# OPTML-Group/Unlearn-Saliency

Measured on AMD Instinct MI355X. Metric: unlearn_steps_per_sec (ResNet-18/CIFAR-10 10%-forget, RL + SalUn mask, batch 256/GPU), higher is better.
Workload: dtype f32

## Files before the change

include/salun.h:

```cpp
#ifndef SALUN_H
#define SALUN_H

#include <stddef.h>
#include <stdint.h>

#ifdef __cplusplus
extern "C" {
#endif

#define SALUN_OK 0
#define SALUN_EINVAL (-22)
#define SALUN_ENOSPC (-28)
#define SALUN_EIO (-5)

#define SALUN_MAX_THRESHOLDS 16

typedef void *salun_stream_t;

int salun_version(void);
const char *salun_strerror(int code);
const char *salun_arch(void);
int salun_clock_probe(unsigned long long *out , int samples, int spins, salun_stream_t stream);

int salun_saliency_accumulate(float *acc , const float *g ,
                              double scale, const float *sqnorm ,
                              double max_norm, int64_t n, salun_stream_t stream);

#define SALUN_TOPK_FORCE_FULL_SCAN 1u
#define SALUN_TOPK_VALUES_ONLY 2u
size_t salun_mask_topk_workspace_bytes(int64_t n, int nk);
int salun_mask_topk(const float *acc , int64_t n, const int64_t *ks ,
                    int nk, uint8_t *const *masks_out ,
                    void *ws , size_t ws_bytes, salun_stream_t stream);
int salun_mask_topk_ex(const float *acc , int64_t n, const int64_t *ks ,
                       int nk, uint8_t *const *masks_out ,
                       void *ws , size_t ws_bytes, unsigned flags, salun_stream_t stream);
int salun_mask_topk_status(const void *ws , int *route_out , int *error_out ,
                           salun_stream_t stream);
int salun_mask_topk_thresholds(const void *ws , int nk, float *tau_out ,
                               salun_stream_t stream);

int salun_mask_u8_to_i64(const uint8_t *m , int64_t *out , int64_t n,
                         salun_stream_t stream);
int salun_mask_i64_to_u8(const int64_t *m , uint8_t *out , int64_t n,
                         salun_stream_t stream);
int salun_mask_popcount(const uint8_t *m , int64_t n, int64_t *count ,
                        void *ws , size_t ws_bytes, salun_stream_t stream);

int salun_masked_sgd_step(float *p , const float *g , float *buf ,
                          const uint8_t *m , double lr, double mu,
                          double wd, int first_step, int64_t n, salun_stream_t stream);

size_t salun_reduce_workspace_bytes(int64_t n);
int salun_grad_sqnorm(const float *g , int64_t n, float *out ,
                      void *ws , size_t ws_bytes, salun_stream_t stream);

int salun_masked_adam_step(float *p , const float *g , float *m1 ,
                           float *v , const uint8_t *mask ,
                           const float *sqnorm , double max_norm,
                           double gscale, double lr, double b1, double b2, double eps,
                           double wd, int step, int64_t n, salun_stream_t stream);

int salun_adam_coefficients(int64_t *step , double lr, double b1, double b2, float *coef ,
                            salun_stream_t stream);
int salun_masked_adam_step_coef(float *p , const float *g , float *m1 , float *v ,
                                const uint8_t *mask , const float *sqnorm ,
                                double max_norm, double gscale, const float *coef , double b1, double b2,
                                double eps, double wd, int64_t n, salun_stream_t stream);

int salun_adam_ema_step(float *p , const float *g , float *m1 , float *v ,
                        float *shadow , const uint8_t *mask ,
                        const float *sqnorm , double max_norm, double gscale, double lr, double b1,
                        double b2, double eps, double wd, double mu, int step, int64_t n, salun_stream_t stream);
int salun_adam_ema_step_coef(float *p , const float *g , float *m1 , float *v ,
                             float *shadow , const uint8_t *mask ,
                             const float *sqnorm , double max_norm, double gscale,
                             const float *coef , double b1, double b2, double eps, double wd, double mu,
                             int64_t n, salun_stream_t stream);

int salun_qsample(const float *x0 , const float *e ,
                  const float *sqrt_ab , const float *sqrt_1mab ,
                  const int64_t *t , int64_t T, float *xt , int64_t B,
                  int64_t chw, salun_stream_t stream);

size_t salun_sqerr_workspace_bytes(int64_t B, int64_t chw);
int salun_sqerr_loss(const float *a , const float *b , int64_t B,
                     int64_t chw, double coef, float *loss ,
                     float *per_sample , float *dloss_db ,
                     void *ws , size_t ws_bytes, salun_stream_t stream);

int salun_fim_square_accumulate(float *F , float *tmp , double n_data,
                                int64_t n, salun_stream_t stream);

int salun_conv2d_forward(const float *x , const float *w , const float *bias ,
                         float *y , int N, int C, int H, int W, int K, int R, int stride, int pad,
                         int P, int Q, salun_stream_t stream);
int salun_conv2d_forward_fused(const float *x , const float *w , const float *bias ,
                               const float *nbias , const float *addend ,
                               float *y , int N, int C, int H, int W, int K, int R, int stride, int pad,
                               int P, int Q, void *ws , size_t ws_bytes, salun_stream_t stream);
size_t salun_conv2d_data_workspace_bytes(int N, int outC, int outH, int outW, int R, int conv_stride);
int salun_conv2d_backward_data_ws(const float *dy , const float *w , const float *addend ,
                                  float *dx , int N, int C, int H, int W, int K, int R, int stride, int pad,
                                  int P, int Q, void *ws , size_t ws_bytes, salun_stream_t stream);
int salun_conv2d_backward_data(const float *dy , const float *w , float *dx , int N, int C,
                               int H, int W, int K, int R, int stride, int pad, int P, int Q,
                               salun_stream_t stream);
int salun_conv2d_backward_data_add(const float *dy , const float *w , const float *addend ,
                                   float *dx , int N, int C, int H, int W, int K, int R, int stride, int pad,
                                   int P, int Q, salun_stream_t stream);
size_t salun_channel_sum_workspace_bytes(int N, int K);
int salun_channel_sum(const float *dy , float *out , int N, int K, int HW, int accumulate,
                      void *ws , size_t ws_bytes, salun_stream_t stream);
size_t salun_conv2d_wgrad_workspace_bytes(int N, int C, int K, int R, int P, int Q);
int salun_conv2d_backward_weight(const float *x , const float *dy , float *dw , int N, int C,
                                 int H, int W, int K, int R, int stride, int pad, int P, int Q, int accumulate,
                                 void *ws , size_t ws_bytes, salun_stream_t stream);
#define SALUN_WGRAD_SHARED 1u
int salun_conv2d_backward_weight_ex(const float *x , const float *dy , float *dw , int N, int C,
                                    int H, int W, int K, int R, int stride, int pad, int P, int Q, int accumulate,
                                    unsigned flags, void *ws , size_t ws_bytes, salun_stream_t stream);

size_t salun_conv3x3_pack_bytes(int K, int C, int dgrad);
#define SALUN_PACK_MAX_JOBS 32
typedef struct {
  const float *w;
  float *img_fwd;
  float *img_dgrad;
  int32_t K, C;
} salun_pack_job_t;
int salun_conv3x3_pack_weights(const salun_pack_job_t *jobs , int njobs, salun_stream_t stream);
int salun_conv3x3_packed(const float *x , const float *img , const float *bias ,
                         const float *nbias , const float *addend , float *y ,
                         int N, int Cred, int H, int W, int Kout, int cfg, salun_stream_t stream);

int salun_conv2d_bf16_supported(int C, int K, int R, int stride, int pad);
int salun_conv2d_bf16_pack_weights(const float *w , uint16_t *wp , int K, int C, int R,
                                   salun_stream_t stream);
#define SALUN_BF16_PACK_MAX_JOBS 64
typedef struct {
  const float *w;
  uint16_t *wp;
  int32_t K, C, R, transposed;
} salun_bf16_pack_job_t;
int salun_bf16_pack_weights_batch(const salun_bf16_pack_job_t *jobs, int n, salun_stream_t stream);
size_t salun_conv2d_bf16_data_workspace_bytes(int N, int H, int W, int C, int K, int R, int stride, int pad);
int salun_conv2d_bf16_forward(const uint16_t *x , const uint16_t *wp , const float *bias ,
                              const float *nbias , const uint16_t *addend ,
                              uint16_t *y , int N, int H, int W, int C, int K, int R, int stride, int pad,
                              void *ws , size_t ws_bytes, salun_stream_t stream);
int salun_conv2d_bf16_backward_data(const uint16_t *dy , const uint16_t *wp ,
                                    const uint16_t *addend , uint16_t *dx , int N, int H, int W,
                                    int C, int K, int R, int stride, int pad, void *ws , size_t ws_bytes,
                                    salun_stream_t stream);
size_t salun_conv2d_bf16_wgrad_workspace_bytes(int N, int H, int W, int C, int K, int R, int stride, int pad);
int salun_conv2d_bf16_backward_weight(const uint16_t *x , const uint16_t *dy , float *dw ,
                                      float *db , int N, int H, int W, int C, int K, int R, int stride,
                                      int pad, int accumulate, void *ws , size_t ws_bytes,
                                      salun_stream_t stream);
size_t salun_colsum_bf16_workspace_bytes(int K);
int salun_colsum_bf16(const uint16_t *dy , float *db , float *dnb , int64_t M, int K,
                      int images, int accumulate, void *ws , size_t ws_bytes, salun_stream_t stream);
int salun_conv2d_bf16_backward_weight_ex(const uint16_t *x , const uint16_t *dy , float *dw ,
                                         float *db , float *dnb , int N, int H, int W, int C,
                                         int K, int R, int stride, int pad, int accumulate, void *ws ,
                                         size_t ws_bytes, salun_stream_t stream);

size_t salun_gn_bf16_workspace_bytes(int N, int C, int HW, int G);
int salun_gn_bf16_forward(const uint16_t *x , const float *gamma , const float *beta ,
                          uint16_t *y , float *mr , float *ab , int N, int C, int HW, int G,
                          double eps, int silu, void *ws , size_t ws_bytes, salun_stream_t stream);
int salun_gn_bf16_backward(const uint16_t *dy , const uint16_t *x , const float *gamma ,
                           const float *mr , const float *ab , uint16_t *dx , float *dgamma ,
                           float *dbeta , int N, int C, int HW, int G, int silu, int accumulate, void *ws ,
                           size_t ws_bytes, salun_stream_t stream);

int salun_attn_supported(int D);
int salun_attn_forward(const uint16_t *q , const uint16_t *k , const uint16_t *v , uint16_t *o ,
                       float *lse , int B, int H, int Nq, int Nk, int D, long long q_bs, int q_ld,
                       long long k_bs, int k_ld, long long v_bs, int v_ld, long long o_bs, int o_ld, double scale,
                       salun_stream_t stream);
int salun_attn_backward(const uint16_t *q , const uint16_t *k , const uint16_t *v ,
                        const uint16_t *o , const uint16_t *d_o , const float *lse ,
                        uint16_t *dq , uint16_t *dk , uint16_t *dv , float *dsum , int B, int H,
                        int Nq, int Nk, int D, long long q_bs, int q_ld, long long k_bs, int k_ld, long long v_bs, int v_ld,
                        long long o_bs, int o_ld, long long do_bs, int do_ld, double scale, salun_stream_t stream);

size_t salun_ln_bf16_workspace_bytes(int64_t rows, int C);
int salun_ln_bf16_forward(const uint16_t *x , const float *gamma , const float *beta ,
                          uint16_t *y , float *stats , int64_t rows, int C, double eps,
                          salun_stream_t stream);
int salun_ln_bf16_backward(const uint16_t *dy , const uint16_t *x , const float *gamma ,
                           const float *stats , uint16_t *dx , float *dgamma , float *dbeta ,
                           int64_t rows, int C, int accumulate, void *ws , size_t ws_bytes, salun_stream_t stream);
int salun_geglu_bf16_forward(const uint16_t *h , uint16_t *out , int64_t rows, int F, salun_stream_t stream);
int salun_geglu_bf16_backward(const uint16_t *h , const uint16_t *dy , uint16_t *dh , int64_t rows,
                              int F, salun_stream_t stream);

size_t salun_bn_workspace_bytes(int C);
int salun_bn_forward(const float *x , const float *res , float *y ,
                     const float *gamma , const float *beta , float *running_mean ,
                     float *running_var , long long *num_batches_tracked ,
                     float *save_mean , float *save_invstd ,
                     int N, int C, int HW, int training, double momentum, double eps, int relu, void *ws ,
                     size_t ws_bytes, salun_stream_t stream);
int salun_bn_backward(const float *dy , const float *y , const float *x ,
                      const float *gamma , const float *save_mean , const float *save_invstd ,
                      float *dx , float *dres , float *dgamma , float *dbeta ,
                      float *grad_gamma_acc , float *grad_beta_acc ,
                      int N, int C, int HW, int training, int relu, void *ws , size_t ws_bytes,
                      salun_stream_t stream);

size_t salun_gn_workspace_bytes(int N, int C);
int salun_gn_forward(const float *x , float *y , const float *gamma , const float *beta ,
                     float *save_mean , float *save_rstd , int N, int C, int HW, int G, double eps,
                     int silu, salun_stream_t stream);
int salun_gn_backward(const float *dz , const float *x , const float *gamma ,
                      const float *beta , const float *save_mean , const float *save_rstd ,
                      float *dx , float *dgamma , float *dbeta ,
                      float *grad_gamma_acc , float *grad_beta_acc ,
                      int N, int C, int HW, int G, int silu, void *ws , size_t ws_bytes,
                      salun_stream_t stream);

int salun_gn_backward_fused(const float *dz , const float *x , const float *gamma ,
                            const float *beta , const float *save_mean , const float *save_rstd ,
                            const float *addend , float *dx , float *dgamma ,
                            float *dbeta , float *grad_gamma_acc ,
                            float *grad_beta_acc , float *nk_sum ,
                            float *csum , float *csum_acc , int N, int C, int HW, int G,
                            int silu, void *ws , size_t ws_bytes, salun_stream_t stream);

int salun_param_diff(const float *p , const float *p0 , float *out , int64_t n,
                     salun_stream_t stream);
int salun_soft_threshold_step(float *p , const float *p0 , const float *tau ,
                              int64_t n, salun_stream_t stream);

size_t salun_ewc_workspace_bytes(int64_t n);
int salun_ewc_penalty_grad(const float *p , const float *p_star , const float *F ,
                           float *g , double lambda, float *loss_out , int64_t n,
                           void *ws , size_t ws_bytes, salun_stream_t stream);

int salun_image_batch(const uint8_t *data , const int64_t *idx ,
                      const int32_t *crop , const uint8_t *flip ,
                      float *out , int64_t B, int H, int W, int C, int pad,
                      salun_stream_t stream);

#define SALUN_GEMM_MAX_JOBS 32
#define SALUN_GEMM_MAX_SEGS 32
typedef struct {
  const float *A , *B ;
  int32_t K;
  int32_t a_i, a_k, b_j, b_k;
} salun_gemm_seg_t;
typedef struct {
  float *C ;
  const float *bias ;
  int32_t M, N, ldc;
  int32_t seg0, nseg;
  int32_t accumulate;
} salun_gemm_job_t;
size_t salun_gemm_f32_workspace_bytes(const salun_gemm_job_t *jobs , int njobs,
                                      const salun_gemm_seg_t *segs , int nsegs,
                                      int batch_outer, int batch_inner);
int salun_gemm_f32(const salun_gemm_job_t *jobs , int njobs, const salun_gemm_seg_t *segs , int nsegs,
                   int batch_outer, int batch_inner, const int64_t *batch_strides ,
                   double alpha, void *ws , size_t ws_bytes, salun_stream_t stream);
size_t salun_colsum_f32_workspace_bytes(int64_t M, int N);
int salun_colsum_f32(const float *x , float *out , int64_t M, int N, int64_t ld, int accumulate,
                     void *ws , size_t ws_bytes, salun_stream_t stream);
int salun_softmax_rows(float *s , int64_t rows, int n, int ld, salun_stream_t stream);
int salun_softmax_rows_backward(const float *p , float *dp , int64_t rows, int n, int ld,
                                double scale, salun_stream_t stream);

int salun_gemm_bf16_supported(int64_t M, int N, int K);
int salun_gemm_bf16_nt(const void *x , const void *w , const float *bias ,
                       const void *addend , void *y , int64_t M, int N, int K,
                       int variant, salun_stream_t stream);
int salun_gemm_bf16_tn_supported(int64_t M, int Na, int Nb);
size_t salun_gemm_bf16_tn_workspace_bytes(int64_t M, int Na, int Nb, int variant);
int salun_gemm_bf16_tn(const void *dy , const void *x , float *dw , int64_t M, int Na, int Nb,
                       int accumulate, int variant, void *ws , size_t ws_bytes, salun_stream_t stream);
int salun_pack_bf16(const float *w , void *wp , int N, int K, int transposed, salun_stream_t stream);

int salun_dropout(const float *x , float *y , int64_t n_samples, int64_t chw,
                  int64_t sample_offset, double p, uint64_t seed,
                  const uint64_t *seed_dev , salun_stream_t stream);
int salun_u64_add(uint64_t *value , uint64_t inc, salun_stream_t stream);

size_t salun_iu_dot_workspace_bytes(int B, int64_t n);
int salun_iu_conv_dot(const float *y2 , const float *dy , int B, int64_t n, double *out ,
                      void *ws , size_t ws_bytes, salun_stream_t stream);
int salun_iu_bn_dot(const float *x , const float *dy , const float *running_mean ,
                    const float *running_var , double eps, const float *u0_gamma ,
                    const float *u0_beta , const float *u1_gamma , const float *u1_beta ,
                    int B, int C, int HW, double *out , void *ws , size_t ws_bytes,
                    salun_stream_t stream);
int salun_iu_linear_dot(const float *x , const float *dy , const float *u0_w ,
                        const float *u0_b , const float *u1_w , const float *u1_b ,
                        int B, int M, int K, double *out , salun_stream_t stream);
int salun_iu_recurrence(const double *ab , int64_t n, double N, double *out ,
                        salun_stream_t stream);
int salun_iu_apply(float *p , const float *v , const float *g0 , const double *beta ,
                   const uint8_t *mask , double alpha, int64_t n, salun_stream_t stream);

size_t salun_ff_conv_sq_workspace_bytes(int G, int B, int C, int K, int R, int P, int Q);
int salun_ff_conv_sq(const float *x , const float *dy , const float *w , float *F ,
                     int G, int B, int C, int H, int W, int K, int R, int stride, int pad, int P, int Q,
                     void *ws , size_t ws_bytes, salun_stream_t stream);
int salun_ff_linear_sq(const float *x , const float *dy , const float *w , float *F ,
                       int G, int B, int M, int K, salun_stream_t stream);
size_t salun_ff_vec_sq_workspace_bytes(int G, int C);
int salun_ff_vec_sq(const float *x , const float *dy , const float *running_mean ,
                    const float *running_var , double eps, const float *w , int G, int B,
                    int C, int HW, float *F_gamma , float *F_beta , void *ws ,
                    size_t ws_bytes, salun_stream_t stream);
int salun_ff_apply(float *p , const float *F , const int64_t *table , int nparam, int64_t ntiles,
                   double nbatches, double alpha, uint64_t seed, salun_stream_t stream);

int salun_fill_uniform(float *out , int64_t n, uint64_t seed, double lo, double hi,
                       salun_stream_t stream);
int salun_fill_normal(float *out , int64_t n, uint64_t seed, double mean, double std,
                      salun_stream_t stream);
int salun_fill_u8(uint8_t *out , int64_t n, uint64_t seed, salun_stream_t stream);

#define SALUN_SAMPLER_ANCESTRAL 0
#define SALUN_SAMPLER_GENERALIZED 1
int salun_sampler_step(const float *x_t , const float *eps_cond , const float *eps_null ,
                       double cond_scale, const float *abar , int table_len, int idx_t, int idx_next, int variant,
                       double eta, const float *noise , uint64_t seed,
                       const int64_t *image_ids , int64_t step, float *x_next ,
                       float *x0 , int64_t B, int64_t chw, salun_stream_t stream);

int salun_sampler_noise(float *out , uint64_t seed, const int64_t *image_ids , int64_t step, int64_t B,
                        int64_t chw, salun_stream_t stream);

size_t salun_minmax_workspace_bytes(int64_t n);
int salun_minmax(const float *x , int64_t n, float *lohi , void *ws , size_t ws_bytes,
                 salun_stream_t stream);

int salun_images_to_u8(const float *x , uint8_t *out , int64_t B, int C, int HW, int rescaled,
                       const float *range , salun_stream_t stream);

#ifdef __cplusplus
}
#endif
#endif
```

unlearn_saliency_amd/_lib.py:

```python
from __future__ import annotations

import ctypes
import os
import subprocess

_HERE = os.path.dirname(os.path.abspath(__file__))
LIB_PATH = os.environ.get("SALUN_LIB") or os.path.join(_HERE, "libsalun.so")
CSRC_DIR = os.path.join(_HERE, "csrc")

SALUN_OK = 0
SALUN_EINVAL = -22
SALUN_ENOSPC = -28
SALUN_EIO = -5
SALUN_MAX_THRESHOLDS = 16
SALUN_TOPK_FORCE_FULL_SCAN = 1
SALUN_TOPK_VALUES_ONLY = 2
SALUN_WGRAD_SHARED = 1

c_void_p, c_int, c_int64, c_uint64 = ctypes.c_void_p, ctypes.c_int, ctypes.c_int64, ctypes.c_uint64
c_double, c_size_t = ctypes.c_double, ctypes.c_size_t

class GemmSeg(ctypes.Structure):
    _fields_ = [("A", c_void_p), ("B", c_void_p), ("K", ctypes.c_int32), ("a_i", ctypes.c_int32),
                ("a_k", ctypes.c_int32), ("b_j", ctypes.c_int32), ("b_k", ctypes.c_int32)]


class GemmJob(ctypes.Structure):
    _fields_ = [("C", c_void_p), ("bias", c_void_p), ("M", ctypes.c_int32), ("N", ctypes.c_int32),
                ("ldc", ctypes.c_int32), ("seg0", ctypes.c_int32), ("nseg", ctypes.c_int32),
                ("accumulate", ctypes.c_int32)]


class PackJob(ctypes.Structure):
    _fields_ = [("w", c_void_p), ("img_fwd", c_void_p), ("img_dgrad", c_void_p), ("K", ctypes.c_int32),
                ("C", ctypes.c_int32)]


class Bf16PackJob(ctypes.Structure):
    _fields_ = [("w", c_void_p), ("wp", c_void_p), ("K", ctypes.c_int32), ("C", ctypes.c_int32), ("R", ctypes.c_int32),
                ("transposed", ctypes.c_int32)]


SALUN_BF16_PACK_MAX_JOBS = 64
SALUN_GEMM_MAX_JOBS = 32
SALUN_GEMM_MAX_SEGS = 32

SIGNATURES = {
    "salun_version": (c_int, []),
    "salun_strerror": (ctypes.c_char_p, [c_int]),
    "salun_arch": (ctypes.c_char_p, []),
    "salun_clock_probe": (c_int, [c_void_p, c_int, c_int, c_void_p]),
    "salun_saliency_accumulate": (c_int, [c_void_p, c_void_p, c_double, c_void_p, c_double, c_int64, c_void_p]),
    "salun_mask_topk_workspace_bytes": (c_size_t, [c_int64, c_int]),
    "salun_mask_topk": (c_int, [c_void_p, c_int64, ctypes.POINTER(c_int64), c_int, ctypes.POINTER(c_void_p),
                                c_void_p, c_size_t, c_void_p]),
    "salun_mask_topk_ex": (c_int, [c_void_p, c_int64, ctypes.POINTER(c_int64), c_int, ctypes.POINTER(c_void_p),
                                   c_void_p, c_size_t, ctypes.c_uint, c_void_p]),
    "salun_mask_topk_status": (c_int, [c_void_p, ctypes.POINTER(c_int), ctypes.POINTER(c_int), c_void_p]),
    "salun_mask_topk_thresholds": (c_int, [c_void_p, c_int, c_void_p, c_void_p]),
    "salun_mask_u8_to_i64": (c_int, [c_void_p, c_void_p, c_int64, c_void_p]),
    "salun_mask_i64_to_u8": (c_int, [c_void_p, c_void_p, c_int64, c_void_p]),
    "salun_mask_popcount": (c_int, [c_void_p, c_int64, c_void_p, c_void_p, c_size_t, c_void_p]),
    "salun_masked_sgd_step": (c_int, [c_void_p, c_void_p, c_void_p, c_void_p, c_double, c_double, c_double, c_int,
                                      c_int64, c_void_p]),
    "salun_reduce_workspace_bytes": (c_size_t, [c_int64]),
    "salun_grad_sqnorm": (c_int, [c_void_p, c_int64, c_void_p, c_void_p, c_size_t, c_void_p]),
    "salun_masked_adam_step": (c_int, [c_void_p, c_void_p, c_void_p, c_void_p, c_void_p, c_void_p, c_double,
                                       c_double, c_double, c_double, c_double, c_double, c_double, c_int, c_int64,
                                       c_void_p]),
    "salun_adam_coefficients": (c_int, [c_void_p, c_double, c_double, c_double, c_void_p, c_void_p]),
    "salun_masked_adam_step_coef": (c_int, [c_void_p, c_void_p, c_void_p, c_void_p, c_void_p, c_void_p, c_double,
                                            c_double, c_void_p, c_double, c_double, c_double, c_double, c_int64,
                                            c_void_p]),
    "salun_adam_ema_step": (c_int, [c_void_p, c_void_p, c_void_p, c_void_p, c_void_p, c_void_p, c_void_p, c_double,
                                    c_double, c_double, c_double, c_double, c_double, c_double, c_double, c_int, c_int64,
                                    c_void_p]),
    "salun_adam_ema_step_coef": (c_int, [c_void_p, c_void_p, c_void_p, c_void_p, c_void_p, c_void_p, c_void_p, c_double,
                                         c_double, c_void_p, c_double, c_double, c_double, c_double, c_double, c_int64,
                                         c_void_p]),
    "salun_qsample": (c_int, [c_void_p, c_void_p, c_void_p, c_void_p, c_void_p, c_int64, c_void_p, c_int64, c_int64,
                              c_void_p]),
    "salun_sqerr_workspace_bytes": (c_size_t, [c_int64, c_int64]),
    "salun_sqerr_loss": (c_int, [c_void_p, c_void_p, c_int64, c_int64, c_double, c_void_p, c_void_p, c_void_p,
                                 c_void_p, c_size_t, c_void_p]),
    "salun_fim_square_accumulate": (c_int, [c_void_p, c_void_p, c_double, c_int64, c_void_p]),
    "salun_conv2d_forward": (c_int, [c_void_p, c_void_p, c_void_p, c_void_p] + [c_int] * 10 + [c_void_p]),
    "salun_conv2d_forward_fused": (c_int, [c_void_p] * 6 + [c_int] * 10 + [c_void_p, c_size_t, c_void_p]),
    "salun_conv2d_data_workspace_bytes": (c_size_t, [c_int] * 6),
    "salun_conv2d_backward_data_ws": (c_int, [c_void_p] * 4 + [c_int] * 10 + [c_void_p, c_size_t, c_void_p]),
    "salun_conv2d_backward_data": (c_int, [c_void_p, c_void_p, c_void_p] + [c_int] * 10 + [c_void_p]),
    "salun_channel_sum_workspace_bytes": (c_size_t, [c_int] * 2),
    "salun_channel_sum": (c_int, [c_void_p, c_void_p] + [c_int] * 4 + [c_void_p, c_size_t, c_void_p]),
    "salun_conv2d_wgrad_workspace_bytes": (c_size_t, [c_int] * 6),
    "salun_conv3x3_pack_bytes": (c_size_t, [c_int] * 3),
    "salun_conv3x3_pack_weights": (c_int, [c_void_p, c_int, c_void_p]),
    "salun_conv3x3_packed": (c_int, [c_void_p] * 6 + [c_int] * 6 + [c_void_p]),
    "salun_conv2d_backward_weight": (c_int, [c_void_p, c_void_p, c_void_p] + [c_int] * 11 + [c_void_p, c_size_t,
                                                                                          c_void_p]),
    "salun_conv2d_backward_weight_ex": (c_int, [c_void_p, c_void_p, c_void_p] + [c_int] * 11 + [ctypes.c_uint, c_void_p,
                                                                                                 c_size_t, c_void_p]),
    "salun_conv2d_bf16_supported": (c_int, [c_int] * 5),
    "salun_conv2d_bf16_pack_weights": (c_int, [c_void_p, c_void_p, c_int, c_int, c_int, c_void_p]),
    "salun_bf16_pack_weights_batch": (c_int, [c_void_p, c_int, c_void_p]),
    "salun_conv2d_bf16_data_workspace_bytes": (c_size_t, [c_int] * 8),
    "salun_conv2d_bf16_forward": (c_int, [c_void_p] * 6 + [c_int] * 8 + [c_void_p, c_size_t, c_void_p]),
    "salun_conv2d_bf16_backward_data": (c_int, [c_void_p] * 4 + [c_int] * 8 + [c_void_p, c_size_t, c_void_p]),
    "salun_conv2d_bf16_wgrad_workspace_bytes": (c_size_t, [c_int] * 8),
    "salun_conv2d_bf16_backward_weight": (c_int, [c_void_p] * 4 + [c_int] * 9 + [c_void_p, c_size_t, c_void_p]),
    "salun_colsum_bf16_workspace_bytes": (c_size_t, [c_int]),
    "salun_colsum_bf16": (c_int, [c_void_p, c_void_p, c_void_p, c_int64, c_int, c_int, c_int, c_void_p, c_size_t, c_void_p]),
    "salun_conv2d_bf16_backward_weight_ex": (c_int, [c_void_p] * 5 + [c_int] * 9 + [c_void_p, c_size_t, c_void_p]),
    "salun_gn_bf16_workspace_bytes": (c_size_t, [c_int] * 4),
    "salun_gn_bf16_forward": (c_int, [c_void_p] * 6 + [c_int] * 4 + [c_double, c_int, c_void_p, c_size_t, c_void_p]),
    "salun_gn_bf16_backward": (c_int, [c_void_p] * 8 + [c_int] * 6 + [c_void_p, c_size_t, c_void_p]),
    "salun_attn_supported": (c_int, [c_int]),
    "salun_attn_forward": (c_int, [c_void_p] * 5 + [c_int] * 5 + [ctypes.c_longlong, c_int] * 4 + [c_double, c_void_p]),
    "salun_attn_backward": (c_int, [c_void_p] * 10 + [c_int] * 5 + [ctypes.c_longlong, c_int] * 5 + [c_double, c_void_p]),
    "salun_ln_bf16_workspace_bytes": (c_size_t, [c_int64, c_int]),
    "salun_ln_bf16_forward": (c_int, [c_void_p] * 5 + [c_int64, c_int, c_double, c_void_p]),
    "salun_ln_bf16_backward": (c_int, [c_void_p] * 7 + [c_int64, c_int, c_int, c_void_p, c_size_t, c_void_p]),
    "salun_geglu_bf16_forward": (c_int, [c_void_p, c_void_p, c_int64, c_int, c_void_p]),
    "salun_geglu_bf16_backward": (c_int, [c_void_p, c_void_p, c_void_p, c_int64, c_int, c_void_p]),
    "salun_bn_workspace_bytes": (c_size_t, [c_int]),
    "salun_bn_forward": (c_int, [c_void_p] * 10 + [c_int] * 4 + [c_double, c_double, c_int, c_void_p, c_size_t, c_void_p]),
    "salun_bn_backward": (c_int, [c_void_p] * 12 + [c_int] * 5 + [c_void_p, c_size_t, c_void_p]),
    "salun_conv2d_backward_data_add": (c_int, [c_void_p] * 4 + [c_int] * 10 + [c_void_p]),
    "salun_gn_workspace_bytes": (c_size_t, [c_int, c_int]),
    "salun_gn_forward": (c_int, [c_void_p] * 6 + [c_int] * 4 + [c_double, c_int, c_void_p]),
    "salun_gn_backward": (c_int, [c_void_p] * 11 + [c_int] * 5 + [c_void_p, c_size_t, c_void_p]),
    "salun_gn_backward_fused": (c_int, [c_void_p] * 15 + [c_int] * 5 + [c_void_p, c_size_t, c_void_p]),
    "salun_param_diff": (c_int, [c_void_p, c_void_p, c_void_p, c_int64, c_void_p]),
    "salun_soft_threshold_step": (c_int, [c_void_p, c_void_p, c_void_p, c_int64, c_void_p]),
    "salun_ewc_workspace_bytes": (c_size_t, [c_int64]),
    "salun_ewc_penalty_grad": (c_int, [c_void_p] * 4 + [c_double, c_void_p, c_int64, c_void_p, c_size_t, c_void_p]),
    "salun_image_batch": (c_int, [c_void_p, c_void_p, c_void_p, c_void_p, c_void_p, c_int64, c_int, c_int, c_int,
                                  c_int, c_void_p]),
    "salun_gemm_f32_workspace_bytes": (c_size_t, [ctypes.POINTER(GemmJob), c_int, ctypes.POINTER(GemmSeg), c_int, c_int,
                                                  c_int]),
    "salun_gemm_f32": (c_int, [ctypes.POINTER(GemmJob), c_int, ctypes.POINTER(GemmSeg), c_int, c_int, c_int,
                               ctypes.POINTER(c_int64), c_double, c_void_p, c_size_t, c_void_p]),
    "salun_colsum_f32_workspace_bytes": (c_size_t, [c_int64, c_int]),
    "salun_colsum_f32": (c_int, [c_void_p, c_void_p, c_int64, c_int, c_int64, c_int, c_void_p, c_size_t, c_void_p]),
    "salun_softmax_rows": (c_int, [c_void_p, c_int64, c_int, c_int, c_void_p]),
    "salun_softmax_rows_backward": (c_int, [c_void_p, c_void_p, c_int64, c_int, c_int, c_double, c_void_p]),
    "salun_gemm_bf16_supported": (c_int, [c_int64, c_int, c_int]),
    "salun_gemm_bf16_nt": (c_int, [c_void_p, c_void_p, c_void_p, c_void_p, c_void_p, c_int64, c_int, c_int, c_int, c_void_p]),
    "salun_pack_bf16": (c_int, [c_void_p, c_void_p, c_int, c_int, c_int, c_void_p]),
    "salun_gemm_bf16_tn_supported": (c_int, [c_int64, c_int, c_int]),
    "salun_gemm_bf16_tn_workspace_bytes": (c_size_t, [c_int64, c_int, c_int, c_int]),
    "salun_gemm_bf16_tn": (c_int, [c_void_p, c_void_p, c_void_p, c_int64, c_int, c_int, c_int, c_int, c_void_p, c_size_t, c_void_p]),
    "salun_dropout": (c_int, [c_void_p, c_void_p, c_int64, c_int64, c_int64, c_double, c_uint64, c_void_p, c_void_p]),
    "salun_u64_add": (c_int, [c_void_p, c_uint64, c_void_p]),
    "salun_iu_dot_workspace_bytes": (c_size_t, [c_int, c_int64]),
    "salun_iu_conv_dot": (c_int, [c_void_p, c_void_p, c_int, c_int64, c_void_p, c_void_p, c_size_t, c_void_p]),
    "salun_iu_bn_dot": (c_int, [c_void_p] * 4 + [c_double] + [c_void_p] * 4 + [c_int] * 3 + [c_void_p, c_void_p,
                                                                                           c_size_t, c_void_p]),
    "salun_iu_linear_dot": (c_int, [c_void_p] * 6 + [c_int] * 3 + [c_void_p, c_void_p]),
    "salun_iu_recurrence": (c_int, [c_void_p, c_int64, c_double, c_void_p, c_void_p]),
    "salun_iu_apply": (c_int, [c_void_p] * 5 + [c_double, c_int64, c_void_p]),
    "salun_ff_conv_sq_workspace_bytes": (c_size_t, [c_int] * 7),
    "salun_ff_conv_sq": (c_int, [c_void_p] * 4 + [c_int] * 11 + [c_void_p, c_size_t, c_void_p]),
    "salun_ff_linear_sq": (c_int, [c_void_p] * 4 + [c_int] * 4 + [c_void_p]),
    "salun_ff_vec_sq_workspace_bytes": (c_size_t, [c_int, c_int]),
    "salun_ff_vec_sq": (c_int, [c_void_p] * 4 + [c_double, c_void_p] + [c_int] * 4 + [c_void_p] * 3
                        + [c_size_t, c_void_p]),
    "salun_ff_apply": (c_int, [c_void_p] * 3 + [c_int, c_int64, c_double, c_double, c_uint64, c_void_p]),
    "salun_fill_uniform": (c_int, [c_void_p, c_int64, c_uint64, c_double, c_double, c_void_p]),
    "salun_fill_normal": (c_int, [c_void_p, c_int64, c_uint64, c_double, c_double, c_void_p]),
    "salun_fill_u8": (c_int, [c_void_p, c_int64, c_uint64, c_void_p]),
    "salun_sampler_step": (c_int, [c_void_p, c_void_p, c_void_p, c_double, c_void_p, c_int, c_int, c_int, c_int,
                                   c_double, c_void_p, c_uint64, c_void_p, c_int64, c_void_p, c_void_p, c_int64,
                                   c_int64, c_void_p]),
    "salun_sampler_noise": (c_int, [c_void_p, c_uint64, c_void_p, c_int64, c_int64, c_int64, c_void_p]),
    "salun_minmax_workspace_bytes": (c_size_t, [c_int64]),
    "salun_minmax": (c_int, [c_void_p, c_int64, c_void_p, c_void_p, c_size_t, c_void_p]),
    "salun_images_to_u8": (c_int, [c_void_p, c_void_p, c_int64, c_int, c_int, c_int, c_void_p, c_void_p]),
}

_lib = None


def build(verbose: bool = False) -> str:
    cmd = ["make", "-C", CSRC_DIR, "-j4"] + ([] if verbose else ["-s"])
    subprocess.check_call(cmd)
    if not os.path.exists(LIB_PATH):
        raise RuntimeError(f"build did not produce {LIB_PATH}")
    return LIB_PATH


def lib() -> ctypes.CDLL:
    global _lib
    if _lib is None:
        if not os.path.exists(LIB_PATH):
            raise ImportError(
                f"{LIB_PATH} is missing: the SalUn HIP extension has not been built "
                f"(run `make -C {CSRC_DIR}` or `python -c 'import __graft_entry__ as g; g.build()'`). "
                "There is no CPU fallback.")
        L = ctypes.CDLL(LIB_PATH)
        for name, (res, args) in SIGNATURES.items():
            try:
                fn = getattr(L, name)
            except AttributeError as e:
                raise ImportError(f"{LIB_PATH} does not export {name}; rebuild it") from e
            fn.restype = res
            fn.argtypes = args
        _lib = L
    return _lib


class SalunError(RuntimeError):
    pass


def check(code: int, what: str) -> None:
    if code != SALUN_OK:
        msg = lib().salun_strerror(code).decode()
        raise SalunError(f"{what} failed: {msg} ({code})")
```

unlearn_saliency_amd/csrc/salun_norm.hip:

```cpp
#include "salun_common.h"

namespace {

constexpr int BN_MAX_SPLIT = 64;


struct BnWalk {
  int n, i, dn, di, hw4;
  __device__ __forceinline__ BnWalk(int n_lo, int hw4_) : hw4(hw4_) {
    const int t = threadIdx.x;
    n = n_lo + t / hw4_;
    i = t - (t / hw4_) * hw4_;
    dn = 256 / hw4_;
    di = 256 - dn * hw4_;
  }
  __device__ __forceinline__ void next() {
    n += dn;
    i += di;
    if (i >= hw4) { i -= hw4; ++n; }
  }
};

__global__ __launch_bounds__(256) void k_bn_stats_partial(const float *__restrict__ x, int N, int C, int HW, int nsplit,
                                                          double *__restrict__ partial) {
  __shared__ double lds[4];
  const int c = blockIdx.x, s = blockIdx.y;
  const int n_lo = (int)((int64_t)N * s / nsplit), n_hi = (int)((int64_t)N * (s + 1) / nsplit);
  float s1 = 0.f, s2 = 0.f;
  double d1 = 0.0, d2 = 0.0;
  const int hw4 = HW >> 2;
  const int work = (n_hi - n_lo) * hw4;
  int it = 0;
  BnWalk wk(n_lo, hw4);
#pragma unroll 2
  for (int e = threadIdx.x; e < work; e += 256, ++it, wk.next()) {
    const int n = wk.n, i = wk.i;
    const float4 v = reinterpret_cast<const float4 *>(x + ((size_t)n * C + c) * HW)[i];
    s1 += (v.x + v.y) + (v.z + v.w);
    s2 += (v.x * v.x + v.y * v.y) + (v.z * v.z + v.w * v.w);
    if ((it & 7) == 7) { d1 += s1; d2 += s2; s1 = 0.f; s2 = 0.f; }
  }
  d1 += s1; d2 += s2;
  const double t1 = salun_block_sum(d1, lds);
  const double t2 = salun_block_sum(d2, lds);
  if (threadIdx.x == 0) {
    partial[((size_t)c * nsplit + s) * 2 + 0] = t1;
    partial[((size_t)c * nsplit + s) * 2 + 1] = t2;
  }
}

__device__ __forceinline__ void bn_channel_stats(const double *__restrict__ partial, int c, int nsplit, double M,
                                                 float eps, float *s_out , bool publish,
                                                 float momentum, float *__restrict__ mean, float *__restrict__ invstd,
                                                 float *__restrict__ running_mean, float *__restrict__ running_var) {
  if (threadIdx.x < 64) {
    double s1 = 0.0, s2 = 0.0;
    if ((int)threadIdx.x < nsplit) {
      s1 = partial[((size_t)c * nsplit + threadIdx.x) * 2 + 0];
      s2 = partial[((size_t)c * nsplit + threadIdx.x) * 2 + 1];
    }
    s1 = salun_wave_sum(s1);
    s2 = salun_wave_sum(s2);
    if (threadIdx.x == 0) {
      const double mu = s1 / M;
      double var = s2 / M - mu * mu;
      if (var < 0.0) var = 0.0;
      const float is = (float)(1.0 / sqrt(var + (double)eps));
      s_out[0] = (float)mu;
      s_out[1] = is;
      if (publish) {
        mean[c] = (float)mu;
        invstd[c] = is;
        if (running_mean) {
          running_mean[c] = (1.f - momentum) * running_mean[c] + momentum * (float)mu;
          const double unbiased = (M > 1.0) ? var * M / (M - 1.0) : var;
          running_var[c] = (1.f - momentum) * running_var[c] + momentum * (float)unbiased;
        }
      }
    }
  }
  __syncthreads();
}

template <bool RELU, bool RES, bool TRAIN>
__global__ __launch_bounds__(256) void k_bn_apply(const float *__restrict__ x, const float *__restrict__ res,
                                                  float *__restrict__ y, const double *__restrict__ partial,
                                                  float *__restrict__ mean, float *__restrict__ invstd,
                                                  const float *__restrict__ gamma, const float *__restrict__ beta,
                                                  float *__restrict__ running_mean, float *__restrict__ running_var,
                                                  long long *__restrict__ num_batches_tracked, int N, int C, int HW,
                                                  int nsplit, float eps, float momentum) {
  __shared__ float st[2];
  const int c = blockIdx.x, s = blockIdx.y;
  if (TRAIN) {
    if (num_batches_tracked && c == 0 && s == 0 && threadIdx.x == 0) *num_batches_tracked += 1;
    bn_channel_stats(partial, c, nsplit, (double)N * HW, eps, st, s == 0, momentum, mean, invstd, running_mean,
                     running_var);
  } else {
    if (threadIdx.x == 0) {
      st[0] = running_mean[c];
      st[1] = 1.0f / sqrtf(running_var[c] + eps);
      if (s == 0) { mean[c] = st[0]; invstd[c] = st[1]; }
    }
    __syncthreads();
  }
  const float a = st[1] * gamma[c];
  const float b = beta[c] - st[0] * a;
  const int n_lo = (int)((int64_t)N * s / nsplit), n_hi = (int)((int64_t)N * (s + 1) / nsplit);
  const int hw4 = HW >> 2;
  const int work = (n_hi - n_lo) * hw4;
  BnWalk wk(n_lo, hw4);
#pragma unroll 2
  for (int e = threadIdx.x; e < work; e += 256, wk.next()) {
    const int n = wk.n, i = wk.i;
    const size_t off = ((size_t)n * C + c) * HW;
    const float4 v = reinterpret_cast<const float4 *>(x + off)[i];
    float4 o;
    o.x = v.x * a + b; o.y = v.y * a + b; o.z = v.z * a + b; o.w = v.w * a + b;
    if (RES) {
      const float4 r = reinterpret_cast<const float4 *>(res + off)[i];
      o.x += r.x; o.y += r.y; o.z += r.z; o.w += r.w;
    }
    if (RELU) {
      o.x = o.x > 0.f ? o.x : 0.f; o.y = o.y > 0.f ? o.y : 0.f;
      o.z = o.z > 0.f ? o.z : 0.f; o.w = o.w > 0.f ? o.w : 0.f;
    }
    reinterpret_cast<float4 *>(y + off)[i] = o;
  }
}

template <bool RELU>
__global__ __launch_bounds__(256) void k_bn_bwd_partial(const float *__restrict__ dy, const float *__restrict__ y,
                                                        const float *__restrict__ x, const float *__restrict__ mean,
                                                        const float *__restrict__ invstd, int N, int C, int HW,
                                                        int nsplit, double *__restrict__ partial) {
  __shared__ double lds[4];
  const int c = blockIdx.x, s = blockIdx.y;
  const int n_lo = (int)((int64_t)N * s / nsplit), n_hi = (int)((int64_t)N * (s + 1) / nsplit);
  const float mu = mean[c], is = invstd[c];
  float s1 = 0.f, s2 = 0.f;
  double d1 = 0.0, d2 = 0.0;
  const int hw4 = HW >> 2;
  const int work = (n_hi - n_lo) * hw4;
  int it = 0;
  BnWalk wk(n_lo, hw4);
#pragma unroll 2
  for (int e = threadIdx.x; e < work; e += 256, ++it, wk.next()) {
    const int n = wk.n, i = wk.i;
    const size_t off = ((size_t)n * C + c) * HW;
    float4 g = reinterpret_cast<const float4 *>(dy + off)[i];
    const float4 xv = reinterpret_cast<const float4 *>(x + off)[i];
    if (RELU) {
      const float4 yv = reinterpret_cast<const float4 *>(y + off)[i];
      g.x = yv.x > 0.f ? g.x : 0.f; g.y = yv.y > 0.f ? g.y : 0.f;
      g.z = yv.z > 0.f ? g.z : 0.f; g.w = yv.w > 0.f ? g.w : 0.f;
    }
    s1 += (g.x + g.y) + (g.z + g.w);
    s2 += (g.x * ((xv.x - mu) * is) + g.y * ((xv.y - mu) * is)) + (g.z * ((xv.z - mu) * is) + g.w * ((xv.w - mu) * is));
    if ((it & 7) == 7) { d1 += s1; d2 += s2; s1 = 0.f; s2 = 0.f; }
  }
  d1 += s1; d2 += s2;
  const double t1 = salun_block_sum(d1, lds);
  const double t2 = salun_block_sum(d2, lds);
  if (threadIdx.x == 0) {
    partial[((size_t)c * nsplit + s) * 2 + 0] = t1;
    partial[((size_t)c * nsplit + s) * 2 + 1] = t2;
  }
}

template <bool RELU, bool TRAIN, bool DRES>
__global__ __launch_bounds__(256) void k_bn_bwd_apply(const float *__restrict__ dy, const float *__restrict__ y,
                                                      const float *__restrict__ x, const float *__restrict__ mean,
                                                      const float *__restrict__ invstd,
                                                      const float *__restrict__ gamma,
                                                      const double *__restrict__ partial, float *__restrict__ dgamma,
                                                      float *__restrict__ dbeta, float *__restrict__ gacc,
                                                      float *__restrict__ bacc, float *__restrict__ dx,
                                                      float *__restrict__ dres, int N, int C, int HW, int nsplit,
                                                      float inv_m) {
  __shared__ float sg[2];
  const int c = blockIdx.x, s = blockIdx.y;
  if (threadIdx.x < 64) {
    double s1 = 0.0, s2 = 0.0;
    if ((int)threadIdx.x < nsplit) {
      s1 = partial[((size_t)c * nsplit + threadIdx.x) * 2 + 0];
      s2 = partial[((size_t)c * nsplit + threadIdx.x) * 2 + 1];
    }
    s1 = salun_wave_sum(s1);
    s2 = salun_wave_sum(s2);
    if (threadIdx.x == 0) {
      sg[0] = (float)s1;
      sg[1] = (float)s2;
      if (s == 0) {
        dbeta[c] = (float)s1;
        dgamma[c] = (float)s2;
        if (gacc) gacc[c] += (float)s2;
        if (bacc) bacc[c] += (float)s1;
      }
    }
  }
  __syncthreads();
  const float mu = mean[c], is = invstd[c];
  const float gi = gamma[c] * is;
  const float kb = sg[0] * inv_m, kg = sg[1] * inv_m;
  const int n_lo = (int)((int64_t)N * s / nsplit), n_hi = (int)((int64_t)N * (s + 1) / nsplit);
  const int hw4 = HW >> 2;
  const int work = (n_hi - n_lo) * hw4;
  BnWalk wk(n_lo, hw4);
#pragma unroll 2
  for (int e = threadIdx.x; e < work; e += 256, wk.next()) {
    const int n = wk.n, i = wk.i;
    const size_t off = ((size_t)n * C + c) * HW;
    float4 g = reinterpret_cast<const float4 *>(dy + off)[i];
    if (RELU) {
      const float4 yv = reinterpret_cast<const float4 *>(y + off)[i];
      g.x = yv.x > 0.f ? g.x : 0.f; g.y = yv.y > 0.f ? g.y : 0.f;
      g.z = yv.z > 0.f ? g.z : 0.f; g.w = yv.w > 0.f ? g.w : 0.f;
    }
    if (DRES) reinterpret_cast<float4 *>(dres + off)[i] = g;
    float4 o;
    if (TRAIN) {
      const float4 xv = reinterpret_cast<const float4 *>(x + off)[i];
      o.x = gi * (g.x - (kb + ((xv.x - mu) * is) * kg));
      o.y = gi * (g.y - (kb + ((xv.y - mu) * is) * kg));
      o.z = gi * (g.z - (kb + ((xv.z - mu) * is) * kg));
      o.w = gi * (g.w - (kb + ((xv.w - mu) * is) * kg));
    } else {
      o.x = gi * g.x; o.y = gi * g.y; o.z = gi * g.z; o.w = gi * g.w;
    }
    reinterpret_cast<float4 *>(dx + off)[i] = o;
  }
}

inline int bn_nsplit(int N, int C) {
  int ns = (1024 + C - 1) / C;
  if (ns > N) ns = N;
  if (ns > BN_MAX_SPLIT) ns = BN_MAX_SPLIT;
  if (ns < 1) ns = 1;
  return ns;
}

}

SALUN_EXPORT size_t salun_bn_workspace_bytes(int C) {
  return sizeof(double) * 2 * (size_t)(C > 0 ? C : 0) * BN_MAX_SPLIT;
}

SALUN_EXPORT int salun_bn_forward(const float *x, const float *res, float *y, const float *gamma, const float *beta,
                                  float *running_mean, float *running_var, long long *num_batches_tracked,
                                  float *save_mean, float *save_invstd, int N, int C, int HW, int training,
                                  double momentum, double eps, int relu, void *ws, size_t ws_bytes,
                                  salun_stream_t stream) {
  if (!x || !y || !gamma || !beta || !save_mean || !save_invstd || N < 1 || C < 1 || HW < 4 || (HW & 3))
    return SALUN_EINVAL;
  if (!training && (!running_mean || !running_var)) return SALUN_EINVAL;
  if (!salun_aligned16(x) || !salun_aligned16(y) || (res && !salun_aligned16(res))) return SALUN_EINVAL;
  hipStream_t st = salun_hip_stream(stream);
  const int ns = bn_nsplit(N, C);
  double *partial = static_cast<double *>(ws);
  if (training) {
    if (!ws || ws_bytes < salun_bn_workspace_bytes(C)) return SALUN_ENOSPC;
    hipLaunchKernelGGL(k_bn_stats_partial, dim3(C, ns), dim3(256), 0, st, x, N, C, HW, ns, partial);
    SALUN_LAUNCH_CHECK();
  }
#define SALUN_BN_APPLY(RELU_, RES_, TRAIN_)                                                                       \
  hipLaunchKernelGGL((k_bn_apply<RELU_, RES_, TRAIN_>), dim3(C, ns), dim3(256), 0, st, x, res, y, partial,         \
                     save_mean, save_invstd, gamma, beta, running_mean, running_var, num_batches_tracked, N, C,  \
                     HW, ns, (float)eps, (float)momentum)
  const bool r = relu != 0, a = res != nullptr, t = training != 0;
  if (r && a && t) SALUN_BN_APPLY(true, true, true);
  else if (r && a) SALUN_BN_APPLY(true, true, false);
  else if (r && t) SALUN_BN_APPLY(true, false, true);
  else if (r) SALUN_BN_APPLY(true, false, false);
  else if (a && t) SALUN_BN_APPLY(false, true, true);
  else if (a) SALUN_BN_APPLY(false, true, false);
  else if (t) SALUN_BN_APPLY(false, false, true);
  else SALUN_BN_APPLY(false, false, false);
#undef SALUN_BN_APPLY
  SALUN_LAUNCH_CHECK();
  return SALUN_OK;
}

SALUN_EXPORT int salun_bn_backward(const float *dy, const float *y, const float *x, const float *gamma,
                                   const float *save_mean, const float *save_invstd, float *dx, float *dres,
                                   float *dgamma, float *dbeta, float *grad_gamma_acc, float *grad_beta_acc, int N,
                                   int C, int HW, int training, int relu, void *ws, size_t ws_bytes,
                                   salun_stream_t stream) {
  if (!dy || !x || !gamma || !save_mean || !save_invstd || !dx || !dgamma || !dbeta || N < 1 || C < 1 || HW < 4 ||
      (HW & 3) || (relu && !y))
    return SALUN_EINVAL;
  if (!ws || ws_bytes < salun_bn_workspace_bytes(C)) return SALUN_ENOSPC;
  if (!salun_aligned16(dy) || !salun_aligned16(x) || !salun_aligned16(dx) || (y && !salun_aligned16(y)) ||
      (dres && !salun_aligned16(dres)))
    return SALUN_EINVAL;
  hipStream_t st = salun_hip_stream(stream);
  const int ns = bn_nsplit(N, C);
  double *partial = static_cast<double *>(ws);
  if (relu) hipLaunchKernelGGL(k_bn_bwd_partial<true>, dim3(C, ns), dim3(256), 0, st, dy, y, x, save_mean, save_invstd, N, C, HW, ns, partial);
  else hipLaunchKernelGGL(k_bn_bwd_partial<false>, dim3(C, ns), dim3(256), 0, st, dy, y, x, save_mean, save_invstd, N, C, HW, ns, partial);
  SALUN_LAUNCH_CHECK();
  const float inv_m = (float)(1.0 / ((double)N * HW));
#define SALUN_BN_BWD(RELU_, TRAIN_, DRES_)                                                                          \
  hipLaunchKernelGGL((k_bn_bwd_apply<RELU_, TRAIN_, DRES_>), dim3(C, ns), dim3(256), 0, st, dy, y, x, save_mean,   \
                     save_invstd, gamma, partial, dgamma, dbeta, grad_gamma_acc, grad_beta_acc, dx, dres, N, C, HW, \
                     ns, inv_m)
  const bool r = relu != 0, t = training != 0, d = dres != nullptr;
  if (r && t && d) SALUN_BN_BWD(true, true, true);
  else if (r && t) SALUN_BN_BWD(true, true, false);
  else if (r && d) SALUN_BN_BWD(true, false, true);
  else if (r) SALUN_BN_BWD(true, false, false);
  else if (t && d) SALUN_BN_BWD(false, true, true);
  else if (t) SALUN_BN_BWD(false, true, false);
  else if (d) SALUN_BN_BWD(false, false, true);
  else SALUN_BN_BWD(false, false, false);
#undef SALUN_BN_BWD
  SALUN_LAUNCH_CHECK();
  return SALUN_OK;
}

namespace {

constexpr int GN_ITEMS = 16;
constexpr int GN_MAX_SEG = 1024;

__device__ __forceinline__ float gn_sigmoid(float y) { return 1.0f / (1.0f + expf(-y)); }

__device__ __forceinline__ float seg_sum(float v, int r) {
  for (int off = 1; off < r; off <<= 1) v += __shfl_xor(v, off, 64);
  return v;
}

template <bool SILU, int ITEMS>
__global__ __launch_bounds__(256) void k_gn_fwd(const float *__restrict__ x, float *__restrict__ y,
                                                const float *__restrict__ gamma, const float *__restrict__ beta,
                                                float *__restrict__ mean, float *__restrict__ rstd, int C, int HW,
                                                int G, float eps) {
  constexpr bool CACHED = ITEMS > 0;
  __shared__ double lds[4];
  __shared__ float st[2];
  const int ng = blockIdx.x, n = ng / G, g = ng - n * G;
  const int cpg = C / G;
  const int L = cpg * HW, nvec = L >> 2;
  const size_t base = ((size_t)n * C + (size_t)g * cpg) * HW;
  const float4 *xv = reinterpret_cast<const float4 *>(x + base);
  float4 v[CACHED ? ITEMS : 1];
  float s1 = 0.f, s2 = 0.f;
  double d1 = 0.0, d2 = 0.0;
  if (CACHED) {
#pragma unroll
    for (int i = 0; i < (CACHED ? ITEMS : 1); ++i) {
      const int e = threadIdx.x + i * 256;
      if (e < nvec) v[i] = xv[e];
    }
#pragma unroll
    for (int i = 0; i < (CACHED ? ITEMS : 1); ++i) {
      const int e = threadIdx.x + i * 256;
      if (e < nvec) {
        s1 += (v[i].x + v[i].y) + (v[i].z + v[i].w);
        s2 += (v[i].x * v[i].x + v[i].y * v[i].y) + (v[i].z * v[i].z + v[i].w * v[i].w);
      }
    }
    d1 = s1; d2 = s2;
  } else {
    int it = 0;
    for (int e = threadIdx.x; e < nvec; e += 256, ++it) {
      const float4 t = xv[e];
      s1 += (t.x + t.y) + (t.z + t.w);
      s2 += (t.x * t.x + t.y * t.y) + (t.z * t.z + t.w * t.w);
      if ((it & 15) == 15) { d1 += s1; d2 += s2; s1 = 0.f; s2 = 0.f; }
    }
    d1 += s1; d2 += s2;
  }
  const double t1 = salun_block_sum(d1, lds);
  const double t2 = salun_block_sum(d2, lds);
  if (threadIdx.x == 0) {
    const double mu = t1 / L;
    double var = t2 / L - mu * mu;
    if (var < 0.0) var = 0.0;
    st[0] = (float)mu;
    st[1] = (float)(1.0 / sqrt(var + (double)eps));
    mean[ng] = st[0];
    rstd[ng] = st[1];
  }
  __syncthreads();
  const float mu = st[0], rs = st[1];
  const int hw4 = HW >> 2;
  float4 *yv = reinterpret_cast<float4 *>(y + base);
  auto apply = [&](int e, float4 t) {
    const int c = g * cpg + e / hw4;
    const float a = rs * gamma[c];
    const float b = beta[c] - mu * a;
    float4 o;
    o.x = t.x * a + b; o.y = t.y * a + b; o.z = t.z * a + b; o.w = t.w * a + b;
    if (SILU) {
      o.x = o.x * gn_sigmoid(o.x); o.y = o.y * gn_sigmoid(o.y);
      o.z = o.z * gn_sigmoid(o.z); o.w = o.w * gn_sigmoid(o.w);
    }
    yv[e] = o;
  };
  if (CACHED) {
#pragma unroll
    for (int i = 0; i < (CACHED ? ITEMS : 1); ++i) {
      const int e = threadIdx.x + i * 256;
      if (e < nvec) apply(e, v[i]);
    }
  } else {
    for (int e = threadIdx.x; e < nvec; e += 256) apply(e, xv[e]);
  }
}

template <bool SILU, int ITEMS, bool EXTRA>
__global__ __launch_bounds__(256) void k_gn_bwd(const float *__restrict__ dz, const float *__restrict__ x,
                                                const float *__restrict__ gamma, const float *__restrict__ beta,
                                                const float *__restrict__ mean, const float *__restrict__ rstd,
                                                float *__restrict__ dx, float *__restrict__ part_dgamma,
                                                float *__restrict__ part_dbeta, int C, int HW, int G,
                                                const float *__restrict__ addend, float *__restrict__ nk_sum) {
  constexpr bool CACHED = ITEMS > 0;
  __shared__ float seg_g[GN_MAX_SEG], seg_b[GN_MAX_SEG];
  __shared__ float grp[2];
  const int ng = blockIdx.x, n = ng / G, g = ng - n * G;
  const int cpg = C / G;
  const int L = cpg * HW, nvec = L >> 2, hw4 = HW >> 2;
  const size_t base = ((size_t)n * C + (size_t)g * cpg) * HW;
  const float4 *xv = reinterpret_cast<const float4 *>(x + base);
  const float4 *gv = reinterpret_cast<const float4 *>(dz + base);
  const float mu = mean[ng], rs = rstd[ng];
  const int r = hw4 < 64 ? hw4 : 64;
  const int segs_per_ch = hw4 / r;
  float4 xc[CACHED ? ITEMS : 1], dc[CACHED ? ITEMS : 1];
  float gac[CACHED ? ITEMS : 1], bec[CACHED ? ITEMS : 1];

  auto dy_of = [&](float ga, float be, float4 xt, float4 gt, float4 &xh) {
    xh.x = (xt.x - mu) * rs; xh.y = (xt.y - mu) * rs; xh.z = (xt.z - mu) * rs; xh.w = (xt.w - mu) * rs;
    if (SILU) {
      const float y0 = xh.x * ga + be, y1 = xh.y * ga + be, y2 = xh.z * ga + be, y3 = xh.w * ga + be;
      const float s0 = gn_sigmoid(y0), s1 = gn_sigmoid(y1), s2 = gn_sigmoid(y2), s3 = gn_sigmoid(y3);
      gt.x = gt.x * (s0 * (1.0f + y0 * (1.0f - s0)));
      gt.y = gt.y * (s1 * (1.0f + y1 * (1.0f - s1)));
      gt.z = gt.z * (s2 * (1.0f + y2 * (1.0f - s2)));
      gt.w = gt.w * (s3 * (1.0f + y3 * (1.0f - s3)));
    }
    return gt;
  };
  auto seg_accumulate = [&](int e, float4 dyv, float4 xh, bool valid) {
    float sg = valid ? (dyv.x * xh.x + dyv.y * xh.y) + (dyv.z * xh.z + dyv.w * xh.w) : 0.f;
    float sb = valid ? (dyv.x + dyv.y) + (dyv.z + dyv.w) : 0.f;
    sg = seg_sum(sg, r);
    sb = seg_sum(sb, r);
    if (valid && (threadIdx.x & (r - 1)) == 0) {
      seg_g[e / r] = sg;
      seg_b[e / r] = sb;
    }
  };
  const int nround = (nvec + 255) / 256;
  if (CACHED) {
#pragma unroll
    for (int i = 0; i < (CACHED ? ITEMS : 1); ++i) {
      const int e = threadIdx.x + i * 256;
      if (e < nvec) {
        xc[i] = xv[e];
        dc[i] = gv[e];
        const int c = g * cpg + e / hw4;
        gac[i] = gamma[c];
        bec[i] = beta[c];
      }
    }
#pragma unroll
    for (int i = 0; i < (CACHED ? ITEMS : 1); ++i) {
      if (i < nround) {
        const int e = threadIdx.x + i * 256;
        const bool valid = e < nvec;
        float4 xh = make_float4(0.f, 0.f, 0.f, 0.f);
        if (valid) dc[i] = dy_of(gac[i], bec[i], xc[i], dc[i], xh);
        seg_accumulate(valid ? e : 0, valid ? dc[i] : xh, xh, valid);
      }
    }
  } else {
    for (int i = 0; i < nround; ++i) {
      const int e = threadIdx.x + i * 256;
      const bool valid = e < nvec;
      float4 xh = make_float4(0.f, 0.f, 0.f, 0.f), d = xh;
      if (valid) {
        const int c = g * cpg + e / hw4;
        d = dy_of(gamma[c], beta[c], xv[e], gv[e], xh);
      }
      seg_accumulate(valid ? e : 0, d, xh, valid);
    }
  }
  __syncthreads();
  float my_g = 0.f, my_b = 0.f;
  if ((int)threadIdx.x < cpg) {
    for (int s = 0; s < segs_per_ch; ++s) {
      my_g += seg_g[threadIdx.x * segs_per_ch + s];
      my_b += seg_b[threadIdx.x * segs_per_ch + s];
    }
    const int c = g * cpg + threadIdx.x;
    part_dgamma[(size_t)n * C + c] = my_g;
    part_dbeta[(size_t)n * C + c] = my_b;
  }
  __syncthreads();
  if ((int)threadIdx.x < cpg) {
    const float ga = gamma[g * cpg + threadIdx.x];
    seg_g[threadIdx.x] = my_g * ga;
    seg_b[threadIdx.x] = my_b * ga;
  }
  __syncthreads();
  if (threadIdx.x == 0) {
    float a = 0.f, b = 0.f;
    for (int c = 0; c < cpg; ++c) { b += seg_g[c]; a += seg_b[c]; }
    grp[0] = a / (float)L;
    grp[1] = b / (float)L;
  }
  __syncthreads();
  const float ma = grp[0], mb = grp[1];
  float4 *ov = reinterpret_cast<float4 *>(dx + base);
  const float4 *av = reinterpret_cast<const float4 *>(EXTRA && addend ? addend + base : nullptr);
  auto emit = [&](int e, float ga, float4 xt, float4 dyv) {
    float4 o;
    o.x = rs * (dyv.x * ga - ma - ((xt.x - mu) * rs) * mb);
    o.y = rs * (dyv.y * ga - ma - ((xt.y - mu) * rs) * mb);
    o.z = rs * (dyv.z * ga - ma - ((xt.z - mu) * rs) * mb);
    o.w = rs * (dyv.w * ga - ma - ((xt.w - mu) * rs) * mb);
    if (EXTRA && av) {
      const float4 ad = av[e];
      o.x += ad.x; o.y += ad.y; o.z += ad.z; o.w += ad.w;
    }
    ov[e] = o;
    return o;
  };
  const bool want_nk = EXTRA && nk_sum != nullptr;
  auto nk_accumulate = [&](int e, float4 o, bool valid) {
    float sv = valid ? (o.x + o.y) + (o.z + o.w) : 0.f;
    sv = seg_sum(sv, r);
    if (valid && (threadIdx.x & (r - 1)) == 0) seg_g[e / r] = sv;
  };
  if (CACHED) {
#pragma unroll
    for (int i = 0; i < (CACHED ? ITEMS : 1); ++i) {
      const int e = threadIdx.x + i * 256;
      const bool valid = e < nvec;
      float4 o = make_float4(0.f, 0.f, 0.f, 0.f);
      if (valid) o = emit(e, gac[i], xc[i], dc[i]);
      if (EXTRA) {
        if (want_nk && i < nround) nk_accumulate(valid ? e : 0, o, valid);
      }
    }
  } else {
    for (int i = 0; i < nround; ++i) {
      const int e = threadIdx.x + i * 256;
      const bool valid = e < nvec;
      float4 o = make_float4(0.f, 0.f, 0.f, 0.f);
      if (valid) {
        float4 xh;
        const float4 xt = xv[e];
        const int c = g * cpg + e / hw4;
        const float ga = gamma[c];
        o = emit(e, ga, xt, dy_of(ga, beta[c], xt, gv[e], xh));
      }
      if (EXTRA) {
        if (want_nk) nk_accumulate(valid ? e : 0, o, valid);
      }
    }
  }
  if (EXTRA) {
    if (want_nk) {
      __syncthreads();
      if ((int)threadIdx.x < cpg) {
        float t = 0.f;
        for (int sgi = 0; sgi < segs_per_ch; ++sgi) t += seg_g[threadIdx.x * segs_per_ch + sgi];
        nk_sum[(size_t)n * C + g * cpg + threadIdx.x] = t;
      }
    }
  }
}

__global__ __launch_bounds__(256) void k_gn_bwd_final(const float *__restrict__ part_dgamma,
                                                      const float *__restrict__ part_dbeta, int N, int C,
                                                      float *__restrict__ dgamma, float *__restrict__ dbeta,
                                                      float *__restrict__ gacc, float *__restrict__ bacc,
                                                      const float *__restrict__ part_nk ,
                                                      float *__restrict__ csum ,
                                                      float *__restrict__ csum_acc ) {
  __shared__ double s_g[8][33], s_b[8][33], s_k[8][33];
  const int cx = threadIdx.x & 31, ry = threadIdx.x >> 5;
  const int c = blockIdx.x * 32 + cx;
  double sg = 0.0, sb = 0.0, sk = 0.0;
  if (c < C)
    for (int n = ry; n < N; n += 8) {
      sg += (double)part_dgamma[(size_t)n * C + c];
      sb += (double)part_dbeta[(size_t)n * C + c];
      if (part_nk) sk += (double)part_nk[(size_t)n * C + c];
    }
  s_g[ry][cx] = sg; s_b[ry][cx] = sb; s_k[ry][cx] = sk;
  __syncthreads();
  if (ry != 0 || c >= C) return;
  for (int q = 1; q < 8; ++q) { sg += s_g[q][cx]; sb += s_b[q][cx]; sk += s_k[q][cx]; }
  dgamma[c] = (float)sg;
  dbeta[c] = (float)sb;
  if (gacc) gacc[c] += (float)sg;
  if (bacc) bacc[c] += (float)sb;
  if (part_nk && csum) csum[c] = (float)sk;
  if (part_nk && csum_acc) csum_acc[c] += (float)sk;
}

inline int gn_items(int C, int HW, int G) {
  const int64_t nvec = (int64_t)(C / G) * HW / 4;
  for (int it = 1; it <= GN_ITEMS; it <<= 1)
    if (nvec <= (int64_t)it * 256) return it;
  return 0;
}

inline bool gn_shape_ok(int N, int C, int HW, int G) {
  if (N < 1 || C < 1 || G < 1 || C % G != 0 || HW < 4 || (HW & (HW - 1)) != 0) return false;
  const int cpg = C / G;
  if (cpg > 256) return false;
  const int hw4 = HW >> 2, r = hw4 < 64 ? hw4 : 64;
  return (int64_t)cpg * hw4 / r <= GN_MAX_SEG && (int64_t)cpg * HW < (1 << 30);
}

}

SALUN_EXPORT size_t salun_gn_workspace_bytes(int N, int C) {
  return sizeof(float) * 2 * (size_t)(N > 0 ? N : 0) * (size_t)(C > 0 ? C : 0);
}

SALUN_EXPORT int salun_gn_forward(const float *x, float *y, const float *gamma, const float *beta, float *save_mean,
                                  float *save_rstd, int N, int C, int HW, int G, double eps, int silu,
                                  salun_stream_t stream) {
  if (!x || !y || !gamma || !beta || !save_mean || !save_rstd || !gn_shape_ok(N, C, HW, G)) return SALUN_EINVAL;
  if (!salun_aligned16(x) || !salun_aligned16(y)) return SALUN_EINVAL;
  hipStream_t st = salun_hip_stream(stream);
  const int items = gn_items(C, HW, G);
#define SALUN_GN_FWD(S_, I_) \
  hipLaunchKernelGGL((k_gn_fwd<S_, I_>), dim3(N * G), dim3(256), 0, st, x, y, gamma, beta, save_mean, save_rstd, C, HW, G, (float)eps)
#define SALUN_GN_FWD_I(S_)                    \
  switch (items) {                            \
    case 1: SALUN_GN_FWD(S_, 1); break;       \
    case 2: SALUN_GN_FWD(S_, 2); break;       \
    case 4: SALUN_GN_FWD(S_, 4); break;       \
    case 8: SALUN_GN_FWD(S_, 8); break;       \
    case 16: SALUN_GN_FWD(S_, 16); break;     \
    default: SALUN_GN_FWD(S_, 0); break;      \
  }
  if (silu) { SALUN_GN_FWD_I(true) } else { SALUN_GN_FWD_I(false) }
#undef SALUN_GN_FWD_I
#undef SALUN_GN_FWD
  SALUN_LAUNCH_CHECK();
  return SALUN_OK;
}

SALUN_EXPORT int salun_gn_backward_fused(const float *dz, const float *x, const float *gamma, const float *beta,
                                         const float *save_mean, const float *save_rstd, const float *addend,
                                         float *dx, float *dgamma, float *dbeta, float *grad_gamma_acc,
                                         float *grad_beta_acc, float *nk_sum, float *csum, float *csum_acc, int N,
                                         int C, int HW, int G, int silu, void *ws, size_t ws_bytes,
                                         salun_stream_t stream) {
  if (!dz || !x || !gamma || !beta || !save_mean || !save_rstd || !dx || !dgamma || !dbeta || !gn_shape_ok(N, C, HW, G))
    return SALUN_EINVAL;
  if ((csum || csum_acc) && !nk_sum) return SALUN_EINVAL;
  if (addend == dx) return SALUN_EINVAL;
  if (!ws || ws_bytes < salun_gn_workspace_bytes(N, C)) return SALUN_ENOSPC;
  if (!salun_aligned16(dz) || !salun_aligned16(x) || !salun_aligned16(dx) || (addend && !salun_aligned16(addend)))
    return SALUN_EINVAL;
  hipStream_t st = salun_hip_stream(stream);
  float *pg = static_cast<float *>(ws), *pb = pg + (size_t)N * C;
  const int items = gn_items(C, HW, G);
  const bool extra = addend != nullptr || nk_sum != nullptr;
#define SALUN_GN_BWD(S_, I_, E_) \
  hipLaunchKernelGGL((k_gn_bwd<S_, I_, E_>), dim3(N * G), dim3(256), 0, st, dz, x, gamma, beta, save_mean, save_rstd, dx, pg, pb, C, HW, G, addend, nk_sum)
#define SALUN_GN_BWD_I(S_, E_)                    \
  switch (items) {                                \
    case 1: SALUN_GN_BWD(S_, 1, E_); break;       \
    case 2: SALUN_GN_BWD(S_, 2, E_); break;       \
    case 4: SALUN_GN_BWD(S_, 4, E_); break;       \
    case 8: SALUN_GN_BWD(S_, 8, E_); break;       \
    case 16: SALUN_GN_BWD(S_, 16, E_); break;     \
    default: SALUN_GN_BWD(S_, 0, E_); break;      \
  }
  if (silu) {
    if (extra) { SALUN_GN_BWD_I(true, true) } else { SALUN_GN_BWD_I(true, false) }
  } else {
    if (extra) { SALUN_GN_BWD_I(false, true) } else { SALUN_GN_BWD_I(false, false) }
  }
#undef SALUN_GN_BWD_I
#undef SALUN_GN_BWD
  SALUN_LAUNCH_CHECK();
  hipLaunchKernelGGL(k_gn_bwd_final, dim3((C + 31) / 32), dim3(256), 0, st, pg, pb, N, C, dgamma, dbeta,
                     grad_gamma_acc, grad_beta_acc, nk_sum, csum, csum_acc);
  SALUN_LAUNCH_CHECK();
  return SALUN_OK;
}

SALUN_EXPORT int salun_gn_backward(const float *dz, const float *x, const float *gamma, const float *beta,
                                   const float *save_mean, const float *save_rstd, float *dx, float *dgamma,
                                   float *dbeta, float *grad_gamma_acc, float *grad_beta_acc, int N, int C, int HW,
                                   int G, int silu, void *ws, size_t ws_bytes, salun_stream_t stream) {
  return salun_gn_backward_fused(dz, x, gamma, beta, save_mean, save_rstd, nullptr, dx, dgamma, dbeta, grad_gamma_acc,
                                 grad_beta_acc, nullptr, nullptr, nullptr, N, C, HW, G, silu, ws, ws_bytes, stream);
}
```

unlearn_saliency_amd/norm.py:

```python
from __future__ import annotations

import torch

from .fastfn import FastFunction
import torch.nn as nn
import torch.nn.functional as F

from . import gradsink, ops


class _FusedBN(FastFunction):
    @staticmethod
    def forward(ctx, x, weight, bias, residual, running_mean, running_var, training, momentum, eps, relu, nbt=None):
        out = ops.bn_forward(x, residual, weight, bias, running_mean, running_var, training, momentum, eps, relu, nbt)
        if out is None:
            raise RuntimeError("fused BN: unsupported shape (H*W must be a multiple of 4)")
        y, mean, invstd = out
        ctx.save_for_backward(x, y if relu else None, weight, bias, mean, invstd)
        ctx.params = (weight, bias)
        ctx.cfg = (bool(training), bool(relu), residual is not None)
        ctx.mark_non_differentiable(mean, invstd)
        return y

    @staticmethod
    def backward(ctx, dy):
        x, y, weight, bias, mean, invstd = ctx.saved_tensors
        training, relu, has_res = ctx.cfg
        gw, gb = gradsink.sink(ctx.params[0]), gradsink.sink(ctx.params[1])
        if gw is None or gb is None:
            gw = gb = None
        dx, dres, dgamma, dbeta = ops.bn_backward(dy.contiguous(), y, x, weight, mean, invstd, training, relu,
                                                  has_res and ctx.needs_input_grad[3], gw, gb)
        if gw is not None:
            gradsink.arrived(weight)
            gradsink.arrived(bias)
            dgamma = dbeta = None
        return dx, dgamma, dbeta, dres, None, None, None, None, None, None, None


def _eligible(x: torch.Tensor, bn: nn.BatchNorm2d) -> bool:
    return (type(bn) is nn.BatchNorm2d and x.is_cuda and x.dtype == torch.float32 and x.dim() == 4 and (x.shape[2] * x.shape[3]) % 4 == 0
            and bn.affine and bn.track_running_stats and bn.momentum is not None and not torch.is_autocast_enabled())


def fused_bn_act(x: torch.Tensor, bn: nn.BatchNorm2d, residual: torch.Tensor = None, relu: bool = True):
    if not _eligible(x, bn):
        y = bn(x)
        if residual is not None:
            y = y + residual
        return F.relu(y) if relu else y
    x = x.contiguous()
    if residual is not None:
        residual = residual.contiguous()
    return _FusedBN.apply(x, bn.weight, bn.bias, residual, bn.running_mean, bn.running_var, bn.training,
                          bn.momentum, bn.eps, relu, bn.num_batches_tracked)


class _FusedGN(FastFunction):
    @staticmethod
    def forward(ctx, x, weight, bias, groups, eps, silu):
        out = ops.gn_forward(x, weight, bias, groups, eps, silu)
        if out is None:
            raise RuntimeError("fused GroupNorm: unsupported shape")
        z, mean, rstd = out
        ctx.save_for_backward(x, weight, bias, mean, rstd)
        ctx.params = (weight, bias)
        ctx.cfg = (int(groups), bool(silu))
        return z

    @staticmethod
    def backward(ctx, dz):
        x, weight, bias, mean, rstd = ctx.saved_tensors
        groups, silu = ctx.cfg
        gw, gb = gradsink.sink(ctx.params[0]), gradsink.sink(ctx.params[1])
        if gw is None or gb is None:
            gw = gb = None
        dx, dgamma, dbeta = ops.gn_backward(dz.contiguous(), x, weight, bias, mean, rstd, groups, silu, gw, gb)
        if gw is not None:
            dgamma = dbeta = None
        return dx, dgamma, dbeta, None, None, None


class _FusedGN16(FastFunction):

    @staticmethod
    def forward(ctx, x, weight, bias, groups, eps, silu):
        xn = x.contiguous(memory_format=torch.channels_last).permute(0, 2, 3, 1)
        y, mr, ab = ops.gn_bf16_forward(xn, weight, bias, groups, eps, silu)
        ctx.save_for_backward(xn, mr, ab)
        ctx.params = (weight, bias)
        ctx.cfg = (int(groups), bool(silu))
        return y.permute(0, 3, 1, 2)

    @staticmethod
    def backward(ctx, dy):
        xn, mr, ab = ctx.saved_tensors
        weight, bias = ctx.params
        groups, silu = ctx.cfg
        dyn = dy.to(torch.bfloat16).contiguous(memory_format=torch.channels_last).permute(0, 2, 3, 1)
        gw, gb = gradsink.sink(ctx.params[0]), gradsink.sink(ctx.params[1])
        sunk = gw is not None and gb is not None
        if not sunk:
            gw, gb = torch.empty_like(weight), torch.empty_like(bias)
        dx = ops.gn_bf16_backward(dyn, xn, weight, mr, ab, groups, silu, gw, gb, accumulate=sunk)
        return dx.permute(0, 3, 1, 2), (None if sunk else gw), (None if sunk else gb), None, None, None


_FUSED_GN = True


def enable_fused_gn(flag: bool) -> None:
    global _FUSED_GN
    _FUSED_GN = bool(flag)


def fused_gn_act(x: torch.Tensor, gn: nn.GroupNorm, silu: bool = True) -> torch.Tensor:
    hw = x.shape[2] * x.shape[3] if x.dim() == 4 else 0
    if (_FUSED_GN and type(gn) in _GN_TYPES and x.is_cuda and x.dtype == torch.bfloat16 and x.dim() == 4 and gn.affine
            and x.shape[1] % 8 == 0 and gn.weight.dtype == torch.float32):
        return _FusedGN16.apply(x, gn.weight, gn.bias, gn.num_groups, gn.eps, silu)
    if (_FUSED_GN and type(gn) in _GN_TYPES and x.is_cuda and x.dtype == torch.float32 and x.dim() == 4
            and gn.affine and hw >= 4 and (hw & (hw - 1)) == 0 and x.shape[1] // gn.num_groups <= 256
            and not torch.is_autocast_enabled()):
        return _FusedGN.apply(x.contiguous(), gn.weight, gn.bias, gn.num_groups, gn.eps, silu)
    y = gn(x)
    return y * torch.sigmoid(y) if silu else y


_GN_TYPES = {nn.GroupNorm}


def use_fused_bn(model: nn.Module, blocks: bool = True) -> int:
    from .Classification.models import resnet_cifar as R
    n = 0
    for mod in model.modules():
        if isinstance(mod, R.BasicBlock):
            mod.fused_bn = True
            mod.fused_block = bool(blocks)
            n += 2 + (1 if mod.downsample is not None else 0)
        elif isinstance(mod, R.ResNetCifar):
            mod.fused_bn = True
            n += 1
    return n
```

unlearn_saliency_amd/ops.py:

```python
from __future__ import annotations

import ctypes
from typing import Optional, Sequence

import torch

from .fastfn import FastFunction

from . import _lib, ringpack, weightimg
from ._lib import c_double, c_int, c_int64, c_size_t, c_uint64, c_void_p, check
from .streams import _stream, _stream_handle


def _dev(t: Optional[torch.Tensor], dtype: torch.dtype, name: str, allow_none: bool = False) -> c_void_p:
    if t is None:
        if allow_none:
            return c_void_p(None)
        raise ValueError(f"{name} must not be None")
    if not t.is_cuda:
        raise RuntimeError(f"{name}: the SalUn HIP kernels need a device tensor (got {t.device}); no CPU fallback")
    if t.dtype != dtype:
        raise TypeError(f"{name}: expected {dtype}, got {t.dtype}")
    if not t.is_contiguous():
        raise ValueError(f"{name} must be contiguous")
    return c_void_p(t.data_ptr())


_shape_memo: dict = {}


def _q(name: str, *args):
    key = (name,) + args
    v = _shape_memo.get(key)
    if v is None:
        fn = getattr(_lib.lib(), name)
        v = _shape_memo[key] = fn(*[c_int64(a) if t is c_int64 else a for a, t in zip(args, fn.argtypes)])
    return v


_ws: dict[tuple, torch.Tensor] = {}


def workspace(nbytes: int, device: torch.device, tag: str = "",
              stream: Optional[torch.cuda.Stream] = None) -> torch.Tensor:
    idx = device.index if device.index is not None else torch.cuda.current_device()
    key = (idx, None if tag == "topk" else _stream_handle(idx) if stream is None else stream.cuda_stream, tag)
    w = _ws.get(key)
    if w is None or w.numel() < nbytes:
        with torch.cuda.stream(stream):
            w = torch.empty(max(int(nbytes), 1 << 20), dtype=torch.uint8, device=device)
        _ws[key] = w
    return w


PARAM_EPOCH = weightimg.PARAM_EPOCH
PACK_CALLS = weightimg.BF16_LAUNCHES


def saliency_accumulate(acc: torch.Tensor, g: torch.Tensor, scale: float = 1.0,
                        sqnorm: Optional[torch.Tensor] = None, max_norm: float = 1.0) -> None:
    assert acc.numel() == g.numel()
    check(_lib.lib().salun_saliency_accumulate(_dev(acc, torch.float32, "acc"), _dev(g, torch.float32, "g"),
                                               c_double(scale), _dev(sqnorm, torch.float32, "sqnorm", True),
                                               c_double(max_norm), c_int64(acc.numel()), _stream()),
          "salun_saliency_accumulate")


class TopkFailed(RuntimeError):
    """The full-scan route's grid barrier timed out (its workgroups were not co-resident): the masks are garbage."""


def mask_topk(acc: torch.Tensor, ks: Sequence[int], out: Optional[Sequence[torch.Tensor]] = None,
              flags: int = 0, check: bool = False) -> list[torch.Tensor]:
    L = _lib.lib()
    n, nk = acc.numel(), len(ks)
    if not 1 <= nk <= _lib.SALUN_MAX_THRESHOLDS:
        raise ValueError(f"1 <= len(ks) <= {_lib.SALUN_MAX_THRESHOLDS}")
    values_only = bool(flags & _lib.SALUN_TOPK_VALUES_ONLY)
    if values_only:
        out, marr = [], None
    else:
        if out is None:
            n_pad = (n + 255) & ~255
            out = [r[:n] for r in torch.empty((nk, n_pad), dtype=torch.uint8, device=acc.device).unbind(0)]
        assert len(out) == nk and all(o.numel() == n for o in out)
        marr = (c_void_p * nk)(*[_dev(o, torch.uint8, "mask").value for o in out])
    nbytes = L.salun_mask_topk_workspace_bytes(c_int64(n), c_int(nk))
    ws = workspace(nbytes, acc.device, "topk")
    karr = (c_int64 * nk)(*[int(k) for k in ks])
    _lib.check(L.salun_mask_topk_ex(_dev(acc, torch.float32, "acc"), c_int64(n), karr, c_int(nk), marr,
                                    c_void_p(ws.data_ptr()), c_size_t(ws.numel()), ctypes.c_uint(flags), _stream()),
               "salun_mask_topk")
    if check:
        route, err = mask_topk_status(acc.device)
        from . import dist as sdist
        if sdist.collectives_on():
            flag = torch.tensor([int(err)], dtype=torch.int32, device=acc.device)
            torch.distributed.all_reduce(flag, op=torch.distributed.ReduceOp.MAX)
            err = int(flag.item())
        if err:
            raise TopkFailed(f"salun_mask_topk: the full scan's grid barrier timed out (route {route}, n = {n}): "
                             "its workgroups were not co-resident; no mask was produced")
    return list(out)


def mask_topk_status(device: torch.device) -> tuple[int, int]:
    ws = workspace(0, device, "topk")
    route, err = c_int(0), c_int(0)
    check(_lib.lib().salun_mask_topk_status(c_void_p(ws.data_ptr()), ctypes.byref(route), ctypes.byref(err), _stream()),
          "salun_mask_topk_status")
    return route.value, err.value


def mask_topk_thresholds(device: torch.device, nk: int) -> torch.Tensor:
    ws = workspace(0, device, "topk")
    out = torch.empty(nk, dtype=torch.float32, device=device)
    check(_lib.lib().salun_mask_topk_thresholds(c_void_p(ws.data_ptr()), c_int(nk), c_void_p(out.data_ptr()),
                                                _stream()), "salun_mask_topk_thresholds")
    return out


def mask_u8_to_i64(m: torch.Tensor) -> torch.Tensor:
    out = torch.empty(m.shape, dtype=torch.int64, device=m.device)
    check(_lib.lib().salun_mask_u8_to_i64(_dev(m, torch.uint8, "mask"), c_void_p(out.data_ptr()),
                                          c_int64(m.numel()), _stream()), "salun_mask_u8_to_i64")
    return out


def mask_i64_to_u8(m: torch.Tensor, out: Optional[torch.Tensor] = None) -> torch.Tensor:
    if out is None:
        out = torch.empty(m.shape, dtype=torch.uint8, device=m.device)
    check(_lib.lib().salun_mask_i64_to_u8(_dev(m, torch.int64, "mask"), _dev(out, torch.uint8, "out"),
                                          c_int64(m.numel()), _stream()), "salun_mask_i64_to_u8")
    return out


def mask_popcount(m: torch.Tensor) -> int:
    L = _lib.lib()
    ws = workspace(L.salun_reduce_workspace_bytes(c_int64(m.numel())), m.device)
    out = torch.empty(1, dtype=torch.int64, device=m.device)
    check(L.salun_mask_popcount(_dev(m, torch.uint8, "mask"), c_int64(m.numel()), c_void_p(out.data_ptr()),
                                c_void_p(ws.data_ptr()), c_size_t(ws.numel()), _stream()), "salun_mask_popcount")
    return int(out.item())


def masked_sgd_step(p: torch.Tensor, g: torch.Tensor, buf: Optional[torch.Tensor], m: Optional[torch.Tensor],
                    lr: float, momentum: float, weight_decay: float, first_step: bool) -> None:
    n = p.numel()
    assert g.numel() == n and (buf is None or buf.numel() == n) and (m is None or m.numel() == n)
    weightimg.params_written()
    check(_lib.lib().salun_masked_sgd_step(_dev(p, torch.float32, "p"), _dev(g, torch.float32, "g"),
                                           _dev(buf, torch.float32, "buf", True), _dev(m, torch.uint8, "mask", True),
                                           c_double(lr), c_double(momentum), c_double(weight_decay),
                                           c_int(int(first_step)), c_int64(n), _stream()), "salun_masked_sgd_step")


def grad_sqnorm(g: torch.Tensor, out: Optional[torch.Tensor] = None) -> torch.Tensor:
    L = _lib.lib()
    if out is None:
        out = torch.empty(1, dtype=torch.float32, device=g.device)
    ws = workspace(L.salun_reduce_workspace_bytes(c_int64(g.numel())), g.device)
    check(L.salun_grad_sqnorm(_dev(g, torch.float32, "g"), c_int64(g.numel()), _dev(out, torch.float32, "out"),
                              c_void_p(ws.data_ptr()), c_size_t(ws.numel()), _stream()), "salun_grad_sqnorm")
    return out


def masked_adam_step(p: torch.Tensor, g: torch.Tensor, m1: torch.Tensor, v: torch.Tensor,
                     mask: Optional[torch.Tensor], lr: float, beta1: float, beta2: float, eps: float,
                     weight_decay: float, step: int, sqnorm: Optional[torch.Tensor] = None,
                     max_norm: float = 1.0, gscale: float = 1.0) -> None:
    n = p.numel()
    assert g.numel() == n and m1.numel() == n and v.numel() == n and (mask is None or mask.numel() == n)
    weightimg.params_written()
    check(_lib.lib().salun_masked_adam_step(_dev(p, torch.float32, "p"), _dev(g, torch.float32, "g"),
                                            _dev(m1, torch.float32, "exp_avg"), _dev(v, torch.float32, "exp_avg_sq"),
                                            _dev(mask, torch.uint8, "mask", True),
                                            _dev(sqnorm, torch.float32, "sqnorm", True), c_double(max_norm),
                                            c_double(gscale), c_double(lr), c_double(beta1), c_double(beta2),
                                            c_double(eps), c_double(weight_decay), c_int(int(step)), c_int64(n),
                                            _stream()), "salun_masked_adam_step")


def adam_coefficients(step_dev: torch.Tensor, lr: float, beta1: float, beta2: float, coef: torch.Tensor) -> None:
    check(_lib.lib().salun_adam_coefficients(_dev(step_dev, torch.int64, "step"), c_double(lr), c_double(beta1),
                                             c_double(beta2), _dev(coef, torch.float32, "coef"), _stream()),
          "salun_adam_coefficients")


def masked_adam_step_coef(p, g, m1, v, mask, coef, beta1, beta2, eps, weight_decay, sqnorm=None, max_norm=1.0,
                          gscale=1.0) -> None:
    n = p.numel()
    weightimg.params_written()
    check(_lib.lib().salun_masked_adam_step_coef(_dev(p, torch.float32, "p"), _dev(g, torch.float32, "g"),
                                                 _dev(m1, torch.float32, "exp_avg"), _dev(v, torch.float32, "exp_avg_sq"),
                                                 _dev(mask, torch.uint8, "mask", True),
                                                 _dev(sqnorm, torch.float32, "sqnorm", True), c_double(max_norm),
                                                 c_double(gscale), _dev(coef, torch.float32, "coef"), c_double(beta1),
                                                 c_double(beta2), c_double(eps), c_double(weight_decay), c_int64(n),
                                                 _stream()), "salun_masked_adam_step_coef")


def adam_ema_step(p: torch.Tensor, g: torch.Tensor, m1: torch.Tensor, v: torch.Tensor, shadow: torch.Tensor,
                  mask: Optional[torch.Tensor], lr: float, beta1: float, beta2: float, eps: float, weight_decay: float,
                  mu: float, step: int, sqnorm: Optional[torch.Tensor] = None, max_norm: float = 1.0,
                  gscale: float = 1.0) -> None:
    n = p.numel()
    assert g.numel() == n and m1.numel() == n and v.numel() == n and shadow.numel() == n
    assert mask is None or mask.numel() == n
    weightimg.params_written()
    check(_lib.lib().salun_adam_ema_step(_dev(p, torch.float32, "p"), _dev(g, torch.float32, "g"),
                                         _dev(m1, torch.float32, "exp_avg"), _dev(v, torch.float32, "exp_avg_sq"),
                                         _dev(shadow, torch.float32, "shadow"), _dev(mask, torch.uint8, "mask", True),
                                         _dev(sqnorm, torch.float32, "sqnorm", True), c_double(max_norm),
                                         c_double(gscale), c_double(lr), c_double(beta1), c_double(beta2),
                                         c_double(eps), c_double(weight_decay), c_double(mu), c_int(int(step)),
                                         c_int64(n), _stream()), "salun_adam_ema_step")


def adam_ema_step_coef(p, g, m1, v, shadow, mask, coef, beta1, beta2, eps, weight_decay, mu, sqnorm=None, max_norm=1.0,
                       gscale=1.0) -> None:
    n = p.numel()
    assert g.numel() == n and m1.numel() == n and v.numel() == n and shadow.numel() == n
    assert mask is None or mask.numel() == n
    weightimg.params_written()
    check(_lib.lib().salun_adam_ema_step_coef(_dev(p, torch.float32, "p"), _dev(g, torch.float32, "g"),
                                              _dev(m1, torch.float32, "exp_avg"), _dev(v, torch.float32, "exp_avg_sq"),
                                              _dev(shadow, torch.float32, "shadow"),
                                              _dev(mask, torch.uint8, "mask", True),
                                              _dev(sqnorm, torch.float32, "sqnorm", True), c_double(max_norm),
                                              c_double(gscale), _dev(coef, torch.float32, "coef"), c_double(beta1),
                                              c_double(beta2), c_double(eps), c_double(weight_decay), c_double(mu),
                                              c_int64(n), _stream()), "salun_adam_ema_step_coef")


def qsample(x0: torch.Tensor, e: torch.Tensor, sqrt_ab: torch.Tensor, sqrt_1mab: torch.Tensor,
            t: torch.Tensor) -> torch.Tensor:
    B = x0.shape[0]
    chw = x0.numel() // max(B, 1)
    xt = torch.empty_like(x0)
    check(_lib.lib().salun_qsample(_dev(x0, torch.float32, "x0"), _dev(e, torch.float32, "e"),
                                   _dev(sqrt_ab, torch.float32, "sqrt_ab"), _dev(sqrt_1mab, torch.float32, "sqrt_1mab"),
                                   _dev(t, torch.int64, "t"), c_int64(sqrt_ab.numel()), c_void_p(xt.data_ptr()),
                                   c_int64(B), c_int64(chw), _stream()), "salun_qsample")
    return xt


def sqerr_loss(a: torch.Tensor, b: torch.Tensor, coef: float, want_per_sample: bool = False,
               want_grad: bool = True):
    L = _lib.lib()
    B = a.shape[0]
    chw = a.numel() // B
    loss = torch.empty(1, dtype=torch.float32, device=a.device)
    per = torch.empty(B, dtype=torch.float32, device=a.device) if want_per_sample else None
    d = torch.empty_like(b) if want_grad else None
    ws = workspace(L.salun_sqerr_workspace_bytes(c_int64(B), c_int64(chw)), a.device)
    check(L.salun_sqerr_loss(_dev(a, torch.float32, "a"), _dev(b, torch.float32, "b"), c_int64(B), c_int64(chw),
                             c_double(coef), c_void_p(loss.data_ptr()), _dev(per, torch.float32, "per_sample", True),
                             _dev(d, torch.float32, "dloss", True), c_void_p(ws.data_ptr()), c_size_t(ws.numel()),
                             _stream()), "salun_sqerr_loss")
    return loss, per, d


class _SqErr(FastFunction):

    @staticmethod
    def forward(ctx, target, pred, coef):
        loss, _, d = sqerr_loss(target.contiguous(), pred.contiguous(), coef, want_grad=True)
        ctx.save_for_backward(d)
        return loss.reshape(())

    @staticmethod
    def backward(ctx, grad_out):
        (d,) = ctx.saved_tensors
        return None, d * grad_out, None


def eps_mse(e: torch.Tensor, out: torch.Tensor) -> torch.Tensor:
    return _SqErr.apply(e, out, 1.0 / e.shape[0])


def mse_loss(target: torch.Tensor, pred: torch.Tensor) -> torch.Tensor:
    return _SqErr.apply(target, pred, 1.0 / target.numel())


def dropout(x: torch.Tensor, p: float, key: int, sample_offset: int = 0, out: Optional[torch.Tensor] = None,
            seed_dev: Optional[torch.Tensor] = None) -> torch.Tensor:
    n = x.shape[0]
    chw = x.numel() // max(n, 1)
    y = out if out is not None else torch.empty_like(x)
    check(_lib.lib().salun_dropout(_dev(x, torch.float32, "x"), _dev(y, torch.float32, "y"), c_int64(n), c_int64(chw),
                                   c_int64(sample_offset), c_double(p), c_uint64(key & 0xFFFFFFFFFFFFFFFF),
                                   _dev(seed_dev, torch.int64, "seed_dev", True), _stream()), "salun_dropout")
    return y


class _Dropout(FastFunction):
    @staticmethod
    def forward(ctx, x, p, key, offset):
        ctx.cfg = (float(p), int(key), int(offset))
        return dropout(x.contiguous(), p, key, offset)

    @staticmethod
    def backward(ctx, dy):
        p, key, offset = ctx.cfg
        return dropout(dy.contiguous(), p, key, offset), None, None, None


def dropout_fn(x: torch.Tensor, p: float, key: int, sample_offset: int = 0) -> torch.Tensor:
    return _Dropout.apply(x, float(p), int(key), int(sample_offset))


def fim_square_accumulate(F: torch.Tensor, tmp: torch.Tensor, n_data: float) -> None:
    check(_lib.lib().salun_fim_square_accumulate(_dev(F, torch.float32, "F"), _dev(tmp, torch.float32, "tmp"),
                                                 c_double(n_data), c_int64(F.numel()), _stream()),
          "salun_fim_square_accumulate")


def _data_ws_bytes(N: int, outC: int, outH: int, outW: int, R: int, conv_stride: int) -> int:
    return _q("salun_conv2d_data_workspace_bytes", N, outC, outH, outW, R, conv_stride)


def conv2d_forward(x: torch.Tensor, w: torch.Tensor, bias: Optional[torch.Tensor], stride: int, pad: int,
                   P: int, Q: int, nbias: Optional[torch.Tensor] = None,
                   addend: Optional[torch.Tensor] = None) -> Optional[torch.Tensor]:
    N, C, H, W = x.shape
    K, _, R, _ = w.shape
    if nbias is not None and tuple(nbias.shape) != (N, K):
        raise ValueError(f"nbias must be [{N}, {K}], got {tuple(nbias.shape)}")
    if addend is not None and tuple(addend.shape) != (N, K, P, Q):
        raise ValueError(f"addend must be {(N, K, P, Q)}, got {tuple(addend.shape)}")
    if R == 3 and stride == 1 and pad == 1 and P == H and Q == W:
        imgs = ringpack.images(w)
        if imgs is not None:
            y = conv3x3_packed(x, imgs[0], K, bias=bias, nbias=nbias, addend=addend)
            if y is not None:
                return y
    y = torch.empty((N, K, P, Q), dtype=torch.float32, device=x.device)
    L = _lib.lib()
    wsb = _data_ws_bytes(N, K, P, Q, R, stride)
    ws = workspace(wsb, x.device) if wsb else None
    rc = L.salun_conv2d_forward_fused(_dev(x, torch.float32, "x"), _dev(w, torch.float32, "w"),
                                      _dev(bias, torch.float32, "bias", True),
                                      _dev(nbias, torch.float32, "nbias", True),
                                      _dev(addend, torch.float32, "addend", True), c_void_p(y.data_ptr()),
                                      N, C, H, W, K, R, stride, pad, P, Q,
                                      c_void_p(ws.data_ptr() if ws is not None else None), c_size_t(wsb), _stream())
    if rc == _lib.SALUN_EINVAL:
        return None
    check(rc, "salun_conv2d_forward_fused")
    return y


def conv2d_backward_data(dy: torch.Tensor, w: torch.Tensor, x_shape, stride: int, pad: int,
                         addend: Optional[torch.Tensor] = None) -> Optional[torch.Tensor]:
    N, C, H, W = x_shape
    K, _, R, _ = w.shape
    P, Q = dy.shape[2], dy.shape[3]
    if R == 3 and stride == 1 and pad == 1 and P == H and Q == W:
        imgs = ringpack.images(w)
        if imgs is not None:
            dx = conv3x3_packed(dy, imgs[1], C, addend=addend)
            if dx is not None:
                return dx
    dx = torch.empty((N, C, H, W), dtype=torch.float32, device=dy.device)
    L = _lib.lib()
    wsb = _data_ws_bytes(N, C, H, W, R, 1) if stride == 1 else 0
    ws = workspace(wsb, dy.device) if wsb else None
    rc = L.salun_conv2d_backward_data_ws(_dev(dy, torch.float32, "dy"), _dev(w, torch.float32, "w"),
                                         _dev(addend, torch.float32, "addend", True),
                                         c_void_p(dx.data_ptr()), N, C, H, W, K, R, stride, pad, P, Q,
                                         c_void_p(ws.data_ptr() if ws is not None else None), c_size_t(wsb), _stream())
    if rc == _lib.SALUN_EINVAL:
        return None
    check(rc, "salun_conv2d_backward_data")
    return dx


WGRAD_KERNEL = [None]


def conv2d_backward_weight(x: torch.Tensor, dy: torch.Tensor, w_shape, stride: int, pad: int,
                           out: Optional[torch.Tensor] = None, accumulate: bool = False,
                           shared: bool = False, stream: Optional[torch.cuda.Stream] = None) -> Optional[torch.Tensor]:
    N, C, H, W = x.shape
    K, _, R, _ = w_shape
    P, Q = dy.shape[2], dy.shape[3]
    L = _lib.lib()
    nbytes = L.salun_conv2d_wgrad_workspace_bytes(N, C, K, R, P, Q)
    if nbytes == 0:
        return None
    ws = workspace(nbytes, x.device, stream=stream)
    dw = out if out is not None else torch.empty(tuple(w_shape), dtype=torch.float32, device=x.device)
    rc = L.salun_conv2d_backward_weight_ex(_dev(x, torch.float32, "x"), _dev(dy, torch.float32, "dy"),
                                           _dev(dw, torch.float32, "dw"), N, C, H, W, K, R, stride, pad, P, Q,
                                           int(bool(accumulate and out is not None)),
                                           _lib.SALUN_WGRAD_SHARED if (shared if WGRAD_KERNEL[0] is None
                                                                       else WGRAD_KERNEL[0] == "shared") else 0,
                                           c_void_p(ws.data_ptr()), c_size_t(ws.numel()),
                                           c_void_p(_stream_handle() if stream is None else stream.cuda_stream))
    if rc == _lib.SALUN_EINVAL:
        return None
    check(rc, "salun_conv2d_backward_weight")
    return dw


def conv3x3_pack(w: torch.Tensor, dgrad: bool, out: Optional[torch.Tensor] = None) -> Optional[torch.Tensor]:
    K, C = w.shape[0], w.shape[1]
    L = _lib.lib()
    nbytes = int(L.salun_conv3x3_pack_bytes(K, C, int(dgrad)))
    if nbytes == 0 or tuple(w.shape[2:]) != (3, 3):
        return None
    img = out if out is not None and out.numel() * 4 == nbytes else torch.empty(nbytes // 4, dtype=torch.float32,
                                                                                device=w.device)
    _dev(w, torch.float32, "w")
    job = _lib.PackJob(w.data_ptr(), None if dgrad else img.data_ptr(), img.data_ptr() if dgrad else None, K, C)
    check(L.salun_conv3x3_pack_weights(ctypes.cast(ctypes.pointer(job), c_void_p), 1, _stream()),
          "salun_conv3x3_pack_weights")
    return img


def conv3x3_packed(x: torch.Tensor, img: torch.Tensor, Kout: int, bias: Optional[torch.Tensor] = None,
                   nbias: Optional[torch.Tensor] = None, addend: Optional[torch.Tensor] = None,
                   out: Optional[torch.Tensor] = None, cfg: int = 0) -> Optional[torch.Tensor]:
    N, Cred, H, W = x.shape
    y = out if out is not None else torch.empty((N, Kout, H, W), dtype=torch.float32, device=x.device)
    rc = _lib.lib().salun_conv3x3_packed(_dev(x, torch.float32, "x"), c_void_p(img.data_ptr()),
                                         _dev(bias, torch.float32, "bias", True),
                                         _dev(nbias, torch.float32, "nbias", True),
                                         _dev(addend, torch.float32, "addend", True), c_void_p(y.data_ptr()),
                                         N, Cred, H, W, Kout, int(cfg), _stream())
    if rc == _lib.SALUN_EINVAL:
        return None
    check(rc, "salun_conv3x3_packed")
    return y


def channel_sum(dy: torch.Tensor, out: Optional[torch.Tensor] = None, accumulate: bool = False) -> torch.Tensor:
    N, K = dy.shape[0], dy.shape[1]
    HW = dy.shape[2] * dy.shape[3]
    L = _lib.lib()
    ws = workspace(L.salun_channel_sum_workspace_bytes(N, K), dy.device)
    res = out if out is not None else torch.empty(K, dtype=torch.float32, device=dy.device)
    check(L.salun_channel_sum(_dev(dy, torch.float32, "dy"), _dev(res, torch.float32, "out"), N, K, HW,
                              int(bool(accumulate and out is not None)), c_void_p(ws.data_ptr()), c_size_t(ws.numel()),
                              _stream()), "salun_channel_sum")
    return res


def conv2d_bf16_supported(C: int, K: int, R: int, stride: int, pad: int) -> bool:
    return bool(_q("salun_conv2d_bf16_supported", C, K, R, stride, pad))


def conv2d_bf16_pack(w: torch.Tensor, out: Optional[torch.Tensor] = None) -> torch.Tensor:
    K, C, R, _ = w.shape
    if out is None:
        out = torch.empty((K, R * R, C), dtype=torch.bfloat16, device=w.device)
    check(_lib.lib().salun_conv2d_bf16_pack_weights(_dev(w, torch.float32, "w"), _dev(out, torch.bfloat16, "wp"), K, C, R,
                                                    _stream()), "salun_conv2d_bf16_pack_weights")
    return out


def bf16_pack_batch(jobs) -> int:
    jobs = list(jobs)
    if not jobs:
        return 0
    L, st, cap = _lib.lib(), _stream(), _lib.SALUN_BF16_PACK_MAX_JOBS
    launches = 0
    for i in range(0, len(jobs), cap):
        part = jobs[i:i + cap]
        arr = (_lib.Bf16PackJob * len(part))()
        for a, (w, wp, K, C, R, tr) in zip(arr, part):
            _dev(w, torch.float32, "w")
            _dev(wp, torch.bfloat16, "wp")
            a.w, a.wp, a.K, a.C, a.R, a.transposed = w.data_ptr(), wp.data_ptr(), K, C, R, int(bool(tr))
        check(L.salun_bf16_pack_weights_batch(ctypes.cast(arr, c_void_p), len(part), st), "salun_bf16_pack_weights_batch")
        launches += 1
    return launches


def conv2d_bf16_forward(x: torch.Tensor, wp: torch.Tensor, R: int, stride: int, pad: int,
                        bias: Optional[torch.Tensor] = None, nbias: Optional[torch.Tensor] = None,
                        addend: Optional[torch.Tensor] = None) -> torch.Tensor:
    N, H, W, C = x.shape
    K = wp.shape[0]
    OH, OW = (H + 2 * pad - R) // stride + 1, (W + 2 * pad - R) // stride + 1
    _dev(x, torch.bfloat16, "x")
    y = torch.empty((N, OH, OW, K), dtype=torch.bfloat16, device=x.device)
    ws = workspace(_q("salun_conv2d_bf16_data_workspace_bytes", N, H, W, C, K, R, stride, pad), x.device)
    check(_lib.lib().salun_conv2d_bf16_forward(_dev(x, torch.bfloat16, "x"), _dev(wp, torch.bfloat16, "wp"),
                                               _dev(bias, torch.float32, "bias", True),
                                               _dev(nbias, torch.float32, "nbias", True),
                                               _dev(addend, torch.bfloat16, "addend", True), c_void_p(y.data_ptr()),
                                               N, H, W, C, K, R, stride, pad, c_void_p(ws.data_ptr()),
                                               c_size_t(ws.numel()), _stream()), "salun_conv2d_bf16_forward")
    return y


def conv2d_bf16_backward_data(dy: torch.Tensor, wp: torch.Tensor, x_shape, R: int, stride: int, pad: int,
                              addend: Optional[torch.Tensor] = None) -> torch.Tensor:
    N, H, W, C = x_shape
    K = wp.shape[0]
    _dev(dy, torch.bfloat16, "dy")
    dx = torch.empty((N, H, W, C), dtype=torch.bfloat16, device=dy.device)
    ws = workspace(_q("salun_conv2d_bf16_data_workspace_bytes", N, H, W, C, K, R, stride, pad), dy.device)
    check(_lib.lib().salun_conv2d_bf16_backward_data(_dev(dy, torch.bfloat16, "dy"), _dev(wp, torch.bfloat16, "wp"),
                                                     _dev(addend, torch.bfloat16, "addend", True),
                                                     c_void_p(dx.data_ptr()), N, H, W, C, K, R, stride, pad,
                                                     c_void_p(ws.data_ptr()), c_size_t(ws.numel()), _stream()),
          "salun_conv2d_bf16_backward_data")
    return dx


def conv2d_bf16_backward_weight(x: torch.Tensor, dy: torch.Tensor, w_shape, stride: int, pad: int,
                                out: Optional[torch.Tensor] = None, accumulate: bool = False,
                                bias_out: Optional[torch.Tensor] = None,
                                nbias_out: Optional[torch.Tensor] = None,
                                stream: Optional[torch.cuda.Stream] = None) -> torch.Tensor:
    N, H, W, C = x.shape
    K, _, R, _ = w_shape
    L = _lib.lib()
    nbytes = _q("salun_conv2d_bf16_wgrad_workspace_bytes", N, H, W, C, K, R, stride, pad)
    if nbytes == 0:
        raise ValueError(f"bf16 backward-weight: unsupported shape C={C} K={K} R={R} stride={stride} pad={pad}")
    ws = workspace(nbytes, x.device, stream=stream)
    dw = out if out is not None else torch.empty(tuple(w_shape), dtype=torch.float32, device=x.device)
    if nbias_out is not None and tuple(nbias_out.shape) != (N, K):
        raise ValueError(f"nbias_out must be [{N}, {K}]")
    check(L.salun_conv2d_bf16_backward_weight_ex(_dev(x, torch.bfloat16, "x"), _dev(dy, torch.bfloat16, "dy"),
                                                 _dev(dw, torch.float32, "dw"), _dev(bias_out, torch.float32, "db", True),
                                                 _dev(nbias_out, torch.float32, "dnb", True),
                                                 N, H, W, C, K, R, stride, pad, int(bool(accumulate and out is not None)),
                                                 c_void_p(ws.data_ptr()), c_size_t(ws.numel()),
                                                 c_void_p(_stream_handle() if stream is None else stream.cuda_stream)),
          "salun_conv2d_bf16_backward_weight_ex")
    return dw


def colsum_bf16(dy: torch.Tensor, images: int, bias_out: Optional[torch.Tensor] = None,
                nbias_out: Optional[torch.Tensor] = None, accumulate: bool = False) -> None:
    K = dy.shape[-1]
    M = dy.numel() // K
    ws = workspace(_q("salun_colsum_bf16_workspace_bytes", K), dy.device)
    check(_lib.lib().salun_colsum_bf16(_dev(dy, torch.bfloat16, "dy"), _dev(bias_out, torch.float32, "db", True),
                                       _dev(nbias_out, torch.float32, "dnb", True), c_int64(M), K, int(images),
                                       int(bool(accumulate)), c_void_p(ws.data_ptr()), c_size_t(ws.numel()), _stream()),
          "salun_colsum_bf16")


def gemm_bf16_supported(M: int, N: int, K: int) -> bool:
    return bool(_q("salun_gemm_bf16_supported", int(M), int(N), int(K)))


def gemm_bf16_nt(x: torch.Tensor, w: torch.Tensor, bias: Optional[torch.Tensor] = None,
                 addend: Optional[torch.Tensor] = None, variant: int = 0) -> torch.Tensor:
    M, K = x.shape
    N = w.shape[0]
    assert w.shape[1] == K
    y = torch.empty((M, N), dtype=torch.bfloat16, device=x.device)
    check(_lib.lib().salun_gemm_bf16_nt(_dev(x, torch.bfloat16, "x"), _dev(w, torch.bfloat16, "w"),
                                        _dev(bias, torch.float32, "bias", True), _dev(addend, torch.bfloat16, "addend", True),
                                        c_void_p(y.data_ptr()), c_int64(M), N, K, int(variant), _stream()),
          "salun_gemm_bf16_nt")
    return y


def gemm_bf16_tn_supported(M: int, Na: int, Nb: int) -> bool:
    return bool(_lib.lib().salun_gemm_bf16_tn_supported(c_int64(M), int(Na), int(Nb)))


def gemm_bf16_tn(dy: torch.Tensor, x: torch.Tensor, out: Optional[torch.Tensor] = None, accumulate: bool = False,
                 variant: int = 0) -> torch.Tensor:
    M, Na = dy.shape
    Nb = x.shape[1]
    assert x.shape[0] == M
    L = _lib.lib()
    if not L.salun_gemm_bf16_tn_supported(c_int64(M), Na, Nb):
        raise ValueError(f"gemm_bf16_tn: unsupported shape M={M} Na={Na} Nb={Nb}")
    nbytes = L.salun_gemm_bf16_tn_workspace_bytes(c_int64(M), Na, Nb, int(variant))
    ws = workspace(nbytes, x.device) if nbytes else None
    dw = out if out is not None else torch.empty((Na, Nb), dtype=torch.float32, device=x.device)
    check(L.salun_gemm_bf16_tn(_dev(dy, torch.bfloat16, "dy"), _dev(x, torch.bfloat16, "x"), _dev(dw, torch.float32, "dw"),
                               c_int64(M), Na, Nb, int(bool(accumulate and out is not None)), int(variant),
                               c_void_p(ws.data_ptr() if ws is not None else None), c_size_t(nbytes), _stream()),
          "salun_gemm_bf16_tn")
    return dw


def pack_bf16(w: torch.Tensor, transposed: bool = False, out: Optional[torch.Tensor] = None) -> torch.Tensor:
    N, K = w.shape
    if out is None:
        out = torch.empty((K, N) if transposed else (N, K), dtype=torch.bfloat16, device=w.device)
    check(_lib.lib().salun_pack_bf16(_dev(w, torch.float32, "w"), _dev(out, torch.bfloat16, "wp"), N, K, int(bool(transposed)),
                                     _stream()), "salun_pack_bf16")
    return out


def gn_bf16_forward(x: torch.Tensor, gamma: torch.Tensor, beta: torch.Tensor, groups: int, eps: float, silu: bool):
    N, H, W, C = x.shape
    L = _lib.lib()
    ws = workspace(_q("salun_gn_bf16_workspace_bytes", N, C, H * W, groups), x.device)
    y = torch.empty_like(x)
    mr = torch.empty((N, groups, 2), dtype=torch.float32, device=x.device)
    ab = torch.empty((N, C, 2), dtype=torch.float32, device=x.device)
    check(L.salun_gn_bf16_forward(_dev(x, torch.bfloat16, "x"), _dev(gamma, torch.float32, "gamma"),
                                  _dev(beta, torch.float32, "beta"), c_void_p(y.data_ptr()), c_void_p(mr.data_ptr()),
                                  c_void_p(ab.data_ptr()), N, C, H * W, groups, c_double(eps), int(bool(silu)),
                                  c_void_p(ws.data_ptr()), c_size_t(ws.numel()), _stream()), "salun_gn_bf16_forward")
    return y, mr, ab


def gn_bf16_backward(dy: torch.Tensor, x: torch.Tensor, gamma: torch.Tensor, mr: torch.Tensor, ab: torch.Tensor,
                     groups: int, silu: bool, dgamma: torch.Tensor, dbeta: torch.Tensor, accumulate: bool) -> torch.Tensor:
    N, H, W, C = x.shape
    L = _lib.lib()
    ws = workspace(_q("salun_gn_bf16_workspace_bytes", N, C, H * W, groups), x.device)
    dx = torch.empty_like(x)
    check(L.salun_gn_bf16_backward(_dev(dy, torch.bfloat16, "dy"), _dev(x, torch.bfloat16, "x"),
                                   _dev(gamma, torch.float32, "gamma"), _dev(mr, torch.float32, "mr"),
                                   _dev(ab, torch.float32, "ab"), c_void_p(dx.data_ptr()),
                                   _dev(dgamma, torch.float32, "dgamma"), _dev(dbeta, torch.float32, "dbeta"), N, C, H * W,
                                   groups, int(bool(silu)), int(bool(accumulate)), c_void_p(ws.data_ptr()),
                                   c_size_t(ws.numel()), _stream()), "salun_gn_bf16_backward")
    return dx


def attn_supported(D: int) -> bool:
    return bool(_q("salun_attn_supported", int(D)))


def _tok_view(t: torch.Tensor, name: str):
    if not t.is_cuda or t.dtype != torch.bfloat16 or t.dim() != 4:
        raise TypeError(f"{name}: expected a 4-D bfloat16 device tensor [B, tokens, H, D]")
    B, N, H, D = t.shape
    if t.stride(3) != 1 or (H > 1 and t.stride(2) != D):
        raise ValueError(f"{name}: heads must be adjacent runs of D contiguous channels")
    return c_void_p(t.data_ptr()), ctypes.c_longlong(t.stride(0) if B > 1 else N * t.stride(1)), c_int(t.stride(1))


def attn_forward(q: torch.Tensor, k: torch.Tensor, v: torch.Tensor, scale: float, need_lse: bool = True):
    B, Nq, H, D = q.shape
    Nk = k.shape[1]
    o = torch.empty((B, Nq, H, D), dtype=torch.bfloat16, device=q.device)
    lse = torch.empty((B * H, Nq), dtype=torch.float32, device=q.device) if need_lse else None
    qp, qb, ql = _tok_view(q, "q")
    kp, kb, kl = _tok_view(k, "k")
    vp, vb, vl = _tok_view(v, "v")
    op, ob, ol = _tok_view(o, "o")
    check(_lib.lib().salun_attn_forward(qp, kp, vp, op, c_void_p(lse.data_ptr() if need_lse else None), B, H, Nq, Nk, D,
                                        qb, ql, kb, kl, vb, vl, ob, ol, c_double(scale), _stream()), "salun_attn_forward")
    return o, lse


def attn_backward(q, k, v, o, d_o, lse, scale: float):
    B, Nq, H, D = q.shape
    Nk = k.shape[1]
    dq = torch.empty((B, Nq, H, D), dtype=torch.bfloat16, device=q.device)
    dk = torch.empty((B, Nk, H, D), dtype=torch.bfloat16, device=q.device)
    dv = torch.empty((B, Nk, H, D), dtype=torch.bfloat16, device=q.device)
    dsum = torch.empty((B * H, Nq), dtype=torch.float32, device=q.device)
    qp, qb, ql = _tok_view(q, "q")
    kp, kb, kl = _tok_view(k, "k")
    vp, vb, vl = _tok_view(v, "v")
    op, ob, ol = _tok_view(o, "o")
    dp, db, dl = _tok_view(d_o, "d_o")
    check(_lib.lib().salun_attn_backward(qp, kp, vp, op, dp, _dev(lse, torch.float32, "lse"), c_void_p(dq.data_ptr()),
                                         c_void_p(dk.data_ptr()), c_void_p(dv.data_ptr()), c_void_p(dsum.data_ptr()),
                                         B, H, Nq, Nk, D, qb, ql, kb, kl, vb, vl, ob, ol, db, dl, c_double(scale), _stream()),
          "salun_attn_backward")
    return dq, dk, dv


class _Attn(FastFunction):
    @staticmethod
    def forward(ctx, q, k, v, scale):
        o, lse = attn_forward(q, k, v, scale, need_lse=True)
        ctx.save_for_backward(q, k, v, o, lse)
        ctx.scale = float(scale)
        return o

    @staticmethod
    def backward(ctx, d_o):
        q, k, v, o, lse = ctx.saved_tensors
        if d_o.stride(3) != 1 or d_o.stride(2) != d_o.shape[3]:
            d_o = d_o.contiguous()
        dq, dk, dv = attn_backward(q, k, v, o, d_o.to(torch.bfloat16), lse, ctx.scale)
        return dq, dk, dv, None


def attention(q: torch.Tensor, k: torch.Tensor, v: torch.Tensor, scale: float) -> torch.Tensor:
    return _Attn.apply(q, k, v, float(scale))


class _LayerNorm16(FastFunction):

    @staticmethod
    def forward(ctx, x, weight, bias, eps):
        C = x.shape[-1]
        xc = x.contiguous()
        rows = xc.numel() // C
        y = torch.empty_like(xc)
        stats = torch.empty((rows, 2), dtype=torch.float32, device=x.device)
        check(_lib.lib().salun_ln_bf16_forward(_dev(xc, torch.bfloat16, "x"), _dev(weight, torch.float32, "gamma"),
                                               _dev(bias, torch.float32, "beta"), c_void_p(y.data_ptr()),
                                               c_void_p(stats.data_ptr()), c_int64(rows), C, c_double(eps), _stream()),
              "salun_ln_bf16_forward")
        ctx.save_for_backward(xc, stats)
        ctx.params = (weight, bias)
        return y

    @staticmethod
    def backward(ctx, dy):
        from . import gradsink
        xc, stats = ctx.saved_tensors
        weight, bias = ctx.params
        C = xc.shape[-1]
        rows = xc.numel() // C
        dyc = dy.to(torch.bfloat16).contiguous()
        L = _lib.lib()
        ws = workspace(_q("salun_ln_bf16_workspace_bytes", rows, C), xc.device)
        gw, gb = gradsink.sink(ctx.params[0]), gradsink.sink(ctx.params[1])
        sunk = gw is not None and gb is not None
        if not sunk:
            gw, gb = torch.empty_like(weight), torch.empty_like(bias)
        dx = torch.empty_like(xc)
        check(L.salun_ln_bf16_backward(_dev(dyc, torch.bfloat16, "dy"), _dev(xc, torch.bfloat16, "x"),
                                       _dev(weight, torch.float32, "gamma"), _dev(stats, torch.float32, "stats"),
                                       c_void_p(dx.data_ptr()), _dev(gw, torch.float32, "dgamma"),
                                       _dev(gb, torch.float32, "dbeta"), c_int64(rows), C, int(sunk),
                                       c_void_p(ws.data_ptr()), c_size_t(ws.numel()), _stream()), "salun_ln_bf16_backward")
        return dx, (None if sunk else gw), (None if sunk else gb), None


def layer_norm_bf16(x: torch.Tensor, ln: "torch.nn.LayerNorm") -> torch.Tensor:
    return _LayerNorm16.apply(x, ln.weight, ln.bias, float(ln.eps))


class _Geglu16(FastFunction):

    @staticmethod
    def forward(ctx, h):
        hc = h.contiguous()
        F2 = hc.shape[-1]
        rows = hc.numel() // F2
        out = torch.empty(hc.shape[:-1] + (F2 // 2,), dtype=torch.bfloat16, device=h.device)
        check(_lib.lib().salun_geglu_bf16_forward(_dev(hc, torch.bfloat16, "h"), c_void_p(out.data_ptr()), c_int64(rows),
                                                  F2 // 2, _stream()), "salun_geglu_bf16_forward")
        ctx.save_for_backward(hc)
        return out

    @staticmethod
    def backward(ctx, dy):
        (hc,) = ctx.saved_tensors
        F2 = hc.shape[-1]
        rows = hc.numel() // F2
        dyc = dy.to(torch.bfloat16).contiguous()
        dh = torch.empty_like(hc)
        check(_lib.lib().salun_geglu_bf16_backward(_dev(hc, torch.bfloat16, "h"), _dev(dyc, torch.bfloat16, "dy"),
                                                   c_void_p(dh.data_ptr()), c_int64(rows), F2 // 2, _stream()),
              "salun_geglu_bf16_backward")
        return dh


def geglu_bf16(h: torch.Tensor) -> torch.Tensor:
    return _Geglu16.apply(h)


def bn_forward(x, res, gamma, beta, running_mean, running_var, training, momentum, eps, relu,
               num_batches_tracked=None):
    N, C, H, W = x.shape
    L = _lib.lib()
    y = torch.empty_like(x)
    mean = torch.empty(C, dtype=torch.float32, device=x.device)
    invstd = torch.empty(C, dtype=torch.float32, device=x.device)
    ws = workspace(L.salun_bn_workspace_bytes(C), x.device)
    rc = L.salun_bn_forward(_dev(x, torch.float32, "x"), _dev(res, torch.float32, "res", True), c_void_p(y.data_ptr()),
                            _dev(gamma, torch.float32, "weight"), _dev(beta, torch.float32, "bias"),
                            _dev(running_mean, torch.float32, "running_mean", True),
                            _dev(running_var, torch.float32, "running_var", True),
                            _dev(num_batches_tracked, torch.int64, "num_batches_tracked", True),
                            c_void_p(mean.data_ptr()),
                            c_void_p(invstd.data_ptr()), N, C, H * W, int(bool(training)), c_double(momentum),
                            c_double(eps), int(bool(relu)), c_void_p(ws.data_ptr()), c_size_t(ws.numel()), _stream())
    if rc == _lib.SALUN_EINVAL:
        return None
    check(rc, "salun_bn_forward")
    return y, mean, invstd


def bn_backward(dy, y, x, gamma, mean, invstd, training, relu, want_dres, gamma_grad_acc=None, beta_grad_acc=None):
    N, C, H, W = x.shape
    L = _lib.lib()
    dx = torch.empty_like(x)
    dres = torch.empty_like(x) if want_dres else None
    dgamma = torch.empty(C, dtype=torch.float32, device=x.device)
    dbeta = torch.empty(C, dtype=torch.float32, device=x.device)
    ws = workspace(L.salun_bn_workspace_bytes(C), x.device)
    check(L.salun_bn_backward(_dev(dy, torch.float32, "dy"), _dev(y, torch.float32, "y", True),
                              _dev(x, torch.float32, "x"), _dev(gamma, torch.float32, "weight"),
                              _dev(mean, torch.float32, "mean"), _dev(invstd, torch.float32, "invstd"),
                              c_void_p(dx.data_ptr()), _dev(dres, torch.float32, "dres", True),
                              c_void_p(dgamma.data_ptr()), c_void_p(dbeta.data_ptr()),
                              _dev(gamma_grad_acc, torch.float32, "gamma.grad", True),
                              _dev(beta_grad_acc, torch.float32, "beta.grad", True), N, C, H * W,
                              int(bool(training)), int(bool(relu)), c_void_p(ws.data_ptr()), c_size_t(ws.numel()),
                              _stream()), "salun_bn_backward")
    return dx, dres, dgamma, dbeta


def gn_forward(x, gamma, beta, groups, eps, silu):
    N, C, H, W = x.shape
    z = torch.empty_like(x)
    mean = torch.empty(N * groups, dtype=torch.float32, device=x.device)
    rstd = torch.empty(N * groups, dtype=torch.float32, device=x.device)
    rc = _lib.lib().salun_gn_forward(_dev(x, torch.float32, "x"), c_void_p(z.data_ptr()),
                                     _dev(gamma, torch.float32, "weight"), _dev(beta, torch.float32, "bias"),
                                     c_void_p(mean.data_ptr()), c_void_p(rstd.data_ptr()), N, C, H * W, int(groups),
                                     c_double(eps), int(bool(silu)), _stream())
    if rc == _lib.SALUN_EINVAL:
        return None
    check(rc, "salun_gn_forward")
    return z, mean, rstd


def gn_backward(dz, x, gamma, beta, mean, rstd, groups, silu, gamma_grad_acc=None, beta_grad_acc=None, addend=None,
                nk_sum: bool = False, csum: bool = False, csum_acc=None):
    N, C, H, W = x.shape
    L = _lib.lib()
    dx = torch.empty_like(x)
    dgamma = torch.empty(C, dtype=torch.float32, device=x.device)
    dbeta = torch.empty(C, dtype=torch.float32, device=x.device)
    ws = workspace(L.salun_gn_workspace_bytes(N, C), x.device)
    if addend is not None and addend.shape != x.shape:
        raise ValueError("gn_backward: addend must have the shape of x")
    want_nk = bool(nk_sum or csum or csum_acc is not None)
    nk = torch.empty((N, C), dtype=torch.float32, device=x.device) if want_nk else None
    cs = torch.empty(C, dtype=torch.float32, device=x.device) if csum else None
    check(L.salun_gn_backward_fused(_dev(dz, torch.float32, "dz"), _dev(x, torch.float32, "x"),
                                    _dev(gamma, torch.float32, "weight"), _dev(beta, torch.float32, "bias"),
                                    _dev(mean, torch.float32, "mean"), _dev(rstd, torch.float32, "rstd"),
                                    _dev(addend, torch.float32, "addend", True),
                                    c_void_p(dx.data_ptr()), c_void_p(dgamma.data_ptr()), c_void_p(dbeta.data_ptr()),
                                    _dev(gamma_grad_acc, torch.float32, "weight.grad", True),
                                    _dev(beta_grad_acc, torch.float32, "bias.grad", True),
                                    _dev(nk, torch.float32, "nk_sum", True), _dev(cs, torch.float32, "csum", True),
                                    _dev(csum_acc, torch.float32, "csum_acc", True), N, C, H * W, int(groups),
                                    int(bool(silu)), c_void_p(ws.data_ptr()), c_size_t(ws.numel()), _stream()),
          "salun_gn_backward_fused")
    if want_nk:
        return dx, dgamma, dbeta, nk, cs
    return dx, dgamma, dbeta


def proximal_step(p: torch.Tensor, p0: torch.Tensor, ratio: int, scratch: Optional[torch.Tensor] = None,
                  scratch_mask: Optional[torch.Tensor] = None) -> torch.Tensor:
    weightimg.params_written()
    n = p.numel()
    if ratio < 1:
        raise IndexError("index -1 is out of bounds for dimension 0 with size 0")
    if ratio > n:
        raise RuntimeError("selected index k out of range")
    L = _lib.lib()
    d = scratch if scratch is not None else torch.empty(n, dtype=torch.float32, device=p.device)
    check(L.salun_param_diff(_dev(p, torch.float32, "p"), _dev(p0, torch.float32, "p0"), _dev(d, torch.float32, "d"),
                             c_int64(n), _stream()), "salun_param_diff")
    mask_topk(d, [n - ratio + 1], flags=_lib.SALUN_TOPK_VALUES_ONLY)
    tau = mask_topk_thresholds(p.device, 1)
    check(L.salun_soft_threshold_step(_dev(p, torch.float32, "p"), _dev(p0, torch.float32, "p0"),
                                      c_void_p(tau.data_ptr()), c_int64(n), _stream()), "salun_soft_threshold_step")
    return tau


def ewc_penalty_grad(p: torch.Tensor, p_star: torch.Tensor, F: torch.Tensor, g: torch.Tensor, lam: float
                     ) -> torch.Tensor:
    n = p.numel()
    L = _lib.lib()
    out = torch.empty(2, dtype=torch.float32, device=p.device)
    ws = workspace(L.salun_ewc_workspace_bytes(c_int64(n)), p.device)
    check(L.salun_ewc_penalty_grad(_dev(p, torch.float32, "p"), _dev(p_star, torch.float32, "p_star"),
                                   _dev(F, torch.float32, "F"), _dev(g, torch.float32, "g"), c_double(lam),
                                   c_void_p(out.data_ptr()), c_int64(n), c_void_p(ws.data_ptr()),
                                   c_size_t(ws.numel()), _stream()), "salun_ewc_penalty_grad")
    return out


def image_batch(data: torch.Tensor, idx: torch.Tensor, crop: Optional[torch.Tensor] = None,
                flip: Optional[torch.Tensor] = None, pad: int = 4, out: Optional[torch.Tensor] = None) -> torch.Tensor:
    num, H, W, C = data.shape
    B = idx.numel()
    if out is None:
        out = torch.empty((B, C, H, W), dtype=torch.float32, device=data.device)
    check(_lib.lib().salun_image_batch(_dev(data, torch.uint8, "data"), _dev(idx, torch.int64, "idx"),
                                       _dev(crop, torch.int32, "crop", True), _dev(flip, torch.uint8, "flip", True),
                                       c_void_p(out.data_ptr()), c_int64(B), c_int(H), c_int(W), c_int(C), c_int(pad),
                                       _stream()), "salun_image_batch")
    return out


def fill_uniform(n: int, seed: int, lo: float = 0.0, hi: float = 1.0, device="cuda") -> torch.Tensor:
    out = torch.empty(n, dtype=torch.float32, device=device)
    check(_lib.lib().salun_fill_uniform(c_void_p(out.data_ptr()), c_int64(n), c_uint64(seed), c_double(lo),
                                        c_double(hi), _stream()), "salun_fill_uniform")
    return out


def fill_normal(n: int, seed: int, mean: float = 0.0, std: float = 1.0, device="cuda") -> torch.Tensor:
    out = torch.empty(n, dtype=torch.float32, device=device)
    check(_lib.lib().salun_fill_normal(c_void_p(out.data_ptr()), c_int64(n), c_uint64(seed), c_double(mean),
                                       c_double(std), _stream()), "salun_fill_normal")
    return out


def fill_u8(n: int, seed: int, device="cuda") -> torch.Tensor:
    out = torch.empty(n, dtype=torch.uint8, device=device)
    check(_lib.lib().salun_fill_u8(c_void_p(out.data_ptr()), c_int64(n), c_uint64(seed), _stream()), "salun_fill_u8")
    return out
```

unlearn_saliency_amd/resblock.py:

```python
from __future__ import annotations

import torch

from .fastfn import FastFunction
import torch.nn as nn

import os

from . import dist as sdist
from . import draws, gradsink, ops, wgrad_side

FWD_SHORTCUT_BESIDE = os.environ.get("SALUN_FWD_SHORTCUT_BESIDE", "1") != "0"


def _bn_args(bn: nn.BatchNorm2d):
    return bn.running_mean, bn.running_var, bn.training, bn.momentum, bn.eps


class _BasicBlockFn(FastFunction):
    @staticmethod
    def forward(ctx, x, blk, w1, g1, b1, w2, g2, b2, wd, gd, bd):
        s = blk.conv1.stride[0]
        N, C, H, W = x.shape
        P, Q = (H + 2 - 3) // s + 1, (W + 2 - 3) // s + 1
        training = blk.bn1.training
        cd = md = idd = None
        fork = None
        if wd is not None:
            def shortcut():
                cd_ = ops.conv2d_forward(x, wd, None, s, 0, P, Q)
                return (cd_,) + tuple(ops.bn_forward(cd_, None, gd, bd, *_bn_args(blk.downsample[1]), False,
                                                     blk.downsample[1].num_batches_tracked))
            if (FWD_SHORTCUT_BESIDE and wgrad_side.OVERLAP and x.is_cuda
                    and not torch.cuda.is_current_stream_capturing()):
                main, fork = torch.cuda.current_stream(x.device), wgrad_side.stream(x.device)
                fork.wait_stream(main)
                with torch.cuda.stream(fork):
                    cd, skip, md, idd = shortcut()
                x.record_stream(fork)
        c1 = ops.conv2d_forward(x, w1, None, s, 1, P, Q)
        y1, m1, i1 = ops.bn_forward(c1, None, g1, b1, *_bn_args(blk.bn1), True, blk.bn1.num_batches_tracked)
        c2 = ops.conv2d_forward(y1, w2, None, 1, 1, P, Q)
        if wd is None:
            skip = x
        elif fork is None:
            cd, skip, md, idd = shortcut()
        else:
            main.wait_stream(fork)
            for t in (cd, skip, md, idd):
                if t is not None:
                    t.record_stream(main)
        out, m2, i2 = ops.bn_forward(c2, skip, g2, b2, *_bn_args(blk.bn2), True, blk.bn2.num_batches_tracked)
        ctx.save_for_backward(x, c1, y1, c2, out, cd, w1, g1, b1, w2, g2, b2, wd, gd, bd, m1, i1, m2, i2, md, idd)
        ctx.cfg = (s, training)
        return out

    @staticmethod
    def backward(ctx, dout):
        x, c1, y1, c2, out, cd, w1, g1, b1, w2, g2, b2, wd, gd, bd, m1, i1, m2, i2, md, idd = ctx.saved_tensors
        s, training = ctx.cfg
        dout = dout.contiguous()
        grads = {}

        def bn_bwd(dy, y, xin, g, b, m, i, relu, want_dres):
            gw, gb = gradsink.sink(g), gradsink.sink(b)
            if gw is None or gb is None:
                gw = gb = None
            dx, dres, dg, db = ops.bn_backward(dy, y, xin, g, m, i, training, relu, want_dres, gw, gb)
            if gw is not None:
                gradsink.arrived(g)
                gradsink.arrived(b)
                dg = db = None
            return dx, dres, dg, db

        dev = dout.device
        overlap = wgrad_side.OVERLAP

        def wgrad(xin, dy, w, stride, pad):
            dst = gradsink.sink(w)
            if overlap:
                dw = wgrad_side.beside(dev, (xin, dy), lambda side: ops.conv2d_backward_weight(
                    xin, dy, w.shape, stride, pad, out=dst, accumulate=True, shared=True, stream=side), alloc=dst is None)
            else:
                dw = ops.conv2d_backward_weight(xin, dy, w.shape, stride, pad, out=dst, accumulate=True)
            if dst is not None:
                gradsink.arrived(w)
                return None
            return dw

        dc2, dskip, dg2, db2 = bn_bwd(dout, out, c2, g2, b2, m2, i2, True, True)
        dwd = dgd = dbd = None
        dxd = dskip
        if wd is not None:
            dcd, _, dgd, dbd = bn_bwd(dskip, None, cd, gd, bd, md, idd, False, False)
            dwd = wgrad(x, dcd, wd, s, 0)
            dxd = ops.conv2d_backward_data(dcd, wd, x.shape, s, 0) if ctx.needs_input_grad[0] else None
        dw2 = wgrad(y1, dc2, w2, 1, 1)
        dy1 = ops.conv2d_backward_data(dc2, w2, y1.shape, 1, 1)
        dc1, _, dg1, db1 = bn_bwd(dy1, y1, c1, g1, b1, m1, i1, True, False)
        dw1 = wgrad(x, dc1, w1, s, 1)
        dx = ops.conv2d_backward_data(dc1, w1, x.shape, s, 1, addend=dxd) if ctx.needs_input_grad[0] else None
        if overlap and not all(g is None for g in (dw1, dw2, dwd)):
            torch.cuda.current_stream(dev).wait_stream(wgrad_side.stream(dev))
            wgrad_side.release_held(dev)
        return dx, None, dw1, dg1, db1, dw2, dg2, db2, dwd, dgd, dbd


def _probe(blk, shape, device) -> bool:
    N, C, H, W = shape
    s = blk.conv1.stride[0]
    P, Q = (H + 2 - 3) // s + 1, (W + 2 - 3) // s + 1
    K = blk.conv1.out_channels
    if (P * Q) % 4 or (H * W) % 4:
        return False
    e = lambda *sh: torch.empty(sh, dtype=torch.float32, device=device)
    x, y1, dy = e(N, C, H, W), e(N, K, P, Q), e(N, K, P, Q)
    convs = [(x, blk.conv1.weight, s, 1), (y1, blk.conv2.weight, 1, 1)]
    if blk.downsample is not None:
        convs.append((x, blk.downsample[0].weight, s, 0))
    for xin, w, st, pad in convs:
        if ops.conv2d_forward(xin, w, None, st, pad, P, Q) is None:
            return False
        if ops.conv2d_backward_data(dy, w, xin.shape, st, pad, addend=xin) is None:
            return False
        if ops.conv2d_backward_weight(xin, dy, w.shape, st, pad) is None:
            return False
    return True


def _structure_ok(blk) -> bool:
    convs = [blk.conv1, blk.conv2] + ([blk.downsample[0]] if blk.downsample is not None else [])
    bns = [blk.bn1, blk.bn2] + ([blk.downsample[1]] if blk.downsample is not None else [])
    if any(type(b) is not nn.BatchNorm2d or not b.affine or not b.track_running_stats or b.momentum is None
           for b in bns):
        return False
    if any(c.bias is not None or c.groups != 1 or c.dilation != (1, 1) or c.weight.dtype != torch.float32
           for c in convs):
        return False
    if len({b.training for b in bns}) != 1:
        return False
    c1, c2 = blk.conv1, blk.conv2
    ok = (c1.kernel_size == (3, 3) and c1.padding == (1, 1) and c1.stride[0] == c1.stride[1] and c1.stride[0] in (1, 2)
          and c2.kernel_size == (3, 3) and c2.padding == (1, 1) and c2.stride == (1, 1))
    if blk.downsample is not None:
        d = blk.downsample[0]
        ok = ok and d.kernel_size == (1, 1) and d.padding == (0, 0) and d.stride == c1.stride
    else:
        ok = ok and c1.stride == (1, 1) and c1.in_channels == c1.out_channels
    return ok


def fused_basic_block(blk, x: torch.Tensor):
    if not (x.is_cuda and x.dtype == torch.float32 and x.dim() == 4) or torch.is_autocast_enabled():
        return None
    cache = blk.__dict__.setdefault("_fused_shapes", {})
    key = (tuple(x.shape), x.device)
    ok = cache.get(key)
    if ok is None:
        with torch.no_grad():
            ok = cache[key] = _structure_ok(blk) and _probe(blk, tuple(x.shape), x.device)
    if not ok or not _structure_ok(blk):
        return None
    x = x.contiguous()
    d = blk.downsample
    return _BasicBlockFn.apply(x, blk, blk.conv1.weight, blk.bn1.weight, blk.bn1.bias, blk.conv2.weight,
                               blk.bn2.weight, blk.bn2.bias, d[0].weight if d is not None else None,
                               d[1].weight if d is not None else None, d[1].bias if d is not None else None)


class _DiffusionResnetBlockFn(FastFunction):
    @staticmethod
    def forward(ctx, x, proj, blk, n1w, n1b, w1, b1, n2w, n2b, w2, b2, ws, bs):
        N, C, H, W = x.shape
        G1, G2 = blk.norm1.num_groups, blk.norm2.num_groups
        a1, m1, r1 = ops.gn_forward(x, n1w, n1b, G1, blk.norm1.eps, True)
        c1 = ops.conv2d_forward(a1, w1, b1, 1, 1, H, W, nbias=proj)
        a2, m2, r2 = ops.gn_forward(c1, n2w, n2b, G2, blk.norm2.eps, True)
        p = float(blk.dropout.p) if blk.dropout.training else 0.0
        dkey = None
        if p > 0.0:
            dkey = draws.dropout_key()
            a2 = ops.dropout(a2, p, dkey[0], dkey[1], out=a2)
        if ws is not None:
            sc = ops.conv2d_forward(x, ws, bs, 1, (ws.shape[2] - 1) // 2, H, W)
        else:
            sc = x
        out = ops.conv2d_forward(a2, w2, b2, 1, 1, H, W, addend=sc)
        ctx.save_for_backward(x, a1, c1, a2, n1w, n1b, w1, b1, n2w, n2b, w2, b2, ws, bs, m1, r1, m2, r2)
        ctx.cfg = (G1, G2, p, dkey)
        return out

    @staticmethod
    def backward(ctx, dout):
        x, a1, c1, a2, n1w, n1b, w1, b1, n2w, n2b, w2, b2, ws, bs, m1, r1, m2, r2 = ctx.saved_tensors
        G1, G2, p, dkey = ctx.cfg
        dout = dout.contiguous()
        dev = dout.device
        overlap = wgrad_side.OVERLAP
        returned = []

        def wgrad(xin, dy, w, pad):
            dst = gradsink.sink(w)
            if overlap:
                dw = wgrad_side.beside(dev, (xin, dy), lambda side: ops.conv2d_backward_weight(
                    xin, dy, w.shape, 1, pad, out=dst, accumulate=True, shared=True, stream=side), alloc=dst is None)
            else:
                dw = ops.conv2d_backward_weight(xin, dy, w.shape, 1, pad, out=dst, accumulate=True)
            if dst is not None:
                gradsink.arrived(w)
                return None
            returned.append(dw)
            return dw

        def gn_sinks(g, b):
            gw, gb = gradsink.sink(g), gradsink.sink(b)
            return (gw, gb) if gw is not None and gb is not None else (None, None)

        db2 = dbs = None
        s2, ss = gradsink.sink(b2), (gradsink.sink(bs) if bs is not None else None)
        if bs is None and s2 is not None:
            ops.channel_sum(dout, out=s2, accumulate=True)
        else:
            csum = ops.channel_sum(dout)
            if s2 is not None:
                s2.add_(csum)
            else:
                db2 = csum
            if bs is not None:
                if ss is not None:
                    ss.add_(csum)
                else:
                    dbs = csum.clone() if db2 is csum else csum
        dw2 = wgrad(a2, dout, w2, 1)
        da2 = ops.conv2d_backward_data(dout, w2, a2.shape, 1, 1)
        if dkey is not None:
            da2 = ops.dropout(da2, p, dkey[0], dkey[1], out=da2)
        gw, gb = gn_sinks(n2w, n2b)
        s1 = gradsink.sink(b1)
        dc1, dg2, dbt2, nk, cs = ops.gn_backward(da2, c1, n2w, n2b, m2, r2, G2, True, gw, gb, nk_sum=True,
                                                 csum=s1 is None, csum_acc=s1)
        if gw is not None:
            dg2 = dbt2 = None
        db1 = cs
        dproj = nk if ctx.needs_input_grad[1] else None
        dw1 = wgrad(a1, dc1, w1, 1)
        da1 = ops.conv2d_backward_data(dc1, w1, a1.shape, 1, 1)
        gw, gb = gn_sinks(n1w, n1b)
        dws = None
        if ws is None:
            dx, dg1, dbt1 = ops.gn_backward(da1, x, n1w, n1b, m1, r1, G1, True, gw, gb, addend=dout)
        else:
            pad = (ws.shape[2] - 1) // 2
            dws = wgrad(x, dout, ws, pad)
            dxg, dg1, dbt1 = ops.gn_backward(da1, x, n1w, n1b, m1, r1, G1, True, gw, gb)
            dx = ops.conv2d_backward_data(dout, ws, x.shape, 1, pad, addend=dxg)
        if gw is not None:
            dg1 = dbt1 = None
        if overlap and returned:
            torch.cuda.current_stream(dev).wait_stream(wgrad_side.stream(dev))
            wgrad_side.release_held(dev)
        if not ctx.needs_input_grad[0]:
            dx = None
        return dx, dproj, None, dg1, dbt1, dw1, db1, dg2, dbt2, dw2, db2, dws, dbs


def _diffusion_block_structure_ok(blk) -> bool:
    convs = [blk.conv1, blk.conv2]
    skip = getattr(blk, "conv_shortcut", None) if blk.use_conv_shortcut else getattr(blk, "nin_shortcut", None)
    if blk.in_channels != blk.out_channels:
        if skip is None:
            return False
        convs.append(skip)
    if any(type(n) is not nn.GroupNorm or not n.affine or n.weight.dtype != torch.float32
           for n in (blk.norm1, blk.norm2)):
        return False
    for c in convs:
        if (c.bias is None or c.groups != 1 or c.dilation != (1, 1) or c.stride != (1, 1)
                or c.padding_mode != "zeros" or c.weight.dtype != torch.float32):
            return False
    ok = all(c.kernel_size == (3, 3) and c.padding == (1, 1) for c in (blk.conv1, blk.conv2))
    if len(convs) == 3:
        k = convs[2].kernel_size
        ok = ok and k in ((1, 1), (3, 3)) and convs[2].padding == ((k[0] - 1) // 2,) * 2
    return ok and type(blk.dropout) is draws.CounterDropout and 0.0 <= blk.dropout.p < 1.0 and not blk.dropout.inplace


def _diffusion_block_probe(blk, shape, device) -> bool:
    N, C, H, W = shape
    K = blk.out_channels
    hw = H * W
    if hw < 4 or hw & (hw - 1) or C // blk.norm1.num_groups > 256 or K // blk.norm2.num_groups > 256:
        return False
    e = lambda *sh: torch.empty(sh, dtype=torch.float32, device=device)
    x, h, proj = e(N, C, H, W), e(N, K, H, W), e(N, K)
    try:
        for t, n in ((x, blk.norm1), (h, blk.norm2)):
            z, m, r = ops.gn_forward(t, n.weight, n.bias, n.num_groups, n.eps, True)
            ops.gn_backward(z, t, n.weight, n.bias, m, r, n.num_groups, True, addend=t, nk_sum=True)
    except Exception:
        return False
    convs = [(x, blk.conv1), (h, blk.conv2)]
    if C != K:
        convs.append((x, blk.conv_shortcut if blk.use_conv_shortcut else blk.nin_shortcut))
    for xin, c in convs:
        pad = c.padding[0]
        if ops.conv2d_forward(xin, c.weight, c.bias, 1, pad, H, W, nbias=proj, addend=h) is None:
            return False
        if ops.conv2d_backward_data(h, c.weight, xin.shape, 1, pad, addend=xin) is None:
            return False
        if ops.conv2d_backward_weight(xin, h, c.weight.shape, 1, pad) is None:
            return False
    return True


def fused_diffusion_resnet_block(blk, x: torch.Tensor, emb_act: torch.Tensor, proj: torch.Tensor = None):
    from . import norm
    if not (x.is_cuda and x.dtype == torch.float32 and x.dim() == 4) or torch.is_autocast_enabled() or not norm._FUSED_GN:
        return None
    cache = blk.__dict__.setdefault("_fused_shapes", {})
    key = (tuple(x.shape), x.device)
    ok = cache.get(key)
    if ok is None:
        with torch.no_grad():
            ok = cache[key] = _diffusion_block_structure_ok(blk) and _diffusion_block_probe(blk, tuple(x.shape), x.device)
    if not ok or not _diffusion_block_structure_ok(blk):
        return None
    if proj is None:
        proj = blk.temb_cemb_proj(emb_act)
    if proj.dtype != torch.float32 or tuple(proj.shape) != (x.shape[0], blk.out_channels):
        return None
    skip = None
    if blk.in_channels != blk.out_channels:
        skip = blk.conv_shortcut if blk.use_conv_shortcut else blk.nin_shortcut
    return _DiffusionResnetBlockFn.apply(x.contiguous(), proj.contiguous(), blk, blk.norm1.weight, blk.norm1.bias,
                                         blk.conv1.weight, blk.conv1.bias, blk.norm2.weight, blk.norm2.bias,
                                         blk.conv2.weight, blk.conv2.bias,
                                         skip.weight if skip is not None else None,
                                         skip.bias if skip is not None else None)
```

Baseline: 117.9.

## Recompute BN ReLU mask from x in backward instead of reading saved y

For BN+ReLU layers without a residual, the backward now rebuilds the ReLU mask by re-evaluating the affine transform on x with gamma and beta, so it no longer has to read the saved output y. This removes one full activation read per element in the backward partial and apply kernels. The standalone BN autograd path also stops saving y in that case, which lowers activation memory. It also adds a register-resident BN route, but that route is disabled by default (BN_RR_AUTO=false). The risk is mask mismatches where the recomputed pre-activation rounds differently near zero, so the code uses explicit _rn intrinsics to keep forward and backward arithmetic consistent.

After: 118.9 (median of 6 runs). No clear change (+0.8%).

```diff
diff --git a/include/salun.h b/include/salun.h
--- a/include/salun.h
+++ b/include/salun.h
@@ -197,6 +197,9 @@
 int salun_geglu_bf16_backward(const uint16_t *h , const uint16_t *dy , uint16_t *dh , int64_t rows,
                               int F, salun_stream_t stream);
 
+#define SALUN_BN_ROUTE_AUTO 0
+#define SALUN_BN_ROUTE_TWO_PASS 1
+#define SALUN_BN_ROUTE_REGISTER 2
 size_t salun_bn_workspace_bytes(int C);
 int salun_bn_forward(const float *x , const float *res , float *y ,
                      const float *gamma , const float *beta , float *running_mean ,
@@ -210,6 +213,19 @@
                       float *grad_gamma_acc , float *grad_beta_acc ,
                       int N, int C, int HW, int training, int relu, void *ws , size_t ws_bytes,
                       salun_stream_t stream);
+int salun_bn_forward_ex(const float *x , const float *res , float *y ,
+                        const float *gamma , const float *beta , float *running_mean ,
+                        float *running_var , long long *num_batches_tracked ,
+                        float *save_mean , float *save_invstd ,
+                        int N, int C, int HW, int training, double momentum, double eps, int relu, int route,
+                        void *ws , size_t ws_bytes, salun_stream_t stream);
+int salun_bn_backward_ex(const float *dy , const float *y ,
+                         const float *x , const float *gamma , const float *save_mean ,
+                         const float *save_invstd , float *dx , float *dres ,
+                         float *dgamma , float *dbeta , float *grad_gamma_acc ,
+                         float *grad_beta_acc , int N, int C, int HW, int training, int relu,
+                         const float *beta , int route, void *ws , size_t ws_bytes,
+                         salun_stream_t stream);
 
 size_t salun_gn_workspace_bytes(int N, int C);
 int salun_gn_forward(const float *x , float *y , const float *gamma , const float *beta ,
diff --git a/unlearn_saliency_amd/_lib.py b/unlearn_saliency_amd/_lib.py
--- a/unlearn_saliency_amd/_lib.py
+++ b/unlearn_saliency_amd/_lib.py
@@ -16,6 +16,7 @@
 SALUN_TOPK_FORCE_FULL_SCAN = 1
 SALUN_TOPK_VALUES_ONLY = 2
 SALUN_WGRAD_SHARED = 1
+SALUN_BN_ROUTE_AUTO, SALUN_BN_ROUTE_TWO_PASS, SALUN_BN_ROUTE_REGISTER = 0, 1, 2
 
 c_void_p, c_int, c_int64, c_uint64 = ctypes.c_void_p, ctypes.c_int, ctypes.c_int64, ctypes.c_uint64
 c_double, c_size_t = ctypes.c_double, ctypes.c_size_t
@@ -124,6 +125,9 @@
     "salun_bn_workspace_bytes": (c_size_t, [c_int]),
     "salun_bn_forward": (c_int, [c_void_p] * 10 + [c_int] * 4 + [c_double, c_double, c_int, c_void_p, c_size_t, c_void_p]),
     "salun_bn_backward": (c_int, [c_void_p] * 12 + [c_int] * 5 + [c_void_p, c_size_t, c_void_p]),
+    "salun_bn_forward_ex": (c_int, [c_void_p] * 10 + [c_int] * 4 + [c_double, c_double, c_int, c_int, c_void_p, c_size_t,
+                                                                   c_void_p]),
+    "salun_bn_backward_ex": (c_int, [c_void_p] * 12 + [c_int] * 5 + [c_void_p, c_int, c_void_p, c_size_t, c_void_p]),
     "salun_conv2d_backward_data_add": (c_int, [c_void_p] * 4 + [c_int] * 10 + [c_void_p]),
     "salun_gn_workspace_bytes": (c_size_t, [c_int, c_int]),
     "salun_gn_forward": (c_int, [c_void_p] * 6 + [c_int] * 4 + [c_double, c_int, c_void_p]),
diff --git a/unlearn_saliency_amd/csrc/salun_norm.hip b/unlearn_saliency_amd/csrc/salun_norm.hip
--- a/unlearn_saliency_amd/csrc/salun_norm.hip
+++ b/unlearn_saliency_amd/csrc/salun_norm.hip
@@ -3,6 +3,11 @@
 namespace {
 
 constexpr int BN_MAX_SPLIT = 64;
+constexpr int BN_RR_MAX_ITEMS = 16;
+constexpr int BN_RR_MIN_C = 128;
+constexpr bool BN_RR_AUTO = false;
+
+enum { BN_MASK_NONE = 0, BN_MASK_Y = 1, BN_MASK_X = 2 };
 
 
 struct BnWalk {
@@ -20,6 +25,62 @@
     if (i >= hw4) { i -= hw4; ++n; }
   }
 };
+
+__device__ __forceinline__ void bn_affine(float mean, float invstd, float gamma, float beta, float &a, float &b) {
+  a = __fmul_rn(invstd, gamma);
+  b = __fsub_rn(beta, __fmul_rn(mean, a));
+}
+__device__ __forceinline__ float bn_eval(float x, float a, float b) { return __fadd_rn(__fmul_rn(x, a), b); }
+
+__device__ __forceinline__ void bn_stats_item(const float4 &v, float &s1, float &s2) {
+  s1 += (v.x + v.y) + (v.z + v.w);
+  s2 += (v.x * v.x + v.y * v.y) + (v.z * v.z + v.w * v.w);
+}
+
+template <bool RELU, bool RES>
+__device__ __forceinline__ float4 bn_apply_item(const float4 &v, const float4 &r, float a, float b) {
+  float4 o;
+  o.x = bn_eval(v.x, a, b); o.y = bn_eval(v.y, a, b); o.z = bn_eval(v.z, a, b); o.w = bn_eval(v.w, a, b);
+  if (RES) { o.x += r.x; o.y += r.y; o.z += r.z; o.w += r.w; }
+  if (RELU) {
+    o.x = o.x > 0.f ? o.x : 0.f; o.y = o.y > 0.f ? o.y : 0.f;
+    o.z = o.z > 0.f ? o.z : 0.f; o.w = o.w > 0.f ? o.w : 0.f;
+  }
+  return o;
+}
+
+template <int MASK>
+__device__ __forceinline__ float4 bn_masked(float4 g, const float4 &xv, const float4 &yv, float a, float b) {
+  if (MASK == BN_MASK_Y) {
+    g.x = yv.x > 0.f ? g.x : 0.f; g.y = yv.y > 0.f ? g.y : 0.f;
+    g.z = yv.z > 0.f ? g.z : 0.f; g.w = yv.w > 0.f ? g.w : 0.f;
+  } else if (MASK == BN_MASK_X) {
+    g.x = bn_eval(xv.x, a, b) > 0.f ? g.x : 0.f; g.y = bn_eval(xv.y, a, b) > 0.f ? g.y : 0.f;
+    g.z = bn_eval(xv.z, a, b) > 0.f ? g.z : 0.f; g.w = bn_eval(xv.w, a, b) > 0.f ? g.w : 0.f;
+  }
+  return g;
+}
+
+__device__ __forceinline__ void bn_bwd_item(const float4 &g, const float4 &xv, float mu, float is, float &s1,
+                                            float &s2) {
+  s1 += (g.x + g.y) + (g.z + g.w);
+  s2 += (g.x * ((xv.x - mu) * is) + g.y * ((xv.y - mu) * is)) + (g.z * ((xv.z - mu) * is) + g.w * ((xv.w - mu) * is));
+}
+
+template <bool TRAIN>
+__device__ __forceinline__ float4 bn_dx_item(const float4 &g, const float4 &xv, float gi, float kb, float kg, float mu,
+                                             float is) {
+  float4 o;
+  if (TRAIN) {
+    o.x = gi * (g.x - (kb + ((xv.x - mu) * is) * kg));
+    o.y = gi * (g.y - (kb + ((xv.y - mu) * is) * kg));
+    o.z = gi * (g.z - (kb + ((xv.z - mu) * is) * kg));
+    o.w = gi * (g.w - (kb + ((xv.w - mu) * is) * kg));
+  } else {
+    o.x = gi * g.x; o.y = gi * g.y; o.z = gi * g.z; o.w = gi * g.w;
+  }
+  return o;
+}
 
 __global__ __launch_bounds__(256) void k_bn_stats_partial(const float *__restrict__ x, int N, int C, int HW, int nsplit,
                                                           double *__restrict__ partial) {
@@ -36,8 +97,7 @@
   for (int e = threadIdx.x; e < work; e += 256, ++it, wk.next()) {
     const int n = wk.n, i = wk.i;
     const float4 v = reinterpret_cast<const float4 *>(x + ((size_t)n * C + c) * HW)[i];
-    s1 += (v.x + v.y) + (v.z + v.w);
-    s2 += (v.x * v.x + v.y * v.y) + (v.z * v.z + v.w * v.w);
+    bn_stats_item(v, s1, s2);
     if ((it & 7) == 7) { d1 += s1; d2 += s2; s1 = 0.f; s2 = 0.f; }
   }
   d1 += s1; d2 += s2;
@@ -49,15 +109,15 @@
   }
 }
 
-__device__ __forceinline__ void bn_channel_stats(const double *__restrict__ partial, int c, int nsplit, double M,
+__device__ __forceinline__ void bn_channel_stats(const double *__restrict__ part, int c, int nsplit, double M,
                                                  float eps, float *s_out , bool publish,
                                                  float momentum, float *__restrict__ mean, float *__restrict__ invstd,
                                                  float *__restrict__ running_mean, float *__restrict__ running_var) {
   if (threadIdx.x < 64) {
     double s1 = 0.0, s2 = 0.0;
     if ((int)threadIdx.x < nsplit) {
-      s1 = partial[((size_t)c * nsplit + threadIdx.x) * 2 + 0];
-      s2 = partial[((size_t)c * nsplit + threadIdx.x) * 2 + 1];
+      s1 = part[threadIdx.x * 2 + 0];
+      s2 = part[threadIdx.x * 2 + 1];
     }
     s1 = salun_wave_sum(s1);
     s2 = salun_wave_sum(s2);
@@ -82,6 +142,25 @@
   __syncthreads();
 }
 
+template <bool TRAIN>
+__device__ __forceinline__ void bn_fwd_stats(const double *__restrict__ part, int c, int nsplit, double M, float eps,
+                                             float *st, bool publish, float momentum, float *__restrict__ mean,
+                                             float *__restrict__ invstd, float *__restrict__ running_mean,
+                                             float *__restrict__ running_var,
+                                             long long *__restrict__ num_batches_tracked) {
+  if (TRAIN) {
+    if (num_batches_tracked && c == 0 && publish && threadIdx.x == 0) *num_batches_tracked += 1;
+    bn_channel_stats(part, c, nsplit, M, eps, st, publish, momentum, mean, invstd, running_mean, running_var);
+  } else {
+    if (threadIdx.x == 0) {
+      st[0] = running_mean[c];
+      st[1] = 1.0f / sqrtf(running_var[c] + eps);
+      if (publish) { mean[c] = st[0]; invstd[c] = st[1]; }
+    }
+    __syncthreads();
+  }
+}
+
 template <bool RELU, bool RES, bool TRAIN>
 __global__ __launch_bounds__(256) void k_bn_apply(const float *__restrict__ x, const float *__restrict__ res,
                                                   float *__restrict__ y, const double *__restrict__ partial,
@@ -92,20 +171,10 @@
                                                   int nsplit, float eps, float momentum) {
   __shared__ float st[2];
   const int c = blockIdx.x, s = blockIdx.y;
-  if (TRAIN) {
-    if (num_batches_tracked && c == 0 && s == 0 && threadIdx.x == 0) *num_batches_tracked += 1;
-    bn_channel_stats(partial, c, nsplit, (double)N * HW, eps, st, s == 0, momentum, mean, invstd, running_mean,
-                     running_var);
-  } else {
-    if (threadIdx.x == 0) {
-      st[0] = running_mean[c];
-      st[1] = 1.0f / sqrtf(running_var[c] + eps);
-      if (s == 0) { mean[c] = st[0]; invstd[c] = st[1]; }
-    }
-    __syncthreads();
-  }
-  const float a = st[1] * gamma[c];
-  const float b = beta[c] - st[0] * a;
+  bn_fwd_stats<TRAIN>(partial + (size_t)c * nsplit * 2, c, nsplit, (double)N * HW, eps, st, s == 0, momentum, mean,
+                      invstd, running_mean, running_var, num_batches_tracked);
+  float a, b;
+  bn_affine(st[0], st[1], gamma[c], beta[c], a, b);
   const int n_lo = (int)((int64_t)N * s / nsplit), n_hi = (int)((int64_t)N * (s + 1) / nsplit);
   const int hw4 = HW >> 2;
   const int work = (n_hi - n_lo) * hw4;
@@ -115,29 +184,25 @@
     const int n = wk.n, i = wk.i;
     const size_t off = ((size_t)n * C + c) * HW;
     const float4 v = reinterpret_cast<const float4 *>(x + off)[i];
-    float4 o;
-    o.x = v.x * a + b; o.y = v.y * a + b; o.z = v.z * a + b; o.w = v.w * a + b;
-    if (RES) {
-      const float4 r = reinterpret_cast<const float4 *>(res + off)[i];
-      o.x += r.x; o.y += r.y; o.z += r.z; o.w += r.w;
-    }
-    if (RELU) {
-      o.x = o.x > 0.f ? o.x : 0.f; o.y = o.y > 0.f ? o.y : 0.f;
-      o.z = o.z > 0.f ? o.z : 0.f; o.w = o.w > 0.f ? o.w : 0.f;
-    }
-    reinterpret_cast<float4 *>(y + off)[i] = o;
-  }
-}
-
-template <bool RELU>
+    float4 r = v;
+    if (RES) r = reinterpret_cast<const float4 *>(res + off)[i];
+    reinterpret_cast<float4 *>(y + off)[i] = bn_apply_item<RELU, RES>(v, r, a, b);
+  }
+}
+
+template <int MASK>
 __global__ __launch_bounds__(256) void k_bn_bwd_partial(const float *__restrict__ dy, const float *__restrict__ y,
                                                         const float *__restrict__ x, const float *__restrict__ mean,
-                                                        const float *__restrict__ invstd, int N, int C, int HW,
+                                                        const float *__restrict__ invstd,
+                                                        const float *__restrict__ gamma,
+                                                        const float *__restrict__ beta, int N, int C, int HW,
                                                         int nsplit, double *__restrict__ partial) {
   __shared__ double lds[4];
   const int c = blockIdx.x, s = blockIdx.y;
   const int n_lo = (int)((int64_t)N * s / nsplit), n_hi = (int)((int64_t)N * (s + 1) / nsplit);
   const float mu = mean[c], is = invstd[c];
+  float a = 0.f, b = 0.f;
+  if (MASK == BN_MASK_X) bn_affine(mu, is, gamma[c], beta[c], a, b);
   float s1 = 0.f, s2 = 0.f;
   double d1 = 0.0, d2 = 0.0;
   const int hw4 = HW >> 2;
@@ -150,13 +215,10 @@
     const size_t off = ((size_t)n * C + c) * HW;
     float4 g = reinterpret_cast<const float4 *>(dy + off)[i];
     const float4 xv = reinterpret_cast<const float4 *>(x + off)[i];
-    if (RELU) {
-      const float4 yv = reinterpret_cast<const float4 *>(y + off)[i];
-      g.x = yv.x > 0.f ? g.x : 0.f; g.y = yv.y > 0.f ? g.y : 0.f;
-      g.z = yv.z > 0.f ? g.z : 0.f; g.w = yv.w > 0.f ? g.w : 0.f;
-    }
-    s1 += (g.x + g.y) + (g.z + g.w);
-    s2 += (g.x * ((xv.x - mu) * is) + g.y * ((xv.y - mu) * is)) + (g.z * ((xv.z - mu) * is) + g.w * ((xv.w - mu) * is));
+    float4 yv = xv;
+    if (MASK == BN_MASK_Y) yv = reinterpret_cast<const float4 *>(y + off)[i];
+    g = bn_masked<MASK>(g, xv, yv, a, b);
+    bn_bwd_item(g, xv, mu, is, s1, s2);
     if ((it & 7) == 7) { d1 += s1; d2 += s2; s1 = 0.f; s2 = 0.f; }
   }
   d1 += s1; d2 += s2;
@@ -168,11 +230,37 @@
   }
 }
 
-template <bool RELU, bool TRAIN, bool DRES>
+__device__ __forceinline__ void bn_bwd_channel_sums(const double *__restrict__ part, int c, int nsplit, bool publish,
+                                                    float *sg , float *__restrict__ dgamma,
+                                                    float *__restrict__ dbeta, float *__restrict__ gacc,
+                                                    float *__restrict__ bacc) {
+  if (threadIdx.x < 64) {
+    double s1 = 0.0, s2 = 0.0;
+    if ((int)threadIdx.x < nsplit) {
+      s1 = part[threadIdx.x * 2 + 0];
+      s2 = part[threadIdx.x * 2 + 1];
+    }
+    s1 = salun_wave_sum(s1);
+    s2 = salun_wave_sum(s2);
+    if (threadIdx.x == 0) {
+      sg[0] = (float)s1;
+      sg[1] = (float)s2;
+      if (publish) {
+        dbeta[c] = (float)s1;
+        dgamma[c] = (float)s2;
+        if (gacc) gacc[c] += (float)s2;
+        if (bacc) bacc[c] += (float)s1;
+      }
+    }
+  }
+  __syncthreads();
+}
+
+template <int MASK, bool TRAIN, bool DRES>
 __global__ __launch_bounds__(256) void k_bn_bwd_apply(const float *__restrict__ dy, const float *__restrict__ y,
                                                       const float *__restrict__ x, const float *__restrict__ mean,
                                                       const float *__restrict__ invstd,
-                                                      const float *__restrict__ gamma,
+                                                      const float *__restrict__ gamma, const float *__restrict__ beta,
                                                       const double *__restrict__ partial, float *__restrict__ dgamma,
                                                       float *__restrict__ dbeta, float *__restrict__ gacc,
                                                       float *__restrict__ bacc, float *__restrict__ dx,
@@ -180,29 +268,12 @@
                                                       float inv_m) {
   __shared__ float sg[2];
   const int c = blockIdx.x, s = blockIdx.y;
-  if (threadIdx.x < 64) {
-    double s1 = 0.0, s2 = 0.0;
-    if ((int)threadIdx.x < nsplit) {
-      s1 = partial[((size_t)c * nsplit + threadIdx.x) * 2 + 0];
-      s2 = partial[((size_t)c * nsplit + threadIdx.x) * 2 + 1];
-    }
-    s1 = salun_wave_sum(s1);
-    s2 = salun_wave_sum(s2);
-    if (threadIdx.x == 0) {
-      sg[0] = (float)s1;
-      sg[1] = (float)s2;
-      if (s == 0) {
-        dbeta[c] = (float)s1;
-        dgamma[c] = (float)s2;
-        if (gacc) gacc[c] += (float)s2;
-        if (bacc) bacc[c] += (float)s1;
-      }
-    }
-  }
-  __syncthreads();
+  bn_bwd_channel_sums(partial + (size_t)c * nsplit * 2, c, nsplit, s == 0, sg, dgamma, dbeta, gacc, bacc);
   const float mu = mean[c], is = invstd[c];
   const float gi = gamma[c] * is;
   const float kb = sg[0] * inv_m, kg = sg[1] * inv_m;
+  float a = 0.f, b = 0.f;
+  if (MASK == BN_MASK_X) bn_affine(mu, is, gamma[c], beta[c], a, b);
   const int n_lo = (int)((int64_t)N * s / nsplit), n_hi = (int)((int64_t)N * (s + 1) / nsplit);
   const int hw4 = HW >> 2;
   const int work = (n_hi - n_lo) * hw4;
@@ -212,24 +283,148 @@
     const int n = wk.n, i = wk.i;
     const size_t off = ((size_t)n * C + c) * HW;
     float4 g = reinterpret_cast<const float4 *>(dy + off)[i];
-    if (RELU) {
-      const float4 yv = reinterpret_cast<const float4 *>(y + off)[i];
-      g.x = yv.x > 0.f ? g.x : 0.f; g.y = yv.y > 0.f ? g.y : 0.f;
-      g.z = yv.z > 0.f ? g.z : 0.f; g.w = yv.w > 0.f ? g.w : 0.f;
-    }
+    float4 xv = g;
+    if (TRAIN || MASK == BN_MASK_X) xv = reinterpret_cast<const float4 *>(x + off)[i];
+    float4 yv = g;
+    if (MASK == BN_MASK_Y) yv = reinterpret_cast<const float4 *>(y + off)[i];
+    g = bn_masked<MASK>(g, xv, yv, a, b);
     if (DRES) reinterpret_cast<float4 *>(dres + off)[i] = g;
-    float4 o;
-    if (TRAIN) {
-      const float4 xv = reinterpret_cast<const float4 *>(x + off)[i];
-      o.x = gi * (g.x - (kb + ((xv.x - mu) * is) * kg));
-      o.y = gi * (g.y - (kb + ((xv.y - mu) * is) * kg));
-      o.z = gi * (g.z - (kb + ((xv.z - mu) * is) * kg));
-      o.w = gi * (g.w - (kb + ((xv.w - mu) * is) * kg));
-    } else {
-      o.x = gi * g.x; o.y = gi * g.y; o.z = gi * g.z; o.w = gi * g.w;
-    }
-    reinterpret_cast<float4 *>(dx + off)[i] = o;
-  }
+    reinterpret_cast<float4 *>(dx + off)[i] = bn_dx_item<TRAIN>(g, xv, gi, kb, kg, mu, is);
+  }
+}
+
+template <int ITEMS, class Item, class Close>
+__device__ __forceinline__ void bn_rr_pass(int N, int nsplit, int hw4, Item item, Close close) {
+  int s = 0, it = 0;
+  int n_hi = (int)((int64_t)N / nsplit);
+  int work = n_hi * hw4;
+  BnWalk wk(0, hw4);
+#pragma unroll
+  for (int j = 0; j < ITEMS; ++j) {
+    if (s < nsplit && it * 256 >= work) {
+      close(s);
+      ++s;
+      it = 0;
+      const int n_lo = n_hi;
+      n_hi = (int)((int64_t)N * (s + 1) / nsplit);
+      work = (n_hi - n_lo) * hw4;
+      wk = BnWalk(n_lo, hw4);
+    }
+    if (s < nsplit) {
+      if ((int)threadIdx.x + it * 256 < work) item(j, it, wk.n, wk.i);
+      ++it;
+      wk.next();
+    }
+  }
+  if (s < nsplit) close(s);
+}
+
+template <bool RELU, bool RES, bool TRAIN, int ITEMS>
+__global__ __launch_bounds__(256) void k_bn_fwd_rr(const float *__restrict__ x, const float *__restrict__ res,
+                                                   float *__restrict__ y, float *__restrict__ mean,
+                                                   float *__restrict__ invstd, const float *__restrict__ gamma,
+                                                   const float *__restrict__ beta, float *__restrict__ running_mean,
+                                                   float *__restrict__ running_var,
+                                                   long long *__restrict__ num_batches_tracked, int N, int C, int HW,
+                                                   int nsplit, float eps, float momentum) {
+  __shared__ double lds[4];
+  __shared__ double tot[2 * BN_MAX_SPLIT];
+  __shared__ float st[2];
+  const int c = blockIdx.x;
+  const int hw4 = HW >> 2;
+  float4 v[ITEMS];
+  bn_rr_pass<ITEMS>(
+      N, nsplit, hw4,
+      [&](int j, int, int n, int i) { v[j] = reinterpret_cast<const float4 *>(x + ((size_t)n * C + c) * HW)[i]; },
+      [](int) {});
+  if (TRAIN) {
+    float s1 = 0.f, s2 = 0.f;
+    double d1 = 0.0, d2 = 0.0;
+    bn_rr_pass<ITEMS>(
+        N, nsplit, hw4,
+        [&](int j, int it, int, int) {
+          bn_stats_item(v[j], s1, s2);
+          if ((it & 7) == 7) { d1 += s1; d2 += s2; s1 = 0.f; s2 = 0.f; }
+        },
+        [&](int s) {
+          d1 += s1; d2 += s2;
+          const double t1 = salun_block_sum(d1, lds);
+          const double t2 = salun_block_sum(d2, lds);
+          if (threadIdx.x == 0) { tot[s * 2 + 0] = t1; tot[s * 2 + 1] = t2; }
+          s1 = 0.f; s2 = 0.f; d1 = 0.0; d2 = 0.0;
+        });
+    __syncthreads();
+  }
+  bn_fwd_stats<TRAIN>(tot, c, nsplit, (double)N * HW, eps, st, true, momentum, mean, invstd, running_mean, running_var,
+                      num_batches_tracked);
+  float a, b;
+  bn_affine(st[0], st[1], gamma[c], beta[c], a, b);
+  bn_rr_pass<ITEMS>(
+      N, nsplit, hw4,
+      [&](int j, int, int n, int i) {
+        const size_t off = ((size_t)n * C + c) * HW;
+        float4 r = v[j];
+        if (RES) r = reinterpret_cast<const float4 *>(res + off)[i];
+        reinterpret_cast<float4 *>(y + off)[i] = bn_apply_item<RELU, RES>(v[j], r, a, b);
+      },
+      [](int) {});
+}
+
+template <int MASK, bool TRAIN, bool DRES, int ITEMS>
+__global__ __launch_bounds__(256) void k_bn_bwd_rr(const float *__restrict__ dy, const float *__restrict__ y,
+                                                   const float *__restrict__ x, const float *__restrict__ mean,
+                                                   const float *__restrict__ invstd, const float *__restrict__ gamma,
+                                                   const float *__restrict__ beta, float *__restrict__ dgamma,
+                                                   float *__restrict__ dbeta, float *__restrict__ gacc,
+                                                   float *__restrict__ bacc, float *__restrict__ dx,
+                                                   float *__restrict__ dres, int N, int C, int HW, int nsplit,
+                                                   float inv_m) {
+  __shared__ double lds[4];
+  __shared__ double tot[2 * BN_MAX_SPLIT];
+  __shared__ float sg[2];
+  const int c = blockIdx.x;
+  const int hw4 = HW >> 2;
+  const float mu = mean[c], is = invstd[c];
+  float a = 0.f, b = 0.f;
+  if (MASK == BN_MASK_X) bn_affine(mu, is, gamma[c], beta[c], a, b);
+  float4 g[ITEMS], xv[ITEMS], yv[MASK == BN_MASK_Y ? ITEMS : 1];
+  bn_rr_pass<ITEMS>(
+      N, nsplit, hw4,
+      [&](int j, int, int n, int i) {
+        const size_t off = ((size_t)n * C + c) * HW;
+        g[j] = reinterpret_cast<const float4 *>(dy + off)[i];
+        xv[j] = reinterpret_cast<const float4 *>(x + off)[i];
+        if (MASK == BN_MASK_Y) yv[MASK == BN_MASK_Y ? j : 0] = reinterpret_cast<const float4 *>(y + off)[i];
+      },
+      [](int) {});
+  float s1 = 0.f, s2 = 0.f;
+  double d1 = 0.0, d2 = 0.0;
+  bn_rr_pass<ITEMS>(
+      N, nsplit, hw4,
+      [&](int j, int it, int, int) {
+        g[j] = bn_masked<MASK>(g[j], xv[j], yv[MASK == BN_MASK_Y ? j : 0], a, b);
+        bn_bwd_item(g[j], xv[j], mu, is, s1, s2);
+        if ((it & 7) == 7) { d1 += s1; d2 += s2; s1 = 0.f; s2 = 0.f; }
+      },
+      [&](int s) {
+        d1 += s1; d2 += s2;
+        const double t1 = salun_block_sum(d1, lds);
+        const double t2 = salun_block_sum(d2, lds);
+        if (threadIdx.x == 0) { tot[s * 2 + 0] = t1; tot[s * 2 + 1] = t2; }
+        s1 = 0.f; s2 = 0.f; d1 = 0.0; d2 = 0.0;
+      });
+  __syncthreads();
+  bn_bwd_channel_sums(tot, c, nsplit, true, sg, dgamma, dbeta, gacc, bacc);
+  const float gi = gamma[c] * is;
+  const float kb = sg[0] * inv_m, kg = sg[1] * inv_m;
+  bn_rr_pass<ITEMS>(
+      N, nsplit, hw4,
+      [&](int j, int, int n, int i) {
+        const size_t off = ((size_t)n * C + c) * HW;
+        if (DRES) reinterpret_cast<float4 *>(dres + off)[i] = g[j];
+        reinterpret_cast<float4 *>(dx + off)[i] = bn_dx_item<TRAIN>(g[j], xv[j], gi, kb, kg, mu, is);
+      },
+      [](int) {});
 }
 
 inline int bn_nsplit(int N, int C) {
@@ -240,10 +435,76 @@
   return ns;
 }
 
+inline int bn_rr_items(int N, int HW, int ns) {
+  int64_t rounds = 0;
+  for (int s = 0; s < ns; ++s) {
+    const int64_t n_lo = (int64_t)N * s / ns, n_hi = (int64_t)N * (s + 1) / ns;
+    rounds += ((n_hi - n_lo) * (HW >> 2) + 255) / 256;
+  }
+  if (rounds > BN_RR_MAX_ITEMS) return 0;
+  return rounds <= 4 ? 4 : rounds <= 8 ? 8 : 16;
+}
+
+inline int bn_route(int route, int N, int C, int HW, int ns) {
+  if (route == SALUN_BN_ROUTE_TWO_PASS) return 0;
+  const int items = bn_rr_items(N, HW, ns);
+  if (route == SALUN_BN_ROUTE_REGISTER) return items > 0 ? items : -1;
+  return BN_RR_AUTO && C >= BN_RR_MIN_C ? items : 0;
+}
+
 }
 
 SALUN_EXPORT size_t salun_bn_workspace_bytes(int C) {
   return sizeof(double) * 2 * (size_t)(C > 0 ? C : 0) * BN_MAX_SPLIT;
+}
+
+SALUN_EXPORT int salun_bn_forward_ex(const float *x, const float *res, float *y, const float *gamma, const float *beta,
+                                     float *running_mean, float *running_var, long long *num_batches_tracked,
+                                     float *save_mean, float *save_invstd, int N, int C, int HW, int training,
+                                     double momentum, double eps, int relu, int route, void *ws, size_t ws_bytes,
+                                     salun_stream_t stream) {
+  if (!x || !y || !gamma || !beta || !save_mean || !save_invstd || N < 1 || C < 1 || HW < 4 || (HW & 3))
+    return SALUN_EINVAL;
+  if (route < SALUN_BN_ROUTE_AUTO || route > SALUN_BN_ROUTE_REGISTER) return SALUN_EINVAL;
+  if (!training && (!running_mean || !running_var)) return SALUN_EINVAL;
+  if (!salun_aligned16(x) || !salun_aligned16(y) || (res && !salun_aligned16(res))) return SALUN_EINVAL;
+  const int ns = bn_nsplit(N, C);
+  const int items = bn_route(route, N, C, HW, ns);
+  if (items < 0) return SALUN_EINVAL;
+  if (training && (!ws || ws_bytes < salun_bn_workspace_bytes(C))) return SALUN_ENOSPC;
+  hipStream_t st = salun_hip_stream(stream);
+  double *partial = static_cast<double *>(ws);
+  if (training && items == 0) {
+    hipLaunchKernelGGL(k_bn_stats_partial, dim3(C, ns), dim3(256), 0, st, x, N, C, HW, ns, partial);
+    SALUN_LAUNCH_CHECK();
+  }
+#define SALUN_BN_RR(RELU_, RES_, TRAIN_, I_)                                                                       \
+  hipLaunchKernelGGL((k_bn_fwd_rr<RELU_, RES_, TRAIN_, I_>), dim3(C), dim3(256), 0, st, x, res, y, save_mean,       \
+                     save_invstd, gamma, beta, running_mean, running_var, num_batches_tracked, N, C, HW, ns,       \
+                     (float)eps, (float)momentum)
+#define SALUN_BN_APPLY(RELU_, RES_, TRAIN_)                                                                       \
+  switch (items) {                                                                                                \
+    case 4: SALUN_BN_RR(RELU_, RES_, TRAIN_, 4); break;                                                           \
+    case 8: SALUN_BN_RR(RELU_, RES_, TRAIN_, 8); break;                                                           \
+    case 16: SALUN_BN_RR(RELU_, RES_, TRAIN_, 16); break;                                                         \
+    default:                                                                                                      \
+      hipLaunchKernelGGL((k_bn_apply<RELU_, RES_, TRAIN_>), dim3(C, ns), dim3(256), 0, st, x, res, y, partial,     \
+                         save_mean, save_invstd, gamma, beta, running_mean, running_var, num_batches_tracked, N, \
+                         C, HW, ns, (float)eps, (float)momentum);                                                 \
+  }
+  const bool r = relu != 0, a = res != nullptr, t = training != 0;
+  if (r && a && t) { SALUN_BN_APPLY(true, true, true) }
+  else if (r && a) { SALUN_BN_APPLY(true, true, false) }
+  else if (r && t) { SALUN_BN_APPLY(true, false, true) }
+  else if (r) { SALUN_BN_APPLY(true, false, false) }
+  else if (a && t) { SALUN_BN_APPLY(false, true, true) }
+  else if (a) { SALUN_BN_APPLY(false, true, false) }
+  else if (t) { SALUN_BN_APPLY(false, false, true) }
+  else { SALUN_BN_APPLY(false, false, false) }
+#undef SALUN_BN_APPLY
+#undef SALUN_BN_RR
+  SALUN_LAUNCH_CHECK();
+  return SALUN_OK;
 }
 
 SALUN_EXPORT int salun_bn_forward(const float *x, const float *res, float *y, const float *gamma, const float *beta,
@@ -251,32 +512,72 @@
                                   float *save_mean, float *save_invstd, int N, int C, int HW, int training,
                                   double momentum, double eps, int relu, void *ws, size_t ws_bytes,
                                   salun_stream_t stream) {
-  if (!x || !y || !gamma || !beta || !save_mean || !save_invstd || N < 1 || C < 1 || HW < 4 || (HW & 3))
+  return salun_bn_forward_ex(x, res, y, gamma, beta, running_mean, running_var, num_batches_tracked, save_mean,
+                             save_invstd, N, C, HW, training, momentum, eps, relu, SALUN_BN_ROUTE_AUTO, ws, ws_bytes,
+                             stream);
+}
+
+SALUN_EXPORT int salun_bn_backward_ex(const float *dy, const float *y, const float *x, const float *gamma,
+                                      const float *save_mean, const float *save_invstd, float *dx, float *dres,
+                                      float *dgamma, float *dbeta, float *grad_gamma_acc, float *grad_beta_acc, int N,
+                                      int C, int HW, int training, int relu, const float *beta, int route, void *ws,
+                                      size_t ws_bytes, salun_stream_t stream) {
+  const int mask = !relu ? BN_MASK_NONE : beta ? BN_MASK_X : BN_MASK_Y;
+  if (!dy || !x || !gamma || !save_mean || !save_invstd || !dx || !dgamma || !dbeta || N < 1 || C < 1 || HW < 4 ||
+      (HW & 3) || (mask == BN_MASK_Y && !y))
     return SALUN_EINVAL;
-  if (!training && (!running_mean || !running_var)) return SALUN_EINVAL;
-  if (!salun_aligned16(x) || !salun_aligned16(y) || (res && !salun_aligned16(res))) return SALUN_EINVAL;
+  if (route < SALUN_BN_ROUTE_AUTO || route > SALUN_BN_ROUTE_REGISTER) return SALUN_EINVAL;
+  if (mask == BN_MASK_X && dres) return SALUN_EINVAL;
+  if (!ws || ws_bytes < salun_bn_workspace_bytes(C)) return SALUN_ENOSPC;
+  if (!salun_aligned16(dy) || !salun_aligned16(x) || !salun_aligned16(dx) ||
+      (mask == BN_MASK_Y && !salun_aligned16(y)) || (dres && !salun_aligned16(dres)))
+    return SALUN_EINVAL;
+  const int ns = bn_nsplit(N, C);
+  const int items = bn_route(route, N, C, HW, ns);
+  if (items < 0) return SALUN_EINVAL;
   hipStream_t st = salun_hip_stream(stream);
-  const int ns = bn_nsplit(N, C);
   double *partial = static_cast<double *>(ws);
-  if (training) {
-    if (!ws || ws_bytes < salun_bn_workspace_bytes(C)) return SALUN_ENOSPC;
-    hipLaunchKernelGGL(k_bn_stats_partial, dim3(C, ns), dim3(256), 0, st, x, N, C, HW, ns, partial);
+  const float inv_m = (float)(1.0 / ((double)N * HW));
+  if (items == 0) {
+#define SALUN_BN_PARTIAL(MASK_)                                                                                  \
+  hipLaunchKernelGGL(k_bn_bwd_partial<MASK_>, dim3(C, ns), dim3(256), 0, st, dy, y, x, save_mean, save_invstd,    \
+                     gamma, beta, N, C, HW, ns, partial)
+    if (mask == BN_MASK_X) SALUN_BN_PARTIAL(BN_MASK_X);
+    else if (mask == BN_MASK_Y) SALUN_BN_PARTIAL(BN_MASK_Y);
+    else SALUN_BN_PARTIAL(BN_MASK_NONE);
+#undef SALUN_BN_PARTIAL
     SALUN_LAUNCH_CHECK();
   }
-#define SALUN_BN_APPLY(RELU_, RES_, TRAIN_)                                                                       \
-  hipLaunchKernelGGL((k_bn_apply<RELU_, RES_, TRAIN_>), dim3(C, ns), dim3(256), 0, st, x, res, y, partial,         \
-                     save_mean, save_invstd, gamma, beta, running_mean, running_var, num_batches_tracked, N, C,  \
-                     HW, ns, (float)eps, (float)momentum)
-  const bool r = relu != 0, a = res != nullptr, t = training != 0;
-  if (r && a && t) SALUN_BN_APPLY(true, true, true);
-  else if (r && a) SALUN_BN_APPLY(true, true, false);
-  else if (r && t) SALUN_BN_APPLY(true, false, true);
-  else if (r) SALUN_BN_APPLY(true, false, false);
-  else if (a && t) SALUN_BN_APPLY(false, true, true);
-  else if (a) SALUN_BN_APPLY(false, true, false);
-  else if (t) SALUN_BN_APPLY(false, false, true);
-  else SALUN_BN_APPLY(false, false, false);
-#undef SALUN_BN_APPLY
+#define SALUN_BN_RR(MASK_, TRAIN_, DRES_, I_)                                                                       \
+  hipLaunchKernelGGL((k_bn_bwd_rr<MASK_, TRAIN_, DRES_, I_>), dim3(C), dim3(256), 0, st, dy, y, x, save_mean,        \
+                     save_invstd, gamma, beta, dgamma, dbeta, grad_gamma_acc, grad_beta_acc, dx, dres, N, C, HW,   \
+                     ns, inv_m)
+#define SALUN_BN_BWD(MASK_, TRAIN_, DRES_)                                                                          \
+  switch (items) {                                                                                                  \
+    case 4: SALUN_BN_RR(MASK_, TRAIN_, DRES_, 4); break;                                                            \
+    case 8: SALUN_BN_RR(MASK_, TRAIN_, DRES_, 8); break;                                                            \
+    case 16: SALUN_BN_RR(MASK_, TRAIN_, DRES_, 16); break;                                                          \
+    default:                                                                                                        \
+      hipLaunchKernelGGL((k_bn_bwd_apply<MASK_, TRAIN_, DRES_>), dim3(C, ns), dim3(256), 0, st, dy, y, x,           \
+                         save_mean, save_invstd, gamma, beta, partial, dgamma, dbeta, grad_gamma_acc,               \
+                         grad_beta_acc, dx, dres, N, C, HW, ns, inv_m);                                             \
+  }
+  const bool t = training != 0, d = dres != nullptr;
+  if (mask == BN_MASK_X) {
+    if (t) { SALUN_BN_BWD(BN_MASK_X, true, false) } else { SALUN_BN_BWD(BN_MASK_X, false, false) }
+  } else if (mask == BN_MASK_Y) {
+    if (t && d) { SALUN_BN_BWD(BN_MASK_Y, true, true) }
+    else if (t) { SALUN_BN_BWD(BN_MASK_Y, true, false) }
+    else if (d) { SALUN_BN_BWD(BN_MASK_Y, false, true) }
+    else { SALUN_BN_BWD(BN_MASK_Y, false, false) }
+  } else {
+    if (t && d) { SALUN_BN_BWD(BN_MASK_NONE, true, true) }
+    else if (t) { SALUN_BN_BWD(BN_MASK_NONE, true, false) }
+    else if (d) { SALUN_BN_BWD(BN_MASK_NONE, false, true) }
+    else { SALUN_BN_BWD(BN_MASK_NONE, false, false) }
+  }
+#undef SALUN_BN_BWD
+#undef SALUN_BN_RR
   SALUN_LAUNCH_CHECK();
   return SALUN_OK;
 }
@@ -286,36 +587,9 @@
                                    float *dgamma, float *dbeta, float *grad_gamma_acc, float *grad_beta_acc, int N,
                                    int C, int HW, int training, int relu, void *ws, size_t ws_bytes,
                                    salun_stream_t stream) {
-  if (!dy || !x || !gamma || !save_mean || !save_invstd || !dx || !dgamma || !dbeta || N < 1 || C < 1 || HW < 4 ||
-      (HW & 3) || (relu && !y))
-    return SALUN_EINVAL;
-  if (!ws || ws_bytes < salun_bn_workspace_bytes(C)) return SALUN_ENOSPC;
-  if (!salun_aligned16(dy) || !salun_aligned16(x) || !salun_aligned16(dx) || (y && !salun_aligned16(y)) ||
-      (dres && !salun_aligned16(dres)))
-    return SALUN_EINVAL;
-  hipStream_t st = salun_hip_stream(stream);
-  const int ns = bn_nsplit(N, C);
-  double *partial = static_cast<double *>(ws);
-  if (relu) hipLaunchKernelGGL(k_bn_bwd_partial<true>, dim3(C, ns), dim3(256), 0, st, dy, y, x, save_mean, save_invstd, N, C, HW, ns, partial);
-  else hipLaunchKernelGGL(k_bn_bwd_partial<false>, dim3(C, ns), dim3(256), 0, st, dy, y, x, save_mean, save_invstd, N, C, HW, ns, partial);
-  SALUN_LAUNCH_CHECK();
-  const float inv_m = (float)(1.0 / ((double)N * HW));
-#define SALUN_BN_BWD(RELU_, TRAIN_, DRES_)                                                                          \
-  hipLaunchKernelGGL((k_bn_bwd_apply<RELU_, TRAIN_, DRES_>), dim3(C, ns), dim3(256), 0, st, dy, y, x, save_mean,   \
-                     save_invstd, gamma, partial, dgamma, dbeta, grad_gamma_acc, grad_beta_acc, dx, dres, N, C, HW, \
-                     ns, inv_m)
-  const bool r = relu != 0, t = training != 0, d = dres != nullptr;
-  if (r && t && d) SALUN_BN_BWD(true, true, true);
-  else if (r && t) SALUN_BN_BWD(true, true, false);
-  else if (r && d) SALUN_BN_BWD(true, false, true);
-  else if (r) SALUN_BN_BWD(true, false, false);
-  else if (t && d) SALUN_BN_BWD(false, true, true);
-  else if (t) SALUN_BN_BWD(false, true, false);
-  else if (d) SALUN_BN_BWD(false, false, true);
-  else SALUN_BN_BWD(false, false, false);
-#undef SALUN_BN_BWD
-  SALUN_LAUNCH_CHECK();
-  return SALUN_OK;
+  return salun_bn_backward_ex(dy, y, x, gamma, save_mean, save_invstd, dx, dres, dgamma, dbeta, grad_gamma_acc,
+                              grad_beta_acc, N, C, HW, training, relu, nullptr, SALUN_BN_ROUTE_AUTO, ws, ws_bytes,
+                              stream);
 }
 
 namespace {
diff --git a/unlearn_saliency_amd/norm.py b/unlearn_saliency_amd/norm.py
--- a/unlearn_saliency_amd/norm.py
+++ b/unlearn_saliency_amd/norm.py
@@ -16,7 +16,7 @@
         if out is None:
             raise RuntimeError("fused BN: unsupported shape (H*W must be a multiple of 4)")
         y, mean, invstd = out
-        ctx.save_for_backward(x, y if relu else None, weight, bias, mean, invstd)
+        ctx.save_for_backward(x, y if relu and residual is not None else None, weight, bias, mean, invstd)
         ctx.params = (weight, bias)
         ctx.cfg = (bool(training), bool(relu), residual is not None)
         ctx.mark_non_differentiable(mean, invstd)
@@ -30,7 +30,8 @@
         if gw is None or gb is None:
             gw = gb = None
         dx, dres, dgamma, dbeta = ops.bn_backward(dy.contiguous(), y, x, weight, mean, invstd, training, relu,
-                                                  has_res and ctx.needs_input_grad[3], gw, gb)
+                                                  has_res and ctx.needs_input_grad[3], gw, gb, beta=bias,
+                                                  no_residual=not has_res)
         if gw is not None:
             gradsink.arrived(weight)
             gradsink.arrived(bias)
diff --git a/unlearn_saliency_amd/ops.py b/unlearn_saliency_amd/ops.py
--- a/unlearn_saliency_amd/ops.py
+++ b/unlearn_saliency_amd/ops.py
@@ -766,44 +766,50 @@
 
 
 def bn_forward(x, res, gamma, beta, running_mean, running_var, training, momentum, eps, relu,
-               num_batches_tracked=None):
+               num_batches_tracked=None, route=0):
     N, C, H, W = x.shape
     L = _lib.lib()
     y = torch.empty_like(x)
     mean = torch.empty(C, dtype=torch.float32, device=x.device)
     invstd = torch.empty(C, dtype=torch.float32, device=x.device)
     ws = workspace(L.salun_bn_workspace_bytes(C), x.device)
-    rc = L.salun_bn_forward(_dev(x, torch.float32, "x"), _dev(res, torch.float32, "res", True), c_void_p(y.data_ptr()),
-                            _dev(gamma, torch.float32, "weight"), _dev(beta, torch.float32, "bias"),
-                            _dev(running_mean, torch.float32, "running_mean", True),
-                            _dev(running_var, torch.float32, "running_var", True),
-                            _dev(num_batches_tracked, torch.int64, "num_batches_tracked", True),
-                            c_void_p(mean.data_ptr()),
-                            c_void_p(invstd.data_ptr()), N, C, H * W, int(bool(training)), c_double(momentum),
-                            c_double(eps), int(bool(relu)), c_void_p(ws.data_ptr()), c_size_t(ws.numel()), _stream())
+    rc = L.salun_bn_forward_ex(_dev(x, torch.float32, "x"), _dev(res, torch.float32, "res", True),
+                               c_void_p(y.data_ptr()),
+                               _dev(gamma, torch.float32, "weight"), _dev(beta, torch.float32, "bias"),
+                               _dev(running_mean, torch.float32, "running_mean", True),
+                               _dev(running_var, torch.float32, "running_var", True),
+                               _dev(num_batches_tracked, torch.int64, "num_batches_tracked", True),
+                               c_void_p(mean.data_ptr()),
+                               c_void_p(invstd.data_ptr()), N, C, H * W, int(bool(training)), c_double(momentum),
+                               c_double(eps), int(bool(relu)), int(route), c_void_p(ws.data_ptr()),
+                               c_size_t(ws.numel()), _stream())
     if rc == _lib.SALUN_EINVAL:
         return None
-    check(rc, "salun_bn_forward")
+    check(rc, "salun_bn_forward_ex")
     return y, mean, invstd
 
 
-def bn_backward(dy, y, x, gamma, mean, invstd, training, relu, want_dres, gamma_grad_acc=None, beta_grad_acc=None):
+def bn_backward(dy, y, x, gamma, mean, invstd, training, relu, want_dres, gamma_grad_acc=None, beta_grad_acc=None,
+                beta=None, no_residual=False, route=0):
     N, C, H, W = x.shape
     L = _lib.lib()
+    mask_from_x = bool(relu) and bool(no_residual) and beta is not None and not want_dres
     dx = torch.empty_like(x)
     dres = torch.empty_like(x) if want_dres else None
     dgamma = torch.empty(C, dtype=torch.float32, device=x.device)
     dbeta = torch.empty(C, dtype=torch.float32, device=x.device)
     ws = workspace(L.salun_bn_workspace_bytes(C), x.device)
-    check(L.salun_bn_backward(_dev(dy, torch.float32, "dy"), _dev(y, torch.float32, "y", True),
-                              _dev(x, torch.float32, "x"), _dev(gamma, torch.float32, "weight"),
-                              _dev(mean, torch.float32, "mean"), _dev(invstd, torch.float32, "invstd"),
-                              c_void_p(dx.data_ptr()), _dev(dres, torch.float32, "dres", True),
-                              c_void_p(dgamma.data_ptr()), c_void_p(dbeta.data_ptr()),
-                              _dev(gamma_grad_acc, torch.float32, "gamma.grad", True),
-                              _dev(beta_grad_acc, torch.float32, "beta.grad", True), N, C, H * W,
-                              int(bool(training)), int(bool(relu)), c_void_p(ws.data_ptr()), c_size_t(ws.numel()),
-                              _stream()), "salun_bn_backward")
+    check(L.salun_bn_backward_ex(_dev(dy, torch.float32, "dy"),
+                                 None if mask_from_x else _dev(y, torch.float32, "y", True),
+                                 _dev(x, torch.float32, "x"), _dev(gamma, torch.float32, "weight"),
+                                 _dev(mean, torch.float32, "mean"), _dev(invstd, torch.float32, "invstd"),
+                                 c_void_p(dx.data_ptr()), _dev(dres, torch.float32, "dres", True),
+                                 c_void_p(dgamma.data_ptr()), c_void_p(dbeta.data_ptr()),
+                                 _dev(gamma_grad_acc, torch.float32, "gamma.grad", True),
+                                 _dev(beta_grad_acc, torch.float32, "beta.grad", True), N, C, H * W,
+                                 int(bool(training)), int(bool(relu)),
+                                 _dev(beta, torch.float32, "bias") if mask_from_x else None, int(route),
+                                 c_void_p(ws.data_ptr()), c_size_t(ws.numel()), _stream()), "salun_bn_backward_ex")
     return dx, dres, dgamma, dbeta
 
 
diff --git a/unlearn_saliency_amd/resblock.py b/unlearn_saliency_amd/resblock.py
--- a/unlearn_saliency_amd/resblock.py
+++ b/unlearn_saliency_amd/resblock.py
@@ -62,11 +62,12 @@
         dout = dout.contiguous()
         grads = {}
 
-        def bn_bwd(dy, y, xin, g, b, m, i, relu, want_dres):
+        def bn_bwd(dy, y, xin, g, b, m, i, relu, want_dres, no_residual=False):
             gw, gb = gradsink.sink(g), gradsink.sink(b)
             if gw is None or gb is None:
                 gw = gb = None
-            dx, dres, dg, db = ops.bn_backward(dy, y, xin, g, m, i, training, relu, want_dres, gw, gb)
+            dx, dres, dg, db = ops.bn_backward(dy, y, xin, g, m, i, training, relu, want_dres, gw, gb, beta=b,
+                                               no_residual=no_residual)
             if gw is not None:
                 gradsink.arrived(g)
                 gradsink.arrived(b)
@@ -97,7 +98,7 @@
             dxd = ops.conv2d_backward_data(dcd, wd, x.shape, s, 0) if ctx.needs_input_grad[0] else None
         dw2 = wgrad(y1, dc2, w2, 1, 1)
         dy1 = ops.conv2d_backward_data(dc2, w2, y1.shape, 1, 1)
-        dc1, _, dg1, db1 = bn_bwd(dy1, y1, c1, g1, b1, m1, i1, True, False)
+        dc1, _, dg1, db1 = bn_bwd(dy1, y1, c1, g1, b1, m1, i1, True, False, no_residual=True)
         dw1 = wgrad(x, dc1, w1, s, 1)
         dx = ops.conv2d_backward_data(dc1, w1, x.shape, s, 1, addend=dxd) if ctx.needs_input_grad[0] else None
         if overlap and not all(g is None for g in (dw1, dw2, dwd)):
```
